# gvanhorn38/multibox

Measured on AMD Instinct MI355X. Metric: images/sec (299x299, 5-AR priors) train, higher is better.
Workload: dtype bf16; 1 GPU; full train step: Inception-ResNet-v2 + multibox heads fwd, on-device matching+loss, bwd, RMSProp+EMA; 299x299, k=5 (P=646), BATCH_SIZE=64/GPU, MAX_NUM_BBOXES=13; global_batch=64, parallelism=dp1, hip_graph=True

## Files before the change

### include/mbx.h

```cpp
#ifndef MBX_H
#define MBX_H

#include <stddef.h>
#include <stdint.h>

#ifdef __cplusplus
extern "C" {
#endif

typedef void* mbx_stream_t;

typedef enum {
  MBX_OK = 0,
  MBX_ERR_INVALID_ARG = -1,
  MBX_ERR_UNSUPPORTED = -2,
  MBX_ERR_LAUNCH = -3,
  MBX_ERR_WORKSPACE = -4
} mbx_status;

int mbx_version(void);
const char* mbx_status_string(int status);

int mbx_priors_count(int k, const int* grids, int n_grids);

uint32_t mbx_crc32c(const void* data, uint64_t n, uint32_t crc);
int mbx_generate_priors(const double* aspect_ratios, int k, double min_scale, double max_scale,
                        int restrict_to_image_bounds, const int* grids, int n_grids,
                        double* out );

int mbx_decode_conf(const float* raw_locs , const float* logits ,
                    const float* priors , int B, int P, float eps_add,
                    float* decoded , float* conf , mbx_stream_t stream);

size_t mbx_match_workspace_bytes(int B, int P, int G);
int mbx_match(const float* decoded , const float* conf ,
              const float* gt , const int32_t* n_gt , float alpha,
              int B, int P, int G, int32_t* match , int32_t* status ,
              void* workspace, size_t workspace_bytes, mbx_stream_t stream);

int mbx_match_extend(const float* priors , const float* gt ,
                     const int32_t* n_gt , const int32_t* status ,
                     float iou_threshold, int B, int P, int G,
                     int32_t* match ,
                     int32_t* n_extra , mbx_stream_t stream);

size_t mbx_loss_workspace_bytes(int B);
int mbx_loss_fwd_bwd(const float* decoded , const float* conf_in ,
                     int conf_is_logit, const float* gt ,
                     const int32_t* match , float alpha, float grad_scale, int B, int P,
                     int G, float* loss2 ,
                     float* d_raw_locs , float* d_logits ,
                     void* workspace, size_t workspace_bytes, mbx_stream_t stream);

size_t mbx_loss_mined_workspace_bytes(int B, int P);
int mbx_loss_fwd_bwd_mined(const float* decoded , const float* conf_in ,
                           int conf_is_logit, const float* gt ,
                           const int32_t* match , float alpha, float grad_scale, int B, int P,
                           int G, float* loss2 ,
                           float* d_raw_locs , float* d_logits ,
                           int neg_per_pos, int min_neg, int32_t* n_neg ,
                           void* workspace, size_t workspace_bytes, mbx_stream_t stream);

size_t mbx_loss_focal_workspace_bytes(int B, int P);
int mbx_loss_fwd_bwd_focal(const float* decoded , const float* conf_in ,
                           int conf_is_logit, const float* gt ,
                           const int32_t* match , float alpha, float grad_scale, int B, int P,
                           int G, float* loss2 ,
                           float* d_raw_locs , float* d_logits ,
                           float gamma, float w_pos, float w_neg,
                           int neg_per_pos , int min_neg, int32_t* n_neg ,
                           void* workspace, size_t workspace_bytes, mbx_stream_t stream);

typedef struct {
  int32_t offset_y, offset_x;
  int32_t patch_h, patch_w;
  int32_t image_h, image_w;
  int32_t is_flipped;
  int32_t max_to_keep;
  float restrictions[4];
} mbx_patch_meta;

int mbx_decode_filter_topk(const float* raw_locs , const float* conf ,
                           const float* priors , const mbx_patch_meta* meta ,
                           int B, int P, int k_max, double* out_boxes ,
                           float* out_scores , int32_t* out_index ,
                           int32_t* out_count , mbx_stream_t stream);

int mbx_nms(double* boxes , float* scores , int32_t* index ,
            int32_t* count , int B, int k_max, double iou_threshold, mbx_stream_t stream);

#define MBX_MERGE_MAX_CANDIDATES 16384
int mbx_merge_detections(const double* boxes , const float* scores ,
                         const int32_t* count , const int32_t* image_rows , int I, int k_max,
                         int max_det, double iou_threshold, double* out_boxes ,
                         float* out_scores , int32_t* out_src ,
                         int32_t* out_count , int32_t* out_status , mbx_stream_t stream);

int mbx_merge_detections_voted(const double* boxes , const float* scores ,
                               const int32_t* count , const int32_t* image_rows , int I,
                               int k_max, int max_det, double iou_threshold, double vote_iou_threshold,
                               double* out_boxes , float* out_scores ,
                               int32_t* out_src , int32_t* out_count ,
                               int32_t* out_status , int32_t* out_votes , mbx_stream_t stream);

#define MBX_SOFT_LINEAR 1
#define MBX_SOFT_GAUSSIAN 2
int mbx_merge_detections_soft(const double* boxes , const float* scores ,
                              const int32_t* count , const int32_t* image_rows , int I, int k_max,
                              int max_det, int method, double iou_threshold , double sigma ,
                              double min_score, double vote_iou_threshold ,
                              double* out_boxes , float* out_scores ,
                              int32_t* out_src , int32_t* out_count , int32_t* out_status ,
                              int32_t* out_votes , mbx_stream_t stream);

#define MBX_COCO_MAX_DET 100
#define MBX_COCO_MAX_GT 128
int mbx_coco_match(const double* dt , const int32_t* dt_rows ,
                   const double* gt , const int32_t* gt_rows , int I,
                   const double* iou_thrs , int T, const double* area_rng ,
                   int A, int16_t* match , uint8_t* ignore ,
                   int32_t* n_gt_counted , int32_t* status , mbx_stream_t stream);

#define MBX_COCO_ACC_MAX_R 128
#define MBX_COCO_ACC_MAX_M 4
#define MBX_COCO_ACC_MAX_ND 4194304
#define MBX_COCO_ACC_CHUNK 256
#define MBX_COCO_ACC_SORT_TILE 1024
size_t mbx_coco_accumulate_workspace(long long ND, int T, int A, int M);
int mbx_coco_accumulate(const double* dt , const int32_t* dt_rows , int I,
                        const int16_t* match , const uint8_t* ignore ,
                        const int32_t* n_gt_counted , int T, int A, const double* rec_thrs , int R,
                        const int32_t* max_dets , int M, double* precision ,
                        double* recall , void* workspace, size_t workspace_bytes, mbx_stream_t stream);

typedef enum {
  MBX_EPI_STORE = 0,
  MBX_EPI_AFFINE = 1,
  MBX_EPI_RESIDUAL = 2,
  MBX_EPI_STORE_F32 = 3
} mbx_epilogue;

typedef struct {
  int32_t n, rows_mod;
  int32_t c_begin[4];
  const void* y[4]; int32_t ld_y[4];
  const float* relu_thr[4];
  float* stats[4]; int32_t stats_ld[4];
} mbx_bn_bwd_stats;

#define MBX_GRID_BARRIER_BYTES 6400
typedef struct {
  void* barrier;
  void* a; int32_t ld_a;
  const float* beta;
  float* mean; float* rstd;
  float* moving_mean; float* moving_var;
  float* relu_thr;
  int32_t relu; float eps, decay;
  float* step_poison;
} mbx_bn_apply_desc;

#define MBX_BN_BWD_SLOTS 8
typedef struct {
  void* barrier;
  int32_t n;
  int32_t c_begin[4];
  const void* y[4]; int32_t ld_y[4];
  void* dy[4]; int32_t ld_dy[4];
  const float* mean[4]; const float* rstd[4]; const float* beta[4];
  float* dbeta[4];
  float* acc[4]; int32_t acc_ld[4];
  int32_t relu[4];
  float* step_poison;
} mbx_bn_bwd_fused;

typedef struct {
  const void* x; int64_t x_img_stride; int32_t ldx;
  int32_t N, H_in, W_in, C_in;
  const void* w; int32_t C_out, R, S;
  int32_t stride, transposed, pad_t, pad_l, H_out, W_out;
  void* y; int64_t y_img_stride; int32_t ldy;
  int32_t epilogue, relu, accumulate;
  const float* scale; const float* shift;
  const void* skip; int64_t skip_img_stride; int32_t ld_skip; float rscale;
  float* stats_partial;
  int32_t tile_config;
  const void* acc_src; int64_t acc_img_stride; int32_t ld_acc;
  int32_t* work_counter;
  int32_t max_workgroups;
  void* splitk_ws; int64_t splitk_ws_bytes;
  int32_t stats_rows_mod, stats_ld;
  const mbx_bn_bwd_stats* bn_bwd_stats;
  void* relu_bits; int32_t ld_bits;
  const mbx_bn_apply_desc* bn_apply;
  const mbx_bn_bwd_fused* bn_bwd;
} mbx_conv_desc;
#define MBX_CONV_TILE_CONFIGS 14
#define MBX_TILE_I5_BASE 32
#define MBX_TILE_I7 65
#define MBX_TILE_DIRECT3 96
#define MBX_TILE_DIRECTW 97
#define MBX_TILE_RESIDENT 98
#define MBX_TILE_PWRES 99
#define MBX_TILE_SPLITK_BASE 128
#define MBX_TILE_SPLITK_MAX 32

int mbx_conv_stats_rows(const mbx_conv_desc* desc );
int mbx_conv(const mbx_conv_desc* desc , mbx_stream_t stream);
int mbx_conv_supported(const mbx_conv_desc* desc );
int mbx_conv_pair(const mbx_conv_desc* a , const mbx_conv_desc* b , mbx_stream_t stream);
size_t mbx_conv_splitk_workspace_bytes(const mbx_conv_desc* desc );

int mbx_conv_wgrad(const mbx_conv_desc* desc , const void* dy,
                   int64_t dy_img_stride, int32_t ld_dy, float* dw, float* db, mbx_stream_t stream);

typedef struct {
  mbx_conv_desc desc;
  const void* dy; int64_t dy_img_stride; int32_t ld_dy;
  float scale;
  float* dw; float* db;
} mbx_wgrad_job;
typedef struct {
  int32_t n_layers, n_items;
  int64_t layers_off, items_off;
  int64_t queues_off, heads_off;
  double flops;
  int64_t tally_off;
} mbx_wgrad_plan_info;
#define MBX_WGRAD_DETERMINISTIC 1
#define MBX_WGRAD_SCATTER 2
size_t mbx_wgrad_plan_bytes(const mbx_wgrad_job* jobs , int n_jobs, int flags);
int mbx_wgrad_plan(const mbx_wgrad_job* jobs , int n_jobs, int flags, void* host_image, size_t bytes,
                   mbx_wgrad_plan_info* info );
int mbx_conv_wgrad_grouped(void* device_image , const mbx_wgrad_plan_info* info ,
                           mbx_stream_t stream);
int mbx_conv_wgrad_grouped_capped(void* device_image, const mbx_wgrad_plan_info* info , int max_workgroups,
                                  mbx_stream_t stream);

int mbx_conv_wgrad_scaled(const mbx_conv_desc* desc, const void* dy, int64_t dy_img_stride,
                          int32_t ld_dy, float scale, float* dw, float* db, mbx_stream_t stream);

int mbx_bn_finalize(const float* stats_partial , int rows, int C, int64_t count,
                    float eps, float decay, float* mean , float* rstd ,
                    float* moving_mean , float* moving_var ,
                    mbx_stream_t stream);
int mbx_bn_apply(const void* y, int64_t M, int C, const float* mean, const float* rstd,
                 const float* beta, int relu, void* a, int ld_a, mbx_stream_t stream);
int mbx_bn_apply_fused(const float* stats_partial, int rows, int64_t count, float eps, float decay,
                       const void* y, int64_t M, int C, const float* beta, int relu, void* a, int ld_a,
                       float* mean, float* rstd, float* moving_mean, float* moving_var,
                       mbx_stream_t stream);
int mbx_bn_apply_fused_mapped(const void* stats_fixed, int rows, int64_t count, float eps, float decay,
                              const void* y, int64_t M, int C, const float* beta, int relu, void* a, int ld_a,
                              const struct mbx_chan_map_s* a_map , float* mean, float* rstd, float* moving_mean,
                              float* moving_var, float* relu_thr, mbx_stream_t stream);
int mbx_bn_moving_update(float* moving_mean, float* moving_var, const float* batch_mean, const float* batch_var,
                         int64_t n, float decay, const float* skip_ctl, uint64_t* skipped_steps,
                         float* ema_mean, float* ema_var, float ema_decay, mbx_stream_t stream);
typedef struct mbx_chan_map_s { int32_t n; int32_t c_begin[4]; int32_t offset[4]; } mbx_chan_map;
int mbx_bn_finalize_parts(const float* const* parts , const int32_t* rows ,
                          const int32_t* Cs , int n_parts, int64_t count, float eps, float decay, float* mean,
                          float* rstd, float* moving_mean, float* moving_var, mbx_stream_t stream);
int mbx_bn_apply_mapped(const void* y, int64_t M, int C, const float* mean, const float* rstd, const float* beta,
                        int relu, void* a, int ld_a, const mbx_chan_map* a_map , mbx_stream_t stream);
int mbx_bn_apply_maxpool(const void* y, int N, int H, int W, int C, const float* mean, const float* rstd, const float* beta,
                         int relu, void* p, int64_t p_img_stride, int ld_p, int Ho, int Wo, uint8_t* argmax,
                         mbx_stream_t stream);
int mbx_bn_fold(const float* moving_mean, const float* moving_var, const float* beta, float eps,
                int C, float* scale, float* shift, mbx_stream_t stream);
int mbx_bn_bwd_rows(int64_t M, int C);
int mbx_bn_bwd_reduce(const void* da, int ld_da, const void* a, int ld_a, int relu, const void* y,
                      int64_t M, int C, const float* mean, const float* rstd, const float* beta,
                      float* partial , mbx_stream_t stream);
int mbx_bn_bwd_finalize(const float* partial, int rows, int C, int64_t M, float* dbeta ,
                        float* m12 , mbx_stream_t stream);
int mbx_bn_bwd_apply(const void* da, int ld_da, const void* a, int ld_a, int relu, const void* y,
                     int64_t M, int C, const float* mean, const float* rstd, const float* beta,
                     const float* m12, void* dy , mbx_stream_t stream);

int mbx_bn_bwd_reduce_mapped(const void* da, int ld_da, const void* a, int ld_a, int relu, const void* y, int64_t M, int C,
                             const float* mean, const float* rstd, const float* beta, float* partial,
                             const mbx_chan_map* da_map , mbx_stream_t stream);
int mbx_bn_bwd_apply_mapped(const void* da, int ld_da, const void* a, int ld_a, int relu, const void* y, int64_t M, int C,
                            const float* mean, const float* rstd, const float* beta, const float* m12, void* dy,
                            const mbx_chan_map* da_map , mbx_stream_t stream);

int mbx_bn_bwd_apply_rows(const float* stats, int rows, const void* da, int ld_da, const void* y, int64_t M, int C,
                          const float* mean, const float* rstd, const float* relu_thr, float* dbeta, void* dy,
                          const mbx_chan_map* da_map , mbx_stream_t stream);

size_t mbx_bn_bwd_onepass_workspace_bytes(int C);
int mbx_bn_bwd_onepass_supported(int64_t M, int C, int max_workgroups);
int mbx_bn_bwd_onepass(const void* da, int ld_da, int relu, const void* y, int64_t M, int C,
                       const float* mean, const float* rstd, const float* beta, float* dbeta ,
                       void* dy , void* ws, int max_workgroups, float* step_poison ,
                       mbx_stream_t stream);

int mbx_bn_bwd_rows_pooled(int N, int H, int W, int C);
int mbx_bn_bwd_reduce_pooled(const void* gy, int64_t gy_img_stride, int ld_gy, const uint8_t* argmax, int N, int H, int W,
                             int Ho, int Wo, int relu, const void* y, int C, const float* mean, const float* rstd,
                             const float* beta, float* partial , mbx_stream_t stream);
int mbx_bn_bwd_apply_pooled(const void* gy, int64_t gy_img_stride, int ld_gy, const uint8_t* argmax, int N, int H, int W,
                            int Ho, int Wo, int relu, const void* y, int C, const float* mean, const float* rstd,
                            const float* beta, const float* m12, void* dy, mbx_stream_t stream);
int mbx_bn_bwd_onepass_mapped(const void* da, int ld_da, int relu, const void* y, int64_t M, int C, const float* mean,
                              const float* rstd, const float* beta, float* dbeta, void* dy, void* ws, int max_workgroups,
                              float* step_poison, const mbx_chan_map* da_map , mbx_stream_t stream);

int mbx_maxpool_fwd(const void* x, int64_t x_img_stride, int ldx, int N, int H, int W, int C,
                    int k, int stride, void* y, int64_t y_img_stride, int ldy, int Ho, int Wo,
                    uint8_t* argmax , mbx_stream_t stream);
int mbx_maxpool_bwd(const void* dy, int64_t dy_img_stride, int ld_dy, const uint8_t* argmax,
                    int N, int H, int W, int C, int k, int stride, int Ho, int Wo, void* dx,
                    int64_t dx_img_stride, int ld_dx, int accumulate, mbx_stream_t stream);
int mbx_avgpool_fwd(const void* x, int64_t x_img_stride, int ldx, int N, int H, int W, int C,
                    int k, int pad, void* y, int64_t y_img_stride, int ldy, int Ho, int Wo,
                    mbx_stream_t stream);
int mbx_avgpool_bwd(const void* dy, int64_t dy_img_stride, int ld_dy, int N, int H, int W, int C,
                    int k, int pad, int Ho, int Wo, void* dx, int64_t dx_img_stride, int ld_dx,
                    int accumulate, mbx_stream_t stream);

int mbx_relu_mask(void* g, int ld_g, const void* a, int ld_a, int64_t M, int C, mbx_stream_t stream);
int mbx_pack_input(const float* img, int64_t pixels, void* out, mbx_stream_t stream);
int mbx_head_gather(const float* h, int ld_h, int N, int cells, int k, int P, int off,
                    float* locs, float* logits, mbx_stream_t stream);
int mbx_head_scatter(const float* d_locs, const float* d_logits, int N, int cells, int k, int P,
                     int off, void* g, int ld_g, mbx_stream_t stream);

typedef struct {
  const float* h; int32_t ld_h;
  void* g; int32_t ld_g;
  int32_t cells, k, off;
} mbx_head;
int mbx_head_gather_all(const mbx_head* heads , int n_heads, int N, int P, float* locs, float* logits,
                        mbx_stream_t stream);
int mbx_head_scatter_all(const float* d_locs, const float* d_logits, const mbx_head* heads , int n_heads, int N,
                         int P, mbx_stream_t stream);

int mbx_step_begin(float* grads, int64_t n_grads, float* bn_ws, int64_t n_ws, int64_t ctl_index, uint64_t* timeouts_total,
                   float* zero_scalar, mbx_stream_t stream);

typedef struct {
  int64_t src_off;
  int64_t dst_off;
  int32_t K, R, S, C, Kpad;
  int32_t first_block;
} mbx_filter_entry;
int mbx_filter_prepare(const void* w_bf16, void* w_dgrad, const mbx_filter_entry* table ,
                       int n_entries, int total_blocks, mbx_stream_t stream);

int mbx_rmsprop_ema_step(float* w, const float* g, float* ms, float* mom ,
                         float* ema , void* w_bf16 , int64_t n, float lr,
                         float decay, float momentum, float eps, float wd, float ema_decay,
                         int trainable, float* reg_loss, const float* skip_ctl, mbx_stream_t stream);
int mbx_ema_update(float* ema, const float* value, int64_t n, float ema_decay, const float* skip_ctl ,
                   mbx_stream_t stream);

typedef struct {
  uint64_t src_offset;
  int32_t src_h, src_w;
  int32_t method;
  int32_t flip;
  int32_t n_ops;
  int32_t op[4];
  int32_t pad_;
  double arg[4];
} mbx_augment_item;
size_t mbx_augment_workspace_bytes(int B, int S);
int mbx_augment_batch(const uint8_t* src , const mbx_augment_item* items , int B, int S,
                      int any_contrast, float* out , void* workspace, mbx_stream_t stream);

typedef struct {
  uint64_t src_offset;
  int32_t img_h, img_w;
  int32_t win_y, win_x, win_h, win_w;
  int32_t flip_source;
  int32_t pad_;
} mbx_patch_item;
int mbx_extract_patches(const uint8_t* src , const mbx_patch_item* items , int n, int S,
                        float* out , mbx_stream_t stream);

#ifdef __cplusplus
}
#endif
#endif
```

### multibox_amd/csrc/conv.hip

```cpp
#include <stdlib.h>

#include "conv_common.h"

namespace {

template <int BM, int BN, int WNW, int WMW, int EV, int MODE = 0, int NSTG = 3>
__device__ __forceinline__ void conv_igemm3_body(const ConvK& p, const int bid_, const int nblk_) {
  constexpr bool SH = MODE == 2, PW = MODE == 1;
  static_assert(WNW * WMW == 4 || WNW * WMW == 8, "four or eight waves");
  constexpr int NT = 64 * WNW * WMW, RPP = NT / 8;
  constexpr int TN = BN / WNW, TM = BM / WMW, NI = TN / 16, MI = TM / 16;
  constexpr int PI = BM / RPP, WI = BN / RPP, NL = PI + WI;
  constexpr int STAGE = (BM + BN) * 8;
  extern __shared__ __attribute__((aligned(16))) u32x4 smem[];

  const int tid = threadIdx.x, lane = tid & 63;
  const int wave = wave_id();
  const int wn = wave % WNW, wm = wave / WNW;
  int lid = xcd_remap(bid_, nblk_);
  int split = 0;
  if constexpr (EV == 5) { const int nt = p.tiles_m * p.tiles_n; split = lid / nt; lid -= split * nt; }
  const int tile_n = lid % p.tiles_n, tile_m = lid / p.tiles_n;
  const int m0 = tile_m * BM, n0 = tile_n * BN;

  const __amdgpu_buffer_rsrc_t xr = make_rsrc(p.x, p.x_bytes);
  const __amdgpu_buffer_rsrc_t wr = make_rsrc(p.w, p.w_bytes);
  const int lrow = tid >> 3;
  const int chunk = (tid & 7) ^ (lrow & 7);
  const int chunkw = (tid & 7) ^ ((((lrow >> 3) & 3) << 1) | ((lrow >> 1) & 1));
  int hb[PI], wb[PI], ro[PI];
#pragma unroll
  for (int i = 0; i < PI; ++i) {
    const int m = m0 + lrow + RPP * i;
    const bool mv = m < p.M;
    const unsigned mm = mv ? (unsigned)m : 0u;
    int img, oh, ow;
    if (SH && p.parity) decode_pixel_parity(p, mm, img, oh, ow); else decode_pixel(p, mm, img, oh, ow);
    hb[i] = mv ? oh * p.mul - p.pad_t : -(1 << 24);
    wb[i] = ow * p.mul - p.pad_l;
    ro[i] = SH ? img * p.x_img_stride * 2 : (img * p.x_img_stride + (hb[i] * p.W_in + wb[i]) * p.ldx) * 2;
    if (PW && !mv) ro[i] = (int)kOOB;
  }
  int wo[WI];
#pragma unroll
  for (int i = 0; i < WI; ++i) {
    const int n = n0 + lrow + RPP * i;
    wo[i] = n < p.C_out ? n * p.Ktot * 2 : -1;
  }

  f32x4 acc[NI][MI];
#pragma unroll
  for (int a = 0; a < NI; ++a)
#pragma unroll
    for (int b = 0; b < MI; ++b) acc[a][b] = f32x4{0.f, 0.f, 0.f, 0.f};

  const int frow = lane & 15, fch = lane >> 4;
  const int fr0 = frow * 8 + (fch ^ (frow & 7));
  const int fr1 = frow * 8 + ((4 + fch) ^ (frow & 7));
  const int fwrow = 8 * (frow >> 2) + (frow & 3), fwkey = ((frow >> 2) << 1) | ((frow >> 1) & 1);
  const int fw0 = fwrow * 8 + (fch ^ fwkey);
  const int fw1 = fwrow * 8 + ((4 + fch) ^ fwkey);
  int kr0 = 0, ks0 = 0, kstep = 1, nk = (p.Ktot + 63) >> 6;
  if (SH && p.skip_taps) {
    const int mlast = min(m0 + BM, p.M) - 1;
    const int c0 = pixel_class(p, m0);
    if (c0 == pixel_class(p, mlast)) {
      kr0 = (p.pad_t + (c0 >> 1)) & 1;
      ks0 = (p.pad_l + (c0 & 1)) & 1;
      kstep = 2;
      nk = ((p.R - kr0 + 1) >> 1) * ((p.S - ks0 + 1) >> 1) * (p.C_in >> 6);
    }
  }
  int kt0 = 0;
  if constexpr (EV == 5) { kt0 = split * p.kps; nk = min(p.kps, nk - kt0); }
  int kc = chunk * 8 + kt0 * 64, kr = kr0, ks = ks0;
  while (kc >= p.C_in) { kc -= p.C_in; if ((ks += kstep) >= p.S) { ks = ks0; kr += kstep; } }
  const int ldx2 = p.ldx * 2;
  int st_issue = 0, st_comp = 0;
#define MBX_ISSUE_TILE(LT)                                                                                   \
  do {                                                                                                       \
    u32x4* sp = smem + st_issue * STAGE + wave * 64;                                                         \
    const bool kv = kr < p.R;                                                                                \
    if (PW) {                                                                                                \
      _Pragma("unroll") for (int i = 0; i < PI; ++i)                                                         \
        glds16(xr, sp + i * NT, (kv && ro[i] >= 0) ? (ro[i] + kc * 2) : (int)kOOB);                          \
    } else if (!SH) {                                                                                        \
      const int toff = (kr * p.W_in + ks) * ldx2 + kc * 2;                                                   \
      _Pragma("unroll") for (int i = 0; i < PI; ++i) {                                                       \
        const bool ok = kv && ((unsigned)(hb[i] + kr) < (unsigned)p.H_in) &&                                 \
                        ((unsigned)(wb[i] + ks) < (unsigned)p.W_in);                                         \
        glds16(xr, sp + i * NT, ok ? (ro[i] + toff) : (int)kOOB);                                            \
      }                                                                                                      \
    } else {                                                                                                 \
      _Pragma("unroll") for (int i = 0; i < PI; ++i) {                                                       \
        const int hn = hb[i] + kr, wn_ = wb[i] + ks;                                                         \
        const bool ok = kv && (((hn | wn_) & 1) == 0) && ((unsigned)(hn >> 1) < (unsigned)p.H_in) &&         \
                        ((unsigned)(wn_ >> 1) < (unsigned)p.W_in);                                           \
        glds16(xr, sp + i * NT, ok ? (ro[i] + ((hn >> 1) * p.W_in + (wn_ >> 1)) * ldx2 + kc * 2) : (int)kOOB); \
      }                                                                                                      \
    }                                                                                                        \
                                 \
    const int kb = (SH && kstep == 2) ? ((kr * p.S + ks) * p.C_in + kc + (chunkw - chunk) * 8) * 2                \
                                      : (((LT) + kt0) * 64 + chunkw * 8) * 2;                                  \
    const bool kvw = (SH && kstep == 2) ? kv : (kb < p.Ktot * 2);                                              \
    u32x4* sw = sp + BM * 8;                                                                                 \
    _Pragma("unroll") for (int i = 0; i < WI; ++i)                                                           \
      glds16(wr, sw + i * NT, (kvw && wo[i] >= 0) ? (wo[i] + kb) : (int)kOOB);                               \
    kc += 64;                                                                                                \
    while (kc >= p.C_in) { kc -= p.C_in; if ((ks += kstep) >= p.S) { ks = ks0; kr += kstep; } }              \
    st_issue = st_issue == NSTG - 1 ? 0 : st_issue + 1;                                                      \
  } while (0)

  static_assert(NSTG == 2 || NSTG == 3, "ring depth");
  u32x4* const probe_base = smem + (PI + WI - 1) * NT + wave * 64 + lane;
  MBX_ISSUE_TILE(0);
  if (NSTG == 3 && nk > 1) { MBX_ISSUE_TILE(1); wait_vmcnt<NL>(); } else wait_vmcnt<0>();
  lds_readback_wait(lds_readback_issue(probe_base));
  raw_barrier();
  for (int it = 0; it < nk; ++it) {
    const bool more = it + NSTG - 1 < nk;
    if (more) MBX_ISSUE_TILE(it + NSTG - 1);
    st_comp = st_comp == NSTG - 1 ? 0 : st_comp + 1;
    const int st_prev = st_comp == 0 ? NSTG - 1 : st_comp - 1;
#ifndef MBX_NO_PROBE_I3
    unsigned probe;
    if constexpr (NSTG == 3) {
      if (more) wait_vmcnt<NL>(); else wait_vmcnt<0>();
      probe = lds_readback_issue(probe_base + st_comp * STAGE);
    }
#endif
    {
      const u32x4* cP = smem + st_prev * STAGE + (wm * TM) * 8;
      const u32x4* cW = smem + st_prev * STAGE + BM * 8 + (wn * TN) * 8;
#pragma unroll
      for (int kk = 0; kk < 2; ++kk) {
        const int fr = kk ? fr1 : fr0, fw = kk ? fw1 : fw0;
        bf16x8 wf[NI], pf[MI];
#pragma unroll
        for (int a = 0; a < NI; ++a) wf[a] = __builtin_bit_cast(bf16x8, cW[(a >> 1) * 256 + (a & 1) * 32 + fw]);
#pragma unroll
        for (int b = 0; b < MI; ++b) pf[b] = __builtin_bit_cast(bf16x8, cP[b * 128 + fr]);
#pragma unroll
        for (int a = 0; a < NI; ++a)
#pragma unroll
          for (int b = 0; b < MI; ++b)
            acc[a][b] = __builtin_amdgcn_mfma_f32_16x16x32_bf16(wf[a], pf[b], acc[a][b], 0, 0, 0);
      }
    }
#ifndef MBX_NO_PROBE_I3
    if constexpr (NSTG == 2) {
      wait_vmcnt<0>();
      probe = lds_readback_issue(probe_base + st_comp * STAGE);
    }
    lds_readback_wait(probe);
#else
    if (NSTG == 3 && more) wait_vmcnt<NL>(); else wait_vmcnt<0>();
#endif
    raw_barrier();
  }
#undef MBX_ISSUE_TILE
  wait_vmcnt<0>();
  static_assert(NI % 2 == 0, "wave tile: a multiple of 32 output channels");
  constexpr int NA = NI / 2;
  const int cl0 = wn * TN + fch * 8;
  if constexpr (EV == 5) {
#pragma unroll
    for (int b = 0; b < MI; ++b) {
      const int m = m0 + wm * TM + b * 16 + frow;
      if (m >= p.M) continue;
      const int img = (int)fast_div((unsigned)m, p.mg_hw, p.sh_hw), pix = m - img * p.HW_out;
      float* yrow = reinterpret_cast<float*>(p.y) + split * p.y_split_stride + img * p.y_img_stride + pix * p.ldy;
#pragma unroll
      for (int a = 0; a < NI; ++a) {
        const int c0 = n0 + cl0 + 32 * (a >> 1) + 4 * (a & 1);
#pragma unroll
        for (int r = 0; r < 4; ++r)
          if (c0 + r < p.C_out) yrow[c0 + r] = acc[a][b][r];
      }
    }
  } else {
    float s1[NA][8], s2[NA][8];
    conv_epilogue_direct<EV, SH, NI, MI, ((EV == 2 || EV == 6) && MI * NA >= 8 && MI % 2 == 0) ? 2 : MI>(p, acc, m0 + wm * TM + frow, n0 + cl0, s1, s2);
    if constexpr (EV == 1 || EV == 6) {
      float* red = reinterpret_cast<float*>(smem);
#pragma unroll
      for (int A = 0; A < NA; ++A) { row_sum16_x8(s1[A]); row_sum16_x8(s2[A]); }
#pragma unroll
      for (int A = 0; A < NA; ++A)
#pragma unroll
        for (int j = 0; j < 8; ++j) {
          const float x1 = s1[A][j], x2 = s2[A][j];
          if (frow == 0) {
            red[((wm * BN) + cl0 + 32 * A + j) * 2] = x1;
            red[((wm * BN) + cl0 + 32 * A + j) * 2 + 1] = x2;
          }
        }
      __syncthreads();
      if (tid < BN && n0 + tid < p.C_out) {
        float x1 = 0.f, x2 = 0.f;
#pragma unroll
        for (int w = 0; w < WMW; ++w) { x1 += red[(w * BN + tid) * 2]; x2 += red[(w * BN + tid) * 2 + 1]; }
        if constexpr (EV == 6) bw_stats_write(p, tile_m, n0 + tid, x1, x2); else stats_write(p, tile_m, n0 + tid, x1, x2);
      }
    }
  }
}

template <int BM, int BN, int WNW, int WMW, int EV, int MODE = 0, int NSTG = 3>
__global__ void __launch_bounds__(64 * WNW * WMW)
conv_igemm3_kernel(const ConvK p) {
  conv_igemm3_body<BM, BN, WNW, WMW, EV, MODE, NSTG>(p, (int)blockIdx.x, (int)gridDim.x);
}

template <int BM, int BN, int WNW, int WMW, int EV, int MODE = 0, int NSTG = 3>
__global__ void __launch_bounds__(64 * WNW * WMW)
conv_igemm3_pair_kernel(const ConvK p0, const ConvK p1, const int n0) {
  if ((int)blockIdx.x < n0) conv_igemm3_body<BM, BN, WNW, WMW, EV, MODE, NSTG>(p0, (int)blockIdx.x, n0);
  else conv_igemm3_body<BM, BN, WNW, WMW, EV, MODE, NSTG>(p1, (int)blockIdx.x - n0, (int)gridDim.x - n0);
}

constexpr int kSplitRows = 16;
__global__ void __launch_bounds__(256)
splitk_reduce_kernel(const float* __restrict__ part, int ksplit, long long slice_stride, int M, int C, int ldp,
                     unsigned short* __restrict__ y, int HW_out, long long y_img_stride, int ldy, float* __restrict__ stats,
                     int stats_mod, int stats_ld, float stats_cap) {
  __shared__ float red[kSplitRows][256][2];
  const int m0 = blockIdx.x * kSplitRows, tid = threadIdx.x;
  for (int cb = 0; cb < C; cb += 256) {
    const int cw = min(256, C - cb), c4 = (cw + 3) >> 2;
    if (cb) __syncthreads();
    for (int item = tid; item < kSplitRows * c4; item += 256) {
      const int r = item / c4, gq = item - r * c4, m = m0 + r, c = cb + 4 * gq;
      float4 a = make_float4(0.f, 0.f, 0.f, 0.f);
      if (m < M) {
        const float* src = part + (size_t)m * ldp + c;
        a = *reinterpret_cast<const float4*>(src);
        int sl = 1;
        for (; sl + 3 < ksplit; sl += 4) {
          const float4 b0 = *reinterpret_cast<const float4*>(src + (sl + 0) * slice_stride);
          const float4 b1 = *reinterpret_cast<const float4*>(src + (sl + 1) * slice_stride);
          const float4 b2 = *reinterpret_cast<const float4*>(src + (sl + 2) * slice_stride);
          const float4 b3 = *reinterpret_cast<const float4*>(src + (sl + 3) * slice_stride);
          a.x = (((a.x + b0.x) + b1.x) + b2.x) + b3.x; a.y = (((a.y + b0.y) + b1.y) + b2.y) + b3.y;
          a.z = (((a.z + b0.z) + b1.z) + b2.z) + b3.z; a.w = (((a.w + b0.w) + b1.w) + b2.w) + b3.w;
        }
        for (; sl < ksplit; ++sl) {
          const float4 b = *reinterpret_cast<const float4*>(src + sl * slice_stride);
          a.x += b.x; a.y += b.y; a.z += b.z; a.w += b.w;
        }
      }
      const float v[4] = {a.x, a.y, a.z, a.w};
      const unsigned q2[2] = {pack2bf(v[0], v[1]), pack2bf(v[2], v[3])};
      const unsigned q[4] = {q2[0] & 0xffffu, q2[0] >> 16, q2[1] & 0xffffu, q2[1] >> 16};
#pragma unroll
      for (int j = 0; j < 4; ++j) {
        const float f = (m < M && c + j < C) ? bf2f((unsigned short)q[j]) : 0.f;
        if (4 * gq + j < 256) { red[r][4 * gq + j][0] = f; red[r][4 * gq + j][1] = f * f; }
      }
      if (m < M) {
        const int img = m / HW_out, pix = m - img * HW_out;
        unsigned short* dst = y + img * y_img_stride + (long long)pix * ldy + c;
        if (c + 3 < C) *reinterpret_cast<u32x2*>(dst) = u32x2{q2[0], q2[1]};
        else for (int j = 0; j < 4; ++j) if (c + j < C) dst[j] = (unsigned short)q[j];
      }
    }
    if (stats) {
      __syncthreads();
      if (tid < cw) {
        float x1 = 0.f, x2 = 0.f;
#pragma unroll
        for (int r = 0; r < kSplitRows; ++r) { x1 += red[r][tid][0]; x2 += red[r][tid][1]; }
        if (stats_mod) {
          unsigned long long* o = reinterpret_cast<unsigned long long*>(stats) + ((size_t)((int)blockIdx.x % stats_mod) * stats_ld + cb + tid) * 2;
          stats_add_fixed(o, x1, x2, stats_cap);
        } else {
          float* o = stats + ((size_t)blockIdx.x * stats_ld + cb + tid) * 2;
          o[0] = x1;
          o[1] = x2;
        }
      }
    }
  }
}

struct TileCfg { int BM, BN; float eff; };
const TileCfg kCfgs[] = {{128, 128, 1.00f}, {128, 64, 0.85f}, {64, 128, 0.85f}, {128, 32, 0.60f}, {64, 64, 0.70f},
                          {256, 128, 1.30f}, {128, 128, 1.10f}, {256, 64, 1.0f},
                          {128, 128, 1.10f},
                          {128, 64, 0.85f}, {64, 64, 0.70f},
                          {128, 64, 0.85f}, {256, 64, 1.0f}, {128, 128, 1.0f}};

int pick_cfg(long M, int C_out) {
  int best = 0;
  double best_t = 1e300;
  for (int i = 0; i < (int)(sizeof(kCfgs) / sizeof(kCfgs[0])); ++i) {
    if (i >= 5) continue;
    const TileCfg& c = kCfgs[i];
    const long tiles = ((M + c.BM - 1) / c.BM) * ((C_out + c.BN - 1) / c.BN);
    const long lds = 3L * (c.BM + c.BN) * 128;
    long per_cu = (160 * 1024) / lds;
    if (per_cu > 2) per_cu = 2;
    const long rounds = (tiles + 256 * per_cu - 1) / (256 * per_cu);
    const double t = (double)rounds * c.BM * c.BN / c.eff;
    if (t < best_t) { best_t = t; best = i; }
  }
  return best;
}



constexpr int kNumCfgs = MBX_CONV_TILE_CONFIGS;
static_assert(kGbCtlWords * 4 == MBX_GRID_BARRIER_BYTES && kFbSlots == MBX_BN_BWD_SLOTS, "include/mbx.h and csrc/grid_barrier.h agree");
constexpr int kI5Flag = MBX_TILE_I5_BASE;
constexpr int kI7Cfg = MBX_TILE_I7;
constexpr int kDirectCfg = MBX_TILE_DIRECT3;
constexpr int kDirectWCfg = MBX_TILE_DIRECTW;
constexpr int kResidentCfg = MBX_TILE_RESIDENT;
constexpr int kPwResCfg = MBX_TILE_PWRES;
constexpr int kSplitFlag = MBX_TILE_SPLITK_BASE;
constexpr int kSplitMax = MBX_TILE_SPLITK_MAX;
inline void splitk_geom(int nk, int S, int& ksplit, int& kps) {
  if (S > nk) S = nk;
  if (S < 1) S = 1;
  kps = (nk + S - 1) / S;
  ksplit = (nk + kps - 1) / kps;
}
int choose_cfg(long M, int C_out, int desc_cfg) {
  static const int force = mbx_env_int("MBX_FORCE_CFG", -1);
  if (force >= 0) return force;
  if (desc_cfg > 0 && desc_cfg <= kNumCfgs) return desc_cfg - 1;
  {
    const long cols = (C_out + 127) / 128, tiles8 = ((M + 127) / 128) * cols;
    if (tiles8 >= 384 && (double)C_out >= 0.6 * (double)(cols * 128)) return 8;
  }
  if (C_out >= 256) {
    const long tiles5 = ((M + 255) / 256) * ((C_out + 127) / 128);
    const long rounds5 = (tiles5 + 255) / 256;
    if (tiles5 >= 128 && (double)tiles5 / (double)(rounds5 * 256) >= 0.7) return 5;
  }
  return pick_cfg(M, C_out);
}

struct PairCapture { ConvK k; int bm, bn, wnw, wmw, nstg, ev, mode, valid; };
thread_local PairCapture g_capture;

template <int BM, int BN, int WNW, int WMW, int EV, int NSTG>
int launch_pair_inst(const ConvK& a, const ConvK& b, hipStream_t s) {
  static bool attr = false;
  const size_t lds = NSTG * (size_t)(BM + BN) * 128;
  if (!attr) {
    (void)hipFuncSetAttribute(reinterpret_cast<const void*>(conv_igemm3_pair_kernel<BM, BN, WNW, WMW, EV, 0, NSTG>),
                              hipFuncAttributeMaxDynamicSharedMemorySize, (int)lds);
    attr = true;
  }
  const int n0 = a.tiles_m * a.tiles_n, n1 = b.tiles_m * b.tiles_n;
  hipLaunchKernelGGL((conv_igemm3_pair_kernel<BM, BN, WNW, WMW, EV, 0, NSTG>), dim3(n0 + n1), dim3(64 * WNW * WMW), lds, s, a, b, n0);
  MBX_LAUNCH_CHECK();
  return MBX_OK;
}

template <int BM, int BN, int WNW, int WMW, int NSTG = 3>
int launch_igemm(ConvK& k, hipStream_t s) {
  k.tiles_m = (k.M + BM - 1) / BM;
  k.tiles_n = (k.C_out + BN - 1) / BN;
  k.stats_cap = stats_cap_for(k.tiles_m);
  if (k.dry == 2) {
    g_capture.k = k; g_capture.bm = BM; g_capture.bn = BN; g_capture.wnw = WNW; g_capture.wmw = WMW; g_capture.nstg = NSTG;
    g_capture.ev = k.epi == MBX_EPI_STORE_F32 ? 5 : k.epi == MBX_EPI_RESIDUAL ? 4 : k.epi == MBX_EPI_AFFINE ? 3
                   : k.bw_n ? 6 : k.stats ? 1 : (k.accumulate || k.skip || k.bits) ? 2 : 0;
    g_capture.mode = k.shift ? 2 : k.pw ? 1 : 0;
    g_capture.valid = 1;
    return MBX_OK;
  }
  {
    const size_t lds = NSTG * (size_t)(BM + BN) * 128;
    const int ev = k.epi == MBX_EPI_STORE_F32 ? 5 : k.epi == MBX_EPI_RESIDUAL ? 4 : k.epi == MBX_EPI_AFFINE ? 3
                   : k.bw_n ? 6 : k.stats ? 1 : (k.accumulate || k.skip || k.bits) ? 2 : 0;
    static bool attr_set3[7] = {false, false, false, false, false, false, false};
#define MBX_LAUNCH_EV(EV)                                                                                     \
    case EV:                                                                                                  \
      if (!attr_set3[EV]) {                                                                                   \
        (void)hipFuncSetAttribute(reinterpret_cast<const void*>(conv_igemm3_kernel<BM, BN, WNW, WMW, EV, 0, NSTG>), \
                                  hipFuncAttributeMaxDynamicSharedMemorySize, (int)lds);                      \
        (void)hipFuncSetAttribute(reinterpret_cast<const void*>(conv_igemm3_kernel<BM, BN, WNW, WMW, EV, 1, NSTG>), \
                                  hipFuncAttributeMaxDynamicSharedMemorySize, (int)lds);                      \
        attr_set3[EV] = true;                                                                                 \
      }                                                                                                       \
      if (k.pw)                                                                                               \
        hipLaunchKernelGGL((conv_igemm3_kernel<BM, BN, WNW, WMW, EV, 1, NSTG>), dim3(k.tiles_m * k.tiles_n * (EV == 5 ? k.ksplit : 1)), \
                           dim3(64 * WNW * WMW), lds, s, k);                                                  \
      else                                                                                                    \
        hipLaunchKernelGGL((conv_igemm3_kernel<BM, BN, WNW, WMW, EV, 0, NSTG>), dim3(k.tiles_m * k.tiles_n * (EV == 5 ? k.ksplit : 1)), \
                           dim3(64 * WNW * WMW), lds, s, k);                                                  \
      break;
    static bool attr_sh[2] = {false, false};
#define MBX_LAUNCH_SH(EV, SLOT)                                                                               \
    do {                                                                                                      \
      if (!attr_sh[SLOT]) {                                                                                   \
        (void)hipFuncSetAttribute(reinterpret_cast<const void*>(conv_igemm3_kernel<BM, BN, WNW, WMW, EV, 2, NSTG>), \
                                  hipFuncAttributeMaxDynamicSharedMemorySize, (int)lds);                      \
        attr_sh[SLOT] = true;                                                                                 \
      }                                                                                                       \
      hipLaunchKernelGGL((conv_igemm3_kernel<BM, BN, WNW, WMW, EV, 2, NSTG>), dim3(k.tiles_m * k.tiles_n),      \
                         dim3(64 * WNW * WMW), lds, s, k);                                                    \
    } while (0)
    if (k.dry) return (k.shift && ev != 0 && ev != 2) ? MBX_ERR_UNSUPPORTED : MBX_OK;
    if (k.shift) {
      if (ev == 0) MBX_LAUNCH_SH(0, 0);
      else if (ev == 2) MBX_LAUNCH_SH(2, 1);
      else return MBX_ERR_UNSUPPORTED;
    } else
    switch (ev) {
      MBX_LAUNCH_EV(0) MBX_LAUNCH_EV(1) MBX_LAUNCH_EV(2) MBX_LAUNCH_EV(3) MBX_LAUNCH_EV(4) MBX_LAUNCH_EV(5) MBX_LAUNCH_EV(6)
    }
#undef MBX_LAUNCH_SH
#undef MBX_LAUNCH_EV
  }
  MBX_LAUNCH_CHECK();
  return MBX_OK;
}

}

extern "C" int mbx_conv_stats_rows(const mbx_conv_desc* d) {
  if (!d) return MBX_ERR_INVALID_ARG;
  if (d->stats_rows_mod > 0) return d->stats_rows_mod;
  const long M = (long)d->N * d->H_out * d->W_out;
  if (d->tile_config > kSplitFlag) return (int)((M + kSplitRows - 1) / kSplitRows);
  if (d->tile_config == kDirectCfg) return mbx_direct3_grid(d->N, d->H_out, d->W_out);
  if (d->tile_config == kDirectWCfg) { const int g = mbx_directw_grid(d->N, d->H_out, d->W_out); return g > 0 ? g : MBX_ERR_UNSUPPORTED; }
  if (d->tile_config == kResidentCfg) return mbx_resident_rows(d->N);
  if (d->tile_config == kI7Cfg) return (int)((M + 127) / 128);
  if (d->tile_config > kI5Flag) {
    const int i = d->tile_config - kI5Flag - 1;
    if (i >= mbx_i5_num_tiles) return MBX_ERR_INVALID_ARG;
    return (int)((M + mbx_i5_tiles[i][0] - 1) / mbx_i5_tiles[i][0]);
  }
  const TileCfg& c = kCfgs[choose_cfg(M, d->C_out, d->tile_config)];
  return (int)((M + c.BM - 1) / c.BM);
}

static int conv_impl(const mbx_conv_desc* d, mbx_stream_t stream, int dry);
extern "C" int mbx_conv(const mbx_conv_desc* d, mbx_stream_t stream) { return conv_impl(d, stream, 0); }
extern "C" int mbx_conv_supported(const mbx_conv_desc* d) { return conv_impl(d, nullptr, 1); }
extern "C" int mbx_conv_pair(const mbx_conv_desc* a, const mbx_conv_desc* b, mbx_stream_t stream) {
  PairCapture ca, cb;
  g_capture.valid = 0;
  int st = conv_impl(a, stream, 2);
  if (st != MBX_OK) return st;
  if (!g_capture.valid) return MBX_ERR_UNSUPPORTED;
  ca = g_capture;
  g_capture.valid = 0;
  st = conv_impl(b, stream, 2);
  if (st != MBX_OK) return st;
  if (!g_capture.valid) return MBX_ERR_UNSUPPORTED;
  cb = g_capture;
  if (ca.bm != cb.bm || ca.bn != cb.bn || ca.wnw != cb.wnw || ca.wmw != cb.wmw || ca.nstg != cb.nstg || ca.ev != cb.ev ||
      ca.mode != 0 || cb.mode != 0 || (ca.ev != 0 && ca.ev != 1 && ca.ev != 6) || ca.wnw != 2 || ca.wmw != 2 || ca.bn != 64)
    return MBX_ERR_UNSUPPORTED;
  ca.k.dry = cb.k.dry = 0;
  hipStream_t s = mbx_s(stream);
#define MBX_PAIR(BM_, NSTG_)                                                                                      \
  if (ca.bm == BM_ && ca.nstg == NSTG_)                                                                           \
    return ca.ev == 6 ? launch_pair_inst<BM_, 64, 2, 2, 6, NSTG_>(ca.k, cb.k, s)                                    \
           : ca.ev ? launch_pair_inst<BM_, 64, 2, 2, 1, NSTG_>(ca.k, cb.k, s) : launch_pair_inst<BM_, 64, 2, 2, 0, NSTG_>(ca.k, cb.k, s);
  MBX_PAIR(128, 2) MBX_PAIR(128, 3) MBX_PAIR(64, 2) MBX_PAIR(64, 3)
#undef MBX_PAIR
  return MBX_ERR_UNSUPPORTED;
}

extern "C" size_t mbx_conv_splitk_workspace_bytes(const mbx_conv_desc* d) {
  if (!d || d->tile_config <= kSplitFlag || d->tile_config > kSplitFlag + kSplitMax) return 0;
  int ksplit, kps;
  splitk_geom((d->R * d->S * d->C_in + 63) >> 6, d->tile_config - kSplitFlag, ksplit, kps);
  return (size_t)4 * d->N * d->H_out * d->W_out * (((d->C_out + 7) / 8) * 8) * ksplit;
}

static int conv_impl(const mbx_conv_desc* d, mbx_stream_t stream, int dry) {
  int st = check_desc(d);
  if (st != MBX_OK) return st;
  if (!d->w || !d->y) return MBX_ERR_INVALID_ARG;
  if ((reinterpret_cast<uintptr_t>(d->w) & 15)) return MBX_ERR_INVALID_ARG;
  const bool f32 = d->epilogue == MBX_EPI_STORE_F32;
  if (!f32 && (d->C_out % 8 || d->ldy % 8 || (reinterpret_cast<uintptr_t>(d->y) & 15))) return MBX_ERR_INVALID_ARG;
  if (d->epilogue == MBX_EPI_RESIDUAL && (!d->skip || d->ld_skip % 8 || (reinterpret_cast<uintptr_t>(d->skip) & 15)))
    return MBX_ERR_INVALID_ARG;
  if ((long long)d->N * d->y_img_stride >= (1LL << 31)) return MBX_ERR_UNSUPPORTED;
  if (d->stats_partial && (d->epilogue != MBX_EPI_STORE || d->accumulate || d->skip)) return MBX_ERR_INVALID_ARG;
  if (d->epilogue == MBX_EPI_STORE && d->skip && (d->ld_skip % 8 || (reinterpret_cast<uintptr_t>(d->skip) & 15))) return MBX_ERR_INVALID_ARG;
  MBX_ENTER();
  ConvK k;
  k.x = reinterpret_cast<const unsigned short*>(d->x);
  k.x_img_stride = (int)d->x_img_stride; k.ldx = d->ldx; k.H_in = d->H_in; k.W_in = d->W_in; k.C_in = d->C_in;
  k.w = reinterpret_cast<const unsigned short*>(d->w);
  k.C_out = d->C_out; k.R = d->R; k.S = d->S; k.Ktot = d->R * d->S * d->C_in;
  k.x_bytes = (unsigned)(2 * ((long long)(d->N - 1) * d->x_img_stride + ((long long)d->H_in * d->W_in - 1) * d->ldx + d->C_in));
  k.w_bytes = (unsigned)(2LL * d->C_out * k.Ktot);
  if (d->transposed) { k.mul = 1; k.shift = d->stride == 2 ? 1 : 0; } else { k.mul = d->stride; k.shift = 0; }
  k.pad_t = d->pad_t; k.pad_l = d->pad_l; k.W_out = d->W_out; k.HW_out = d->H_out * d->W_out;
  k.M = d->N * k.HW_out;
  k.y = d->y; k.y_img_stride = (int)d->y_img_stride; k.ldy = d->ldy;
  k.epi = d->epilogue; k.relu = d->relu; k.accumulate = d->accumulate;
  k.scale = d->scale; k.shiftv = d->shift;
  k.skip = reinterpret_cast<const unsigned short*>(d->skip);
  k.skip_img_stride = (int)d->skip_img_stride; k.ld_skip = d->ld_skip; k.rscale = d->rscale;
  k.bits = nullptr; k.bits_ld = 0; k.bits_bytes = 0;
  if (d->relu_bits) {
    const bool wr = d->epilogue == MBX_EPI_RESIDUAL && d->relu, rd = d->epilogue == MBX_EPI_STORE && !d->skip;
    if ((!wr && !rd) || d->ld_bits % 4 || d->ld_bits < 4 * ((d->C_out + 31) / 32) || (reinterpret_cast<uintptr_t>(d->relu_bits) & 3)) return MBX_ERR_INVALID_ARG;
    if (d->stats_partial || d->bn_bwd_stats) return MBX_ERR_UNSUPPORTED;
    const long long bb = (long long)d->N * d->H_out * d->W_out * d->ld_bits;
    if (bb >= (1LL << 31)) return MBX_ERR_UNSUPPORTED;
    k.bits = reinterpret_cast<unsigned char*>(d->relu_bits); k.bits_ld = d->ld_bits; k.bits_bytes = (unsigned)bb;
  }
  k.stats = d->stats_partial;
  if (d->stats_rows_mod < 0 || d->stats_rows_mod > 1024 || d->stats_ld < 0 || (d->stats_ld && d->stats_ld < d->C_out)) return MBX_ERR_INVALID_ARG;
  k.stats_mod = d->stats_rows_mod; k.stats_ld = d->stats_ld ? d->stats_ld : d->C_out;
  k.stats_cap = 0.f;
  k.fa = FusedApply{};
  k.fa.bar = nullptr;
  k.fb = FusedBwd{};
  k.fb.bar = nullptr;
  if (d->bn_bwd) {
    const mbx_bn_bwd_fused* b = d->bn_bwd;
    if (!b->barrier || (reinterpret_cast<uintptr_t>(b->barrier) & 127) || b->n < 1 || b->n > 4 || b->c_begin[0] != 0) return MBX_ERR_INVALID_ARG;
    if (d->epilogue != MBX_EPI_STORE || d->accumulate || d->skip || d->relu_bits || d->stats_partial || d->bn_bwd_stats || d->bn_apply ||
        d->stride != 1 || d->C_out > 2048 || d->y_img_stride != (int64_t)d->H_out * d->W_out * d->ldy)
      return MBX_ERR_UNSUPPORTED;
    const int tc = d->tile_config;
    if (!((tc > kI5Flag && tc <= kI5Flag + 7) || tc == kDirectWCfg || tc == kResidentCfg)) return MBX_ERR_UNSUPPORTED;
    const long long Mll = (long long)d->N * d->H_out * d->W_out;
    for (int i = 0; i < 4; ++i) k.fb.cb[i] = 1 << 30;
    for (int i = 0; i < b->n; ++i) {
      if (!b->y[i] || !b->dy[i] || !b->mean[i] || !b->rstd[i] || (b->relu[i] && !b->beta[i]) || !b->acc[i] ||
          (reinterpret_cast<uintptr_t>(b->y[i]) & 15) || (reinterpret_cast<uintptr_t>(b->dy[i]) & 15) || b->ld_y[i] % 8 || b->ld_dy[i] % 8 ||
          b->c_begin[i] % 8 || b->c_begin[i] >= d->C_out || (i && b->c_begin[i] <= b->c_begin[i - 1]) || b->acc_ld[i] <= 0)
        return MBX_ERR_INVALID_ARG;
      if (Mll * b->ld_y[i] >= (1LL << 31) || Mll * b->ld_dy[i] >= (1LL << 31)) return MBX_ERR_UNSUPPORTED;
      k.fb.cb[i] = b->c_begin[i];
      k.fb.y[i] = reinterpret_cast<const unsigned short*>(b->y[i]); k.fb.ldy[i] = b->ld_y[i];
      k.fb.dy[i] = reinterpret_cast<unsigned short*>(b->dy[i]); k.fb.lddy[i] = b->ld_dy[i];
      k.fb.mean[i] = b->mean[i]; k.fb.rstd[i] = b->rstd[i]; k.fb.beta[i] = b->beta[i]; k.fb.dbeta[i] = b->dbeta[i];
      k.fb.acc[i] = b->acc[i]; k.fb.acc_ld[i] = b->acc_ld[i]; k.fb.relu[i] = b->relu[i];
    }
    const int fault = mbx_barrier_fault() == '3';
    k.fb.n = b->n;
    k.fb.bar = reinterpret_cast<unsigned*>(b->barrier);
    static const int probe = mbx_env_int("MBX_FUSED_PROBE", 0) & ~1;
    k.fb.spin_limit = fault ? (1u << 10) : (1u << 22); k.fb.fault = fault | probe; k.fb.step_poison = b->step_poison;
    k.fb.inv_M = (float)(1.0 / (double)Mll);
  }
  if (d->bn_apply) {
    const mbx_bn_apply_desc* b = d->bn_apply;
    if (!b->barrier || !b->a || !b->beta || !b->mean || !b->rstd || (reinterpret_cast<uintptr_t>(b->barrier) & 127) ||
        (reinterpret_cast<uintptr_t>(b->a) & 15) || b->ld_a % 8 || b->ld_a < d->C_out)
      return MBX_ERR_INVALID_ARG;
    if (!d->stats_partial || d->stats_rows_mod < 1 || d->stats_rows_mod > 16 || d->epilogue != MBX_EPI_STORE || d->accumulate || d->skip ||
        d->transposed || d->rscale != 0.f || d->C_out > 2048 || d->y_img_stride != (int64_t)d->H_out * d->W_out * d->ldy ||
        (long long)d->N * d->H_out * d->W_out * b->ld_a >= (1LL << 31))
      return MBX_ERR_UNSUPPORTED;
    const int tc = d->tile_config;
    if (!((tc > kI5Flag && tc <= kI5Flag + 7) || tc == kDirectWCfg || tc == kResidentCfg)) return MBX_ERR_UNSUPPORTED;
    const int fault = mbx_barrier_fault() == '2';
    k.fa.bar = reinterpret_cast<unsigned*>(b->barrier);
    static const int probe = mbx_env_int("MBX_FUSED_PROBE", 0) & ~1;
    k.fa.spin_limit = fault ? (1u << 10) : (1u << 22); k.fa.fault = fault | probe; k.fa.step_poison = b->step_poison;
    k.fa.a = reinterpret_cast<unsigned short*>(b->a); k.fa.ld_a = b->ld_a; k.fa.beta = b->beta;
    k.fa.mean = b->mean; k.fa.rstd = b->rstd; k.fa.mmean = b->moving_mean; k.fa.mvar = b->moving_var; k.fa.thr = b->relu_thr;
    k.fa.relu = b->relu; k.fa.eps = b->eps; k.fa.decay = b->decay;
    k.fa.inv_count = 1.0 / (double)((long long)d->N * d->H_out * d->W_out);
  }
  k.bw_n = 0; k.bw_mod = 1;
  for (int i = 0; i < 4; ++i) { k.bw_cb[i] = 1 << 30; k.bw_ldy[i] = 0; k.bw_sld[i] = 0; k.bw_y[i] = nullptr; k.bw_thr[i] = nullptr; k.bw_stats[i] = nullptr; }
  if (d->bn_bwd_stats) {
    const mbx_bn_bwd_stats* b = d->bn_bwd_stats;
    if (d->epilogue != MBX_EPI_STORE || d->accumulate || d->skip || d->stats_partial || b->n < 1 || b->n > 4 || b->rows_mod < 1 ||
        b->rows_mod > 1024 || b->c_begin[0] != 0)
      return MBX_ERR_INVALID_ARG;
    for (int i = 0; i < b->n; ++i) {
      if (!b->y[i] || !b->relu_thr[i] || !b->stats[i] || (reinterpret_cast<uintptr_t>(b->y[i]) & 15) || b->ld_y[i] % 8 || b->c_begin[i] % 32 ||
          b->c_begin[i] >= d->C_out || (i && b->c_begin[i] <= b->c_begin[i - 1]) || b->stats_ld[i] <= 0)
        return MBX_ERR_INVALID_ARG;
      k.bw_cb[i] = b->c_begin[i]; k.bw_ldy[i] = b->ld_y[i]; k.bw_sld[i] = b->stats_ld[i];
      k.bw_y[i] = reinterpret_cast<const unsigned short*>(b->y[i]); k.bw_thr[i] = b->relu_thr[i]; k.bw_stats[i] = b->stats[i];
    }
    k.bw_n = b->n; k.bw_mod = b->rows_mod;
  }
  if (d->accumulate && d->acc_src) {
    if (d->ld_acc % 8 || (reinterpret_cast<uintptr_t>(d->acc_src) & 15) || (long long)d->N * d->acc_img_stride >= (1LL << 31))
      return MBX_ERR_INVALID_ARG;
    k.acc_src = reinterpret_cast<const unsigned short*>(d->acc_src); k.acc_img_stride = (int)d->acc_img_stride; k.ld_acc = d->ld_acc;
  } else {
    k.acc_src = reinterpret_cast<const unsigned short*>(d->y); k.acc_img_stride = (int)d->y_img_stride; k.ld_acc = d->ldy;
  }
  {
    const long long last_pix = (long long)k.HW_out - 1, span = ((d->C_out + 7) / 8) * 8;
    const long long yb = 2 * ((long long)(d->N - 1) * d->y_img_stride + last_pix * d->ldy + span);
    const long long sb = d->skip ? 2 * ((long long)(d->N - 1) * d->skip_img_stride + last_pix * d->ld_skip + span) : 0;
    const long long ab = 2 * ((long long)(d->N - 1) * k.acc_img_stride + last_pix * k.ld_acc + span);
    if (!f32 && (yb >= (1LL << 31) || sb >= (1LL << 31) || ab >= (1LL << 31))) return MBX_ERR_UNSUPPORTED;
    k.y_bytes = (unsigned)yb; k.skip_bytes = (unsigned)sb; k.acc_bytes = (unsigned)ab;
  }
  set_magic((unsigned)k.HW_out, k.mg_hw, k.sh_hw);
  set_magic((unsigned)k.W_out, k.mg_w, k.sh_w);
  k.pw = (d->R == 1 && d->S == 1 && d->pad_t == 0 && d->pad_l == 0 && d->stride == 1) ? 1 : 0;
  k.skip_taps = 0; k.parity = 0;
  k.work_counter = d->work_counter;
  k.max_wg = d->max_workgroups;
  k.dry = dry;
  k.ksplit = 1; k.kps = 1 << 30; k.y_split_stride = 0;
#ifdef MBX_I5_STAMPS
  {
    static const unsigned long long sp = getenv("MBX_I5_STAMP_PTR") ? strtoull(getenv("MBX_I5_STAMP_PTR"), nullptr, 10) : 0ull;
    k.stamps = reinterpret_cast<unsigned long long*>(sp);
    k.dbg = mbx_env_int("MBX_I5_DBG", 0);
    k.stagger = mbx_env_int("MBX_STAGGER", 0);
  }
#endif
  for (int c = 0; c < 4; ++c) { k.cls_m0[c] = 0; k.cls_hw[c] = 1; k.cls_w[c] = 1; }
  static const bool notap = mbx_env_char("MBX_NO_TAP_SKIP") == '1';
  if (k.shift && d->C_in % 64 == 0 && !notap) {
    int m0 = 0;
    for (int c = 0; c < 4; ++c) {
      const int hc = (d->H_out - (c >> 1) + 1) / 2, wc = (d->W_out - (c & 1) + 1) / 2;
      k.cls_m0[c] = m0;
      k.cls_hw[c] = hc * wc > 0 ? hc * wc : 1;
      k.cls_w[c] = wc > 0 ? wc : 1;
      m0 += d->N * hc * wc;
    }
    k.skip_taps = k.parity = 1;
  }
  if (k.bits && k.shift) return MBX_ERR_UNSUPPORTED;
  hipStream_t s = mbx_s(stream);
  if (d->tile_config > kSplitFlag) {
    const int S = d->tile_config - kSplitFlag;
    if (S < 2 || S > kSplitMax || d->transposed || d->bn_bwd_stats || d->relu_bits || d->epilogue != MBX_EPI_STORE || d->accumulate || d->skip || d->rscale != 0.f)
      return MBX_ERR_UNSUPPORTED;
    const int ldp = ((d->C_out + 7) / 8) * 8;
    int ksplit, kps;
    splitk_geom((k.Ktot + 63) >> 6, S, ksplit, kps);
    const long long slice = (long long)k.M * ldp;
    if (!d->splitk_ws || (reinterpret_cast<uintptr_t>(d->splitk_ws) & 15) || d->splitk_ws_bytes < (int64_t)(4 * slice * ksplit) ||
        slice * ksplit >= (1LL << 31))
      return MBX_ERR_WORKSPACE;
    ConvK g = k;
    g.epi = MBX_EPI_STORE_F32; g.stats = nullptr; g.relu = 0;
    g.y = d->splitk_ws; g.ldy = ldp; g.y_img_stride = k.HW_out * ldp;
    g.ksplit = ksplit; g.kps = kps; g.y_split_stride = slice;
    st = launch_igemm<128, 64, 2, 2>(g, s);
    if (st != MBX_OK || dry) return st;
    hipLaunchKernelGGL(splitk_reduce_kernel, dim3((k.M + kSplitRows - 1) / kSplitRows), dim3(256), 0, s, reinterpret_cast<const float*>(d->splitk_ws),
                       ksplit, slice, k.M, k.C_out, ldp, reinterpret_cast<unsigned short*>(k.y), k.HW_out,
                       (long long)k.y_img_stride, k.ldy, k.stats, k.stats_mod, k.stats_ld, stats_cap_for((k.M + kSplitRows - 1) / kSplitRows));
    MBX_LAUNCH_CHECK();
    return MBX_OK;
  }
  if (d->tile_config == kDirectCfg) return mbx_launch_direct3(k, d->N, d->H_out, s);
  if (d->tile_config == kDirectWCfg) return mbx_launch_directw(k, d->N, d->H_out, s);
  if (d->tile_config == kResidentCfg) return mbx_launch_resident(k, d->N, d->H_out, s);
  if (d->tile_config == kPwResCfg) return mbx_launch_pwres(k, s);
  if (d->tile_config == kI7Cfg) return mbx_launch_igemm7(k, s);
  if (d->tile_config > kI5Flag) return mbx_launch_igemm5(k, d->tile_config - kI5Flag - 1, s);
  switch (choose_cfg(k.M, k.C_out, d->tile_config)) {
    case 0: return launch_igemm<128, 128, 2, 2>(k, s);
    case 1: return launch_igemm<128, 64, 2, 2>(k, s);
    case 2: return launch_igemm<64, 128, 2, 2>(k, s);
    case 3: return launch_igemm<128, 32, 1, 4>(k, s);
    case 5: return launch_igemm<256, 128, 2, 4>(k, s);
    case 6: return launch_igemm<128, 128, 2, 4>(k, s);
    case 7: return launch_igemm<256, 64, 1, 8>(k, s);
    case 8: return launch_igemm<128, 128, 2, 4, 2>(k, s);
    case 9: return launch_igemm<128, 64, 2, 2, 2>(k, s);
    case 10: return launch_igemm<64, 64, 2, 2, 2>(k, s);
    case 11: return launch_igemm<128, 64, 2, 4, 2>(k, s);
    case 12: return launch_igemm<256, 64, 1, 8, 2>(k, s);
    case 13: return launch_igemm<128, 128, 2, 2, 2>(k, s);
    default: return launch_igemm<64, 64, 2, 2>(k, s);
  }
}
```

### multibox_amd/csrc/conv5.hip

```cpp
#include "conv_common.h"
#ifndef MBX_I5_NST4
#define MBX_I5_NST4 4
#endif

namespace {

template <int MY, int NW>
struct Ig5 {
  static constexpr int BM = 64 * MY, BN = 64 * NW;
  static_assert(NW >= 1 && NW <= 4, "64 / 128 / 192 / 256 output channels per tile");
  static constexpr int WM = (NW == 1) ? (MY == 4 ? 8 : 4) : (NW == 3) ? 4 : (MY == 4 && NW == 2) ? 4 : 2;
  static constexpr int WN = 8 / WM;
  static constexpr int TM = BM / WM, TN = BN / WN, MI = TM / 16, NI = TN / 16;
  static constexpr int STAGE = (BM + BN) * 8;
  static constexpr int RED_BYTES = WM * BN * 2 * 4;
  static constexpr int NST = (4 * STAGE * 16 + RED_BYTES + 64 <= 160 * 1024) ? MBX_I5_NST4 : 3;
  static constexpr int RING_BYTES = NST * STAGE * 16;
  static constexpr int LDS_BYTES = RING_BYTES + RED_BYTES + 16;
  static_assert(TM % 16 == 0 && TN % 32 == 0 && WM * WN == 8, "wave grid");
  static_assert(LDS_BYTES <= 160 * 1024, "LDS");
};

template <int MY, int NW, int EV, int MODE>
__global__ void __launch_bounds__(1024)
conv_igemm5_kernel(const ConvK p) {
  using G = Ig5<MY, NW>;
  constexpr bool PW = MODE == 1;
  constexpr int BM = G::BM, BN = G::BN, TM = G::TM, TN = G::TN, MI = G::MI, NI = G::NI, STAGE = G::STAGE, NST = G::NST;
  constexpr int NLW = 8, LV = 1;
  constexpr int NL = LV * (MY + NW);
  static_assert((NST - 2) * NL < 64, "vmcnt");
  constexpr int NBAR = (EV == 1 || EV == 6) ? 1 : 0;
  extern __shared__ __attribute__((aligned(16))) u32x4 smem[];
  float* const red = reinterpret_cast<float*>(smem + NST * STAGE);
  typedef __attribute__((address_space(3))) int* lds_int_ptr;
  const lds_int_ptr s_ids = (lds_int_ptr)(red + G::WM * BN * 2);

  const int tid = threadIdx.x, lane = tid & 63;
  const int wave = wave_id();
  const int ntiles = p.tiles_m * p.tiles_n;
  const int first = xcd_remap(blockIdx.x, gridDim.x);
#ifdef MBX_I5_STAMPS
  if (p.stagger) {
    const int n = (first & 3) * p.stagger;
    for (int i = 0; i < n; ++i) __builtin_amdgcn_s_sleep(8);
  }
#endif
  const int nk = (p.Ktot + 63) >> 6;
  const bool fused_tail = ((EV == 1) && p.fa.bar != nullptr) || ((EV == 0) && p.fb.bar != nullptr);
  const bool queued = p.work_counter != nullptr && nk > NST && ntiles > (int)gridDim.x && !fused_tail;

  if (wave >= 8) {
    const int lw0 = wave - 8;
    const __amdgpu_buffer_rsrc_t xr = make_rsrc(p.x, p.x_bytes);
    const __amdgpu_buffer_rsrc_t wr = make_rsrc(p.w, p.w_bytes);
    const int r8 = lane >> 3;
    const int chunk = (lane & 7) ^ r8;
    int chunkw[LV];
#pragma unroll
    for (int v = 0; v < LV; ++v) chunkw[v] = (lane & 7) ^ ((((lw0 + NLW * v) & 3) << 1) | ((r8 >> 1) & 1));
    const int ldx2 = p.ldx * 2;
    int t_i = first, it_i = 0, st_issue = 0, j_i = 0;
    int hb[LV][MY], wb[LV][MY], ro[LV][MY], wo[LV][NW];
    int kc = 0, kr = 0, ks = 0;
#define MBX5_SETUP_TILE()                                                                                     \
  do {                                                                                                        \
    const int tn_ = t_i % p.tiles_n, tm_ = t_i / p.tiles_n;                                                   \
    _Pragma("unroll") for (int v = 0; v < LV; ++v) {                                                          \
      const int lw = lw0 + NLW * v;                                                                           \
      _Pragma("unroll") for (int i = 0; i < MY; ++i) {                                                        \
        const int m = tm_ * BM + 64 * i + 8 * lw + r8;                                                        \
        const bool mv = m < p.M;                                                                              \
        int img, oh, ow;                                                                                      \
        decode_pixel(p, mv ? (unsigned)m : 0u, img, oh, ow);                                                  \
        hb[v][i] = mv ? oh * p.mul - p.pad_t : -(1 << 24);                                                    \
        wb[v][i] = ow * p.mul - p.pad_l;                                                                      \
        ro[v][i] = (img * p.x_img_stride + (hb[v][i] * p.W_in + wb[v][i]) * p.ldx) * 2;                       \
        if (PW && !mv) ro[v][i] = (int)kOOB;                                                                  \
      }                                                                                                       \
      _Pragma("unroll") for (int i = 0; i < NW; ++i) {                                                        \
        const int n = tn_ * BN + 64 * i + 8 * lw + r8;                                                        \
        wo[v][i] = n < p.C_out ? n * p.Ktot * 2 : -1;                                                         \
      }                                                                                                       \
    }                                                                                                         \
    kc = chunk * 8; kr = 0; ks = 0;                                                                           \
    while (kc >= p.C_in) { kc -= p.C_in; if (++ks >= p.S) { ks = 0; ++kr; } }                                 \
  } while (0)
#define MBX5_ISSUE_A()                                                                                        \
  do {                                                                                                        \
    const bool kv = kr < p.R;                                                                                 \
    _Pragma("unroll") for (int v = 0; v < LV; ++v) {                                                          \
      u32x4* sp = smem + st_issue * STAGE + (lw0 + NLW * v) * 64;                                             \
      if (PW) {                                                                                               \
        _Pragma("unroll") for (int i = 0; i < MY; ++i)                                                        \
          glds16(xr, sp + i * 512, (kv && ro[v][i] >= 0) ? (ro[v][i] + kc * 2) : (int)kOOB);                  \
      } else {                                                                                                \
        const int toff = (kr * p.W_in + ks) * ldx2 + kc * 2;                                                  \
        _Pragma("unroll") for (int i = 0; i < MY; ++i) {                                                      \
          const bool ok = kv && ((unsigned)(hb[v][i] + kr) < (unsigned)p.H_in) &&                             \
                          ((unsigned)(wb[v][i] + ks) < (unsigned)p.W_in);                                     \
          glds16(xr, sp + i * 512, ok ? (ro[v][i] + toff) : (int)kOOB);                                       \
        }                                                                                                     \
      }                                                                                                       \
    }                                                                                                         \
  } while (0)
#define MBX5_ISSUE_B()                                                                                        \
  do {                                                                                                        \
    _Pragma("unroll") for (int v = 0; v < LV; ++v) {                                                          \
      u32x4* sp = smem + st_issue * STAGE + (lw0 + NLW * v) * 64;                                             \
      const int kb = (it_i * 64 + chunkw[v] * 8) * 2;                     \
      const bool kvw = kb < p.Ktot * 2;                                                                       \
      _Pragma("unroll") for (int i = 0; i < NW; ++i)                                                          \
        glds16(wr, sp + (MY + i) * 512, (kvw && wo[v][i] >= 0) ? (wo[v][i] + kb) : (int)kOOB);                \
    }                                                                                                         \
    kc += 64;                                                                                                 \
    while (kc >= p.C_in) { kc -= p.C_in; if (++ks >= p.S) { ks = 0; ++kr; } }                                 \
    st_issue = st_issue == NST - 1 ? 0 : st_issue + 1;                                                        \
    if (++it_i == nk) {                                                                                       \
      it_i = 0; ++j_i;                                                                                        \
      t_i = queued ? s_ids[j_i & 3] : t_i + (int)gridDim.x;                                                   \
      if (t_i < ntiles) MBX5_SETUP_TILE();                                                                    \
    }                                                                                                         \
  } while (0)
#define MBX5_ISSUE() do { MBX5_ISSUE_A(); MBX5_ISSUE_B(); } while (0)
#define MBX5_READBACK() lds_readback_wait(lds_readback_issue(smem + st_pub * STAGE + (MY + NW - 1) * 512 + (lw0 + NLW * (LV - 1)) * 64 + lane))

    int st_pub = 0;
    if (t_i < ntiles) {
      MBX5_SETUP_TILE();
      MBX5_ISSUE();
      bool full = true;
#pragma unroll
      for (int a = 1; a < NST - 1; ++a) {
        if (t_i < ntiles) MBX5_ISSUE(); else full = false;
      }
      if (full) wait_vmcnt<(NST - 2) * NL>(); else wait_vmcnt<0>();
      MBX5_READBACK();
    }
    raw_barrier();
    int jc = 0;
    for (int t = first; t < ntiles; t = queued ? s_ids[++jc & 3] : t + (int)gridDim.x) {
      for (int it = 0; it < nk; ++it) {
        const bool more = t_i < ntiles;
        st_pub = st_pub == NST - 1 ? 0 : st_pub + 1;
#ifdef MBX_I5_STAMPS
        if (p.dbg & 4) { raw_barrier(); continue; }
#endif
        if (more) MBX5_ISSUE_A();
#ifdef MBX_I5_STAMPS
        if (p.dbg & 2) { if (more) MBX5_ISSUE_B(); raw_barrier(); continue; }
#endif
#ifndef MBX_NO_PROBE_I5
        if (more) wait_vmcnt<(NST - 3) * NL + LV * MY>(); else wait_vmcnt<0>();
        const unsigned probe = lds_readback_issue(smem + st_pub * STAGE + (MY + NW - 1) * 512 + (lw0 + NLW * (LV - 1)) * 64 + lane);
        if (more) MBX5_ISSUE_B();
        lds_readback_wait(probe);
#else
        if (more) { MBX5_ISSUE_B(); wait_vmcnt<(NST - 2) * NL>(); } else wait_vmcnt<0>();
#endif
        raw_barrier();
      }
#pragma unroll 1
      for (int b = 0; b < NBAR; ++b) raw_barrier();
    }
#undef MBX5_READBACK
#undef MBX5_ISSUE_B
#undef MBX5_ISSUE_A
#undef MBX5_ISSUE
#undef MBX5_SETUP_TILE
  } else {
  constexpr int WN = G::WN;
  const int wn = wave % WN, wm = wave / WN;
  const int frow = lane & 15, fch = lane >> 4;
  const int fr0 = frow * 8 + (fch ^ (frow & 7));
  const int fr1 = frow * 8 + ((4 + fch) ^ (frow & 7));
  const int fwrow = 8 * (frow >> 2) + (frow & 3), fwkey = ((frow >> 2) << 1) | ((frow >> 1) & 1);
  const int fw0 = fwrow * 8 + (fch ^ fwkey);
  const int fw1 = fwrow * 8 + ((4 + fch) ^ fwkey);
  int st_comp = 0;
  const bool fetcher = queued && tid == 0;
  auto fetch_raw = [&]() -> int { return atomicAdd(p.work_counter, 1); };
  auto tile_of = [&](const int raw) -> int { const int v = (int)gridDim.x + raw; return v < ntiles ? v : ntiles; };
  int raw1 = 0;
  if (fetcher) { s_ids[0] = first; raw1 = fetch_raw(); }
  raw_barrier();
  if (fetcher) s_ids[1] = tile_of(raw1);
  int jt = 0;
  for (int t = first; t < ntiles; t = queued ? s_ids[++jt & 3] : t + (int)gridDim.x) {
    const int tile_n = t % p.tiles_n, tile_m = t / p.tiles_n;
    const int m0 = tile_m * BM, n0 = tile_n * BN;
#ifdef MBX_I5_STAMPS
    const int tnum = (t - first) / (int)gridDim.x;
    const bool stamp = p.stamps && tid == 0 && tnum < 8 && blockIdx.x < 64;
#define MBX5_STAMP(i) do { if (stamp) p.stamps[(blockIdx.x * 8 + tnum) * 4 + (i)] = wall_clock64(); } while (0)
#else
#define MBX5_STAMP(i) do { } while (0)
#endif
    MBX5_STAMP(0);
#ifdef MBX_I5_STAMPS
    const unsigned long long cyc0 = __builtin_amdgcn_s_memtime();
#endif
    constexpr int NA = NI / 2;
    constexpr int EVC = EV == 7 ? 2 : EV, BMODE = EV == 7 ? 2 : EV == 2 ? 0 : 1;
    constexpr int PRE_RAW = (EV == 4 && G::BM * G::BN >= 256 * 128) ? 1
                            : (EV == 4 || EVC == 2 || EV == 6) ? 4 / (NA * (EVC == 2 ? 2 : 1)) : 0;
    constexpr int PREB = PRE_RAW > MI ? MI : PRE_RAW;
    const int cl0 = wn * TN + fch * 8, mlane = m0 + wm * TM + frow, clane = n0 + cl0;
    u32x4 pla[PREB > 0 ? PREB : 1][NA], plb[PREB > 0 ? PREB : 1][NA];
    if constexpr (PREB > 0) conv_epilogue_issue_reads<EVC, false, NA, PREB, BMODE>(p, mlane, clane, 0, pla, plb);
    int raw2 = 0;
    if (fetcher) raw2 = fetch_raw();
    f32x4 acc[NI][MI];
#pragma unroll
    for (int a = 0; a < NI; ++a)
#pragma unroll
      for (int b = 0; b < MI; ++b) acc[a][b] = f32x4{0.f, 0.f, 0.f, 0.f};
    for (int it = 0; it < nk; ++it) {
#ifdef MBX_I5_STAMPS
      if (p.dbg & 1) { st_comp = st_comp == NST - 1 ? 0 : st_comp + 1; raw_barrier(); continue; }
#endif
      const u32x4* cP = smem + st_comp * STAGE + (wm * TM) * 8;
      const u32x4* cW = smem + st_comp * STAGE + BM * 8 + (wn * TN) * 8;
#pragma unroll
      for (int kk = 0; kk < 2; ++kk) {
        const int fr = kk ? fr1 : fr0, fw = kk ? fw1 : fw0;
        bf16x8 wf[NI], pf[MI];
#pragma unroll
        for (int a = 0; a < NI; ++a) wf[a] = __builtin_bit_cast(bf16x8, cW[(a >> 1) * 256 + (a & 1) * 32 + fw]);
#pragma unroll
        for (int b = 0; b < MI; ++b) pf[b] = __builtin_bit_cast(bf16x8, cP[b * 128 + fr]);
#pragma unroll
        for (int a = 0; a < NI; ++a)
#pragma unroll
          for (int b = 0; b < MI; ++b)
            acc[a][b] = __builtin_amdgcn_mfma_f32_16x16x32_bf16(wf[a], pf[b], acc[a][b], 0, 0, 0);
      }
      st_comp = st_comp == NST - 1 ? 0 : st_comp + 1;
      asm volatile("s_waitcnt lgkmcnt(0)" ::: "memory");
      raw_barrier();
    }
    MBX5_STAMP(1);
#ifdef MBX_I5_STAMPS
    if (stamp) p.stamps[(blockIdx.x * 8 + tnum) * 4 + 3] = __builtin_amdgcn_s_memtime() - cyc0;
#endif
    if (fetcher) s_ids[(jt + 2) & 3] = tile_of(raw2);
    float s1[NA][8], s2[NA][8], sc[NA][8], sh[NA][8];
    conv_epilogue_channels<EVC, NA>(p, clane, sc, sh, s1, s2);
    if constexpr (PREB > 0) {
      conv_epilogue_finish<EVC, false, NI, MI, PREB, BMODE>(p, acc, mlane, clane, 0, pla, plb, sh, sc, s1, s2);
      asm volatile("" ::: "memory");
    }
    if constexpr (PREB < MI) {
      constexpr int REM = MI - PREB, CH = (EV == 0 || EV == 1 || EV == 3) ? REM : (REM % 2 == 0 ? 2 : 1);
      conv_epilogue_range<EVC, false, NI, MI, PREB, MI, CH, BMODE>(p, acc, mlane, clane, sh, sc, s1, s2);
    }
    MBX5_STAMP(2);
    if constexpr (EV == 1 || EV == 6) {
#pragma unroll
      for (int A = 0; A < NA; ++A) { row_sum16_x8(s1[A]); row_sum16_x8(s2[A]); }
#pragma unroll
      for (int A = 0; A < NA; ++A)
#pragma unroll
        for (int j = 0; j < 8; ++j) {
          const float x1 = s1[A][j], x2 = s2[A][j];
          if (frow == 0) {
            red[(wm * BN + cl0 + 32 * A + j) * 2] = x1;
            red[(wm * BN + cl0 + 32 * A + j) * 2 + 1] = x2;
          }
        }
      lds_barrier();
      if (tid < BN && n0 + tid < p.C_out) {
        float x1 = 0.f, x2 = 0.f;
#pragma unroll
        for (int w = 0; w < G::WM; ++w) { x1 += red[(w * BN + tid) * 2]; x2 += red[(w * BN + tid) * 2 + 1]; }
        if constexpr (EV == 6) bw_stats_write(p, tile_m, n0 + tid, x1, x2); else stats_write(p, tile_m, n0 + tid, x1, x2);
      }
    }
#undef MBX5_STAMP
  }
  }
  if constexpr (EV == 1) {
    if (fused_tail) {
      constexpr int NT = 512 + 64 * NLW;
      fused_apply_tail<NT>(p, smem, [&](auto&& fn) {
        for (int t = first; t < ntiles; t += (int)gridDim.x) fn((t / p.tiles_n) * BM, BM, (t % p.tiles_n) * BN, BN);
      });
    }
  }
  if constexpr (EV == 0 && !(MY == 2 && NW == 3)) {
    if (fused_tail) {
      constexpr int NT = 512 + 64 * NLW;
      static_assert(NT * 68 + sizeof(FbShared) <= G::RING_BYTES, "the tail's reduce area fits the ring");
      static_assert(BM * BN <= 8 * kFbChunk * NT, "a lane's share of a tile is one chunk");
      fused_bwd_tail<NT, true>(p, smem, [&](auto&& fn) {
        for (int t = first; t < ntiles; t += (int)gridDim.x) fn((t / p.tiles_n) * BM, BM, (t % p.tiles_n) * BN, BN);
      });
    }
  }
}


template <int MY, int NW>
int launch5(ConvK& k, hipStream_t s) {
  using G = Ig5<MY, NW>;
  k.tiles_m = (k.M + G::BM - 1) / G::BM;
  k.tiles_n = (k.C_out + G::BN - 1) / G::BN;
  k.stats_cap = stats_cap_for(k.tiles_m);
  const int ntiles = k.tiles_m * k.tiles_n;
  const int ncu = conv_cus();
  int grid = ntiles < ncu ? ntiles : ncu;
  if (k.max_wg > 0 && grid > k.max_wg) grid = k.max_wg;
  const int ev = k.epi == MBX_EPI_RESIDUAL ? 4 : k.epi == MBX_EPI_AFFINE ? 3 : k.bw_n ? 6 : k.stats ? 1 : k.bits ? 7 : (k.accumulate || k.skip) ? 2 : 0;
  constexpr bool kNo6 = (MY == 4 && NW == 2) || NW >= 3;
  constexpr bool kNo2 = NW == 3;
  if ((ev == 6 && kNo6) || ((ev == 2 || ev == 7) && kNo2)) return MBX_ERR_UNSUPPORTED;
  if (k.fb.bar && (ev != 0 || (MY == 2 && NW == 3))) return MBX_ERR_UNSUPPORTED;
  if (k.fa.bar && ev != 1) return MBX_ERR_UNSUPPORTED;
  if (k.dry) return MBX_OK;
  static bool attr[8][2] = {};
#define MBX5_LAUNCH(EV, MODE)                                                                                 \
  do {                                                                                                        \
    if (!attr[EV][MODE]) {                                                                                    \
      (void)hipFuncSetAttribute(reinterpret_cast<const void*>(conv_igemm5_kernel<MY, NW, EV, MODE>),          \
                                hipFuncAttributeMaxDynamicSharedMemorySize, G::LDS_BYTES);                    \
      attr[EV][MODE] = true;                                                                                  \
    }                                                                                                         \
    hipLaunchKernelGGL((conv_igemm5_kernel<MY, NW, EV, MODE>), dim3(grid), dim3(1024), G::LDS_BYTES, s, k);   \
  } while (0)
#define MBX5_EV(EV) case EV: if (k.pw) MBX5_LAUNCH(EV, 1); else MBX5_LAUNCH(EV, 0); break;
  switch (ev) {
    MBX5_EV(0) MBX5_EV(1) MBX5_EV(3) MBX5_EV(4)
    case 2:
      if constexpr (!kNo2) { if (k.pw) MBX5_LAUNCH(2, 1); else MBX5_LAUNCH(2, 0); }
      break;
    case 6:
      if constexpr (!kNo6) { if (k.pw) MBX5_LAUNCH(6, 1); else MBX5_LAUNCH(6, 0); }
      break;
    case 7:
      if constexpr (!kNo2) { if (k.pw) MBX5_LAUNCH(7, 1); else MBX5_LAUNCH(7, 0); }
      break;
  }
#undef MBX5_EV
#undef MBX5_LAUNCH
  MBX_LAUNCH_CHECK();
  return MBX_OK;
}

}

extern const int mbx_i5_tiles[][2] = {{128, 64}, {128, 128}, {192, 128}, {256, 128}, {256, 64}, {128, 192}, {128, 256}};
extern const int mbx_i5_num_tiles = 7;

int mbx_launch_igemm5(ConvK& k, int index, hipStream_t s) {
  if (k.shift || k.epi == MBX_EPI_STORE_F32) return MBX_ERR_UNSUPPORTED;
  switch (index) {
    case 0: return launch5<2, 1>(k, s);
    case 1: return launch5<2, 2>(k, s);
    case 2: return launch5<3, 2>(k, s);
    case 3: return launch5<4, 2>(k, s);
    case 4: return launch5<4, 1>(k, s);
    case 5: return launch5<2, 3>(k, s);
    case 6: return launch5<2, 4>(k, s);
    default: return MBX_ERR_UNSUPPORTED;
  }
}
```

### multibox_amd/csrc/conv_common.h

```cpp
#pragma once
#include "common.h"
#include "grid_barrier.h"

namespace mbx {

struct ConvK {
  const unsigned short* x; int x_img_stride, ldx, H_in, W_in, C_in;
  const unsigned short* w; int C_out, R, S, Ktot;
  unsigned x_bytes, w_bytes;
  unsigned y_bytes, skip_bytes, acc_bytes;
  int mul, shift, pad_t, pad_l, W_out, HW_out, M;
  void* y; int y_img_stride, ldy;
  int epi, relu, accumulate;
  const float* scale; const float* shiftv;
  const unsigned short* skip; int skip_img_stride, ld_skip; float rscale;
  const unsigned short* acc_src; int acc_img_stride, ld_acc;
  unsigned char* bits; int bits_ld; unsigned bits_bytes;
  float* stats;
  float stats_cap;
  int stats_mod, stats_ld;
  int bw_n, bw_mod;
  int bw_cb[4], bw_ldy[4], bw_sld[4];
  const unsigned short* bw_y[4];
  const float* bw_thr[4];
  float* bw_stats[4];
  FusedApply fa;
  FusedBwd fb;
  int tiles_m, tiles_n;
  unsigned mg_hw, sh_hw, mg_w, sh_w;
  int pw;
  int cls_m0[4], cls_hw[4], cls_w[4];
  int skip_taps;
  int parity;
  int* work_counter;
  int max_wg;
  int dry;
  int ksplit, kps; long long y_split_stride;
#ifdef MBX_I5_STAMPS
  unsigned long long* stamps;
  int dbg;
  int stagger;
#endif
};

}

int mbx_launch_igemm5(mbx::ConvK& k, int index, hipStream_t s);
extern const int mbx_i5_tiles[][2];
extern const int mbx_i5_num_tiles;
int mbx_launch_igemm7(mbx::ConvK& k, hipStream_t s);
int mbx_launch_direct3(mbx::ConvK& k, int N, int H_out, hipStream_t s);
int mbx_direct3_grid(int N, int H_out, int W_out);
int mbx_launch_directw(mbx::ConvK& k, int N, int H_out, hipStream_t s);
int mbx_directw_grid(int N, int H_out, int W_out);
int mbx_launch_resident(mbx::ConvK& k, int N, int H_out, hipStream_t s);
int mbx_resident_rows(int N);
int mbx_launch_pwres(mbx::ConvK& k, hipStream_t s);

namespace {

using mbx::ConvK;
using mbx::FusedApply;
using mbx::FusedBwd;

typedef __attribute__((ext_vector_type(8))) __bf16 bf16x8;
typedef __attribute__((ext_vector_type(4))) float f32x4;
typedef __attribute__((ext_vector_type(4))) short s16x4;
typedef __attribute__((ext_vector_type(4))) unsigned int u32x4;
typedef __attribute__((ext_vector_type(2))) unsigned int u32x2;

__device__ __forceinline__ float bf2f(unsigned short h) { return __uint_as_float(((unsigned)h) << 16); }
__device__ __forceinline__ unsigned short f2bf(float f) { return __builtin_bit_cast(unsigned short, (__bf16)f); }
typedef float f32x4u __attribute__((ext_vector_type(4), aligned(4)));
__device__ __forceinline__ unsigned pack2bf(float lo, float hi) {
  typedef float pk_f32x2 __attribute__((ext_vector_type(2)));
  typedef __bf16 pk_bf16x2 __attribute__((ext_vector_type(2)));
  return __builtin_bit_cast(unsigned, __builtin_convertvector(pk_f32x2{lo, hi}, pk_bf16x2));
}
__device__ __forceinline__ float bf_lo(unsigned w) { return __uint_as_float(w << 16); }
__device__ __forceinline__ float bf_hi(unsigned w) { return __uint_as_float(w & 0xffff0000u); }
__device__ __forceinline__ unsigned gather4_rows(unsigned b) {
  typedef unsigned g4_u32x2 __attribute__((ext_vector_type(2)));
  const g4_u32x2 r = __builtin_amdgcn_permlane16_swap(b, b, false, false);
  const unsigned t = r.x | (r.y << 8);
  const g4_u32x2 q = __builtin_amdgcn_permlane32_swap(t, t, false, false);
  return q.x | (q.y << 16);
}
__device__ __forceinline__ float relu_f(float x) {
  float r;
  asm("v_max_f32 %0, 0, %1" : "=v"(r) : "v"(x));
  return r;
}

constexpr int kThreads = 256;

inline int conv_cus() { const int n = mbx_cu_count(); return n ? n : 256; }

inline void set_magic(unsigned d, unsigned& mg, unsigned& sh) {
  unsigned l = 0;
  while ((1ull << l) < d) ++l;
  sh = 31 + l;
  mg = (unsigned)((1ull << sh) / d + 1);
}

inline int check_desc(const mbx_conv_desc* d) {
  if (!d || !d->x || !d->N || d->N < 0) return MBX_ERR_INVALID_ARG;
  if (d->C_in <= 0 || d->C_in % 8 || d->ldx % 8 || d->ldx < d->C_in) return MBX_ERR_INVALID_ARG;
  if (d->R <= 0 || d->S <= 0 || d->C_out <= 0 || d->H_out <= 0 || d->W_out <= 0) return MBX_ERR_INVALID_ARG;
  if (d->stride != 1 && d->stride != 2) return MBX_ERR_UNSUPPORTED;
  if ((reinterpret_cast<uintptr_t>(d->x) & 15)) return MBX_ERR_INVALID_ARG;
  const long long xe = (long long)d->N * d->x_img_stride;
  if (xe >= (1LL << 30) || (long long)d->N * d->H_out * d->W_out >= (1LL << 31)) return MBX_ERR_UNSUPPORTED;
  return MBX_OK;
}

__device__ __forceinline__ float row_sum16(float v) {
  asm volatile("s_nop 1\n\t"
               "v_add_f32_dpp %0, %0, %0 row_ror:8 row_mask:0xf bank_mask:0xf\n\t"
               "s_nop 1\n\t"
               "v_add_f32_dpp %0, %0, %0 row_ror:4 row_mask:0xf bank_mask:0xf\n\t"
               "s_nop 1\n\t"
               "v_add_f32_dpp %0, %0, %0 row_ror:2 row_mask:0xf bank_mask:0xf\n\t"
               "s_nop 1\n\t"
               "v_add_f32_dpp %0, %0, %0 row_ror:1 row_mask:0xf bank_mask:0xf"
               : "+v"(v));
  return v;
}
__device__ __forceinline__ void row_sum16_x8(float (&v)[8]) {
#define MBX_RS_STEP(R)                                                                                                     \
  "v_add_f32_dpp %0, %0, %0 row_ror:" #R " row_mask:0xf bank_mask:0xf\n\tv_add_f32_dpp %1, %1, %1 row_ror:" #R " row_mask:0xf bank_mask:0xf\n\t" \
  "v_add_f32_dpp %2, %2, %2 row_ror:" #R " row_mask:0xf bank_mask:0xf\n\tv_add_f32_dpp %3, %3, %3 row_ror:" #R " row_mask:0xf bank_mask:0xf\n\t" \
  "v_add_f32_dpp %4, %4, %4 row_ror:" #R " row_mask:0xf bank_mask:0xf\n\tv_add_f32_dpp %5, %5, %5 row_ror:" #R " row_mask:0xf bank_mask:0xf\n\t" \
  "v_add_f32_dpp %6, %6, %6 row_ror:" #R " row_mask:0xf bank_mask:0xf\n\tv_add_f32_dpp %7, %7, %7 row_ror:" #R " row_mask:0xf bank_mask:0xf\n\t"
  asm volatile("s_nop 1\n\t" MBX_RS_STEP(8) MBX_RS_STEP(4) MBX_RS_STEP(2) MBX_RS_STEP(1)
               : "+v"(v[0]), "+v"(v[1]), "+v"(v[2]), "+v"(v[3]), "+v"(v[4]), "+v"(v[5]), "+v"(v[6]), "+v"(v[7]));
#undef MBX_RS_STEP
}
__device__ __forceinline__ unsigned fast_div(unsigned m, unsigned magic, unsigned shift) {
  return (unsigned)(((unsigned long long)m * magic) >> shift);
}
constexpr float kStatsFix = 1048576.f;
constexpr float kStatsTotal = 4398046511104.f;
__host__ __device__ __forceinline__ float stats_cap_for(long long adders) { return kStatsTotal / (float)(adders > 0 ? adders : 1); }
__device__ __forceinline__ void stats_add_fixed(unsigned long long* o, const float x1, const float x2, const float cap) {
  if (__builtin_fabsf(x1) < cap && __builtin_fabsf(x2) < cap) {
    atomicAdd(o, (unsigned long long)__float2ll_rn(x1 * kStatsFix));
    atomicAdd(o + 1, (unsigned long long)__float2ll_rn(x2 * kStatsFix));
  } else {
    atomicMin(reinterpret_cast<long long*>(o + 1), (long long)0x8000000000000000ull);
  }
}
__device__ __forceinline__ void stats_write(const ConvK& p, const int tile_row, const int ch, const float x1, const float x2) {
  if (p.stats_mod) {
    unsigned long long* o = reinterpret_cast<unsigned long long*>(p.stats) + ((size_t)(tile_row % p.stats_mod) * p.stats_ld + ch) * 2;
    stats_add_fixed(o, x1, x2, p.stats_cap);
  } else {
    float* o = p.stats + ((size_t)tile_row * p.stats_ld + ch) * 2;
    o[0] = x1;
    o[1] = x2;
  }
}
__device__ __forceinline__ int bw_seg(const ConvK& p, const int c) {
  int s = 0;
#pragma unroll
  for (int i = 1; i < 4; ++i) if (i < p.bw_n && c >= p.bw_cb[i]) s = i;
  return s;
}
__device__ __forceinline__ void bw_stats_write(const ConvK& p, const int tile_row, const int ch, const float x1, const float x2) {
  const int s = bw_seg(p, ch);
  float* o = p.bw_stats[s] + ((size_t)(tile_row % p.bw_mod) * p.bw_sld[s] + (ch - p.bw_cb[s])) * 2;
  unsafeAtomicAdd(o, x1);
  unsafeAtomicAdd(o + 1, x2);
}
__device__ __forceinline__ void decode_pixel(const ConvK& p, unsigned m, int& img, int& oh, int& ow) {
  img = (int)fast_div(m, p.mg_hw, p.sh_hw);
  const int rem = (int)m - img * p.HW_out;
  oh = (int)fast_div((unsigned)rem, p.mg_w, p.sh_w);
  ow = rem - oh * p.W_out;
}
__device__ __forceinline__ void decode_pixel_parity(const ConvK& p, unsigned m, int& img, int& oh, int& ow) {
  const int c = ((int)m >= p.cls_m0[1]) + ((int)m >= p.cls_m0[2]) + ((int)m >= p.cls_m0[3]);
  const int m0 = c == 0 ? p.cls_m0[0] : c == 1 ? p.cls_m0[1] : c == 2 ? p.cls_m0[2] : p.cls_m0[3];
  const int hw = c == 0 ? p.cls_hw[0] : c == 1 ? p.cls_hw[1] : c == 2 ? p.cls_hw[2] : p.cls_hw[3];
  const int wc = c == 0 ? p.cls_w[0] : c == 1 ? p.cls_w[1] : c == 2 ? p.cls_w[2] : p.cls_w[3];
  unsigned r = m - (unsigned)m0;
  img = (int)(r / (unsigned)hw);
  r -= (unsigned)img * (unsigned)hw;
  const int a = (int)(r / (unsigned)wc), b = (int)r - a * wc;
  oh = 2 * a + (c >> 1);
  ow = 2 * b + (c & 1);
}
__device__ __forceinline__ int pixel_class(const ConvK& p, int m) {
  return (m >= p.cls_m0[1]) + (m >= p.cls_m0[2]) + (m >= p.cls_m0[3]);
}
constexpr unsigned kOOB = 0x80000000u;

__device__ __forceinline__ __amdgpu_buffer_rsrc_t make_rsrc(const void* p, unsigned bytes) {
  return __builtin_amdgcn_make_buffer_rsrc(const_cast<void*>(p), (short)0, (int)bytes, 0x00020000);
}
__device__ __forceinline__ u32x4 buf_load16(__amdgpu_buffer_rsrc_t r, unsigned byte_off) {
  return __builtin_amdgcn_raw_buffer_load_b128(r, (int)byte_off, 0, 0);
}

__device__ __forceinline__ int xcd_remap(int bid, int nblk) {
  const int xcd = bid & 7, q = nblk >> 3, r = nblk & 7;
  return (xcd < r ? xcd * (q + 1) : r * (q + 1) + (xcd - r) * q) + (bid >> 3);
}

__device__ __forceinline__ void glds16(__amdgpu_buffer_rsrc_t r, u32x4* lds_dst, int off) {
  __builtin_amdgcn_raw_ptr_buffer_load_lds(r, (__attribute__((address_space(3))) void*)lds_dst, 16, off, 0, 0, 0);
}
__device__ __forceinline__ int wave_id() { return __builtin_amdgcn_readfirstlane(threadIdx.x >> 6); }
__device__ __forceinline__ void raw_barrier() {
#ifndef MBX_UNFENCED_BARRIER
  asm volatile("" ::: "memory");
#endif
  __builtin_amdgcn_s_barrier();
#ifndef MBX_UNFENCED_BARRIER
  asm volatile("" ::: "memory");
#endif
}
__device__ __forceinline__ void lds_barrier() {
  asm volatile("s_waitcnt lgkmcnt(0)" ::: "memory");
  __builtin_amdgcn_s_barrier();
  asm volatile("" ::: "memory");
}

#ifdef MBX_NO_LANDING_PROBE
#define MBX_NO_PROBE_I3 1
#define MBX_NO_PROBE_I5 1
#define MBX_NO_PROBE_WG 1
#endif

template <int N>
__device__ __forceinline__ void wait_vmcnt() { asm volatile("s_waitcnt vmcnt(%0)" ::"n"(N) : "memory"); }

__device__ __forceinline__ unsigned lds_readback_issue(const void* lds_slot) {
  unsigned v;
  const unsigned long long a = reinterpret_cast<unsigned long long>(lds_slot) - 12ull * (threadIdx.x & 63);
  asm volatile("flat_load_dword %0, %1" : "=v"(v) : "v"(a) : "memory");
  return v;
}
__device__ __forceinline__ void lds_readback_wait(unsigned v) { asm volatile("s_waitcnt lgkmcnt(0)" ::"v"(v) : "memory"); }

template <bool SH>
__device__ __forceinline__ void epi_pixel(const ConvK& p, const int m, int& img, int& pix) {
  const unsigned mm = m < p.M ? (unsigned)m : 0u;
  if (SH && p.parity) {
    int oh_, ow_;
    decode_pixel_parity(p, mm, img, oh_, ow_);
    pix = oh_ * p.W_out + ow_;
  } else {
    img = (int)fast_div(mm, p.mg_hw, p.sh_hw);
    pix = (int)mm - img * p.HW_out;
  }
}

template <int EV, bool SH, int NA, int BCH, int BMODE = 1>
__device__ __forceinline__ void conv_epilogue_issue_reads(const ConvK& p, const int mlane, const int clane, const int b0,
                                                          u32x4 (&la)[BCH][NA], u32x4 (&lb)[BCH][NA]) {
  if constexpr (EV == 6) {
#pragma unroll
    for (int A = 0; A < NA; ++A) {
      const int c0 = clane + 32 * A;
      const int sg = bw_seg(p, c0 < p.C_out ? c0 : 0);
      const unsigned short* yb = p.bw_y[sg] + (c0 < p.C_out ? c0 - p.bw_cb[sg] : 0);
      const long long ld = p.bw_ldy[sg];
#pragma unroll
      for (int bb = 0; bb < BCH; ++bb) {
        const int m = mlane + (b0 + bb) * 16;
        la[bb][A] = *reinterpret_cast<const u32x4*>(yb + ((m < p.M && c0 < p.C_out) ? m * ld : 0ll));
      }
    }
  }
  if constexpr (EV == 2 || EV == 4) {
    const __amdgpu_buffer_rsrc_t kr_ = make_rsrc(p.skip, p.skip ? p.skip_bytes : 0u);
    const __amdgpu_buffer_rsrc_t ar = make_rsrc(p.acc_src, p.acc_bytes);
    const bool do_acc = EV == 2 && p.accumulate, do_mask = EV == 2 && BMODE != 2 && p.skip != nullptr;
    const bool do_bits = EV == 2 && (BMODE == 2 || (BMODE == 1 && p.bits != nullptr));
    const __amdgpu_buffer_rsrc_t br = make_rsrc(p.bits, p.bits ? p.bits_bytes : 0u);
#pragma unroll
    for (int bb = 0; bb < BCH; ++bb) {
      const int m = mlane + (b0 + bb) * 16;
      int img, pix;
      epi_pixel<SH>(p, m, img, pix);
#pragma unroll
      for (int A = 0; A < NA; ++A) {
        const int c0 = clane + 32 * A;
        const bool ok = m < p.M && c0 < p.C_out;
        const unsigned so = ok ? (unsigned)((img * p.skip_img_stride + pix * p.ld_skip + c0) * 2) : kOOB;
        if constexpr (EV == 4) {
          la[bb][A] = buf_load16(kr_, so);
        } else {
          const unsigned ao = ok ? (unsigned)((img * p.acc_img_stride + pix * p.ld_acc + c0) * 2) : kOOB;
          if (do_acc) la[bb][A] = buf_load16(ar, ao);
          if (do_mask) lb[bb][A] = buf_load16(kr_, so);
          if (do_bits) lb[bb][A].x = __builtin_amdgcn_raw_buffer_load_b8(br, ok ? m * p.bits_ld + (c0 >> 3) : (int)kOOB, 0, 0);
        }
      }
    }
  }
}

template <int EV, bool SH, int NI, int MI, int BCH, int BMODE = 1>
__device__ __forceinline__ void conv_epilogue_finish(const ConvK& p, const f32x4 (&acc)[NI][MI], const int mlane, const int clane,
                                                     const int b0, const u32x4 (&la)[BCH][NI / 2], const u32x4 (&lb)[BCH][NI / 2],
                                                     const float (&sh)[NI / 2][8], const float (&sc)[NI / 2][8],
                                                     float (&s1)[NI / 2][8], float (&s2)[NI / 2][8]) {
  constexpr int NA = NI / 2;
  const __amdgpu_buffer_rsrc_t yr = make_rsrc(p.y, p.y_bytes);
  const bool do_acc = EV == 2 && p.accumulate, do_mask = EV == 2 && BMODE != 2 && p.skip != nullptr;
  const bool do_bits = (EV == 2 && BMODE == 2) || ((EV == 2 || EV == 4) && BMODE == 1 && p.bits != nullptr);
  const __amdgpu_buffer_rsrc_t br = make_rsrc(p.bits, p.bits ? p.bits_bytes : 0u);
  const int fch_ = (threadIdx.x >> 4) & 3;
#pragma unroll
  for (int bb = 0; bb < BCH; ++bb) {
    const int b = b0 + bb;
    const int m = mlane + b * 16;
    int img, pix;
    epi_pixel<SH>(p, m, img, pix);
    unsigned bits_dw = 0;
#pragma unroll
    for (int A = 0; A < NA; ++A) {
      const int c0 = clane + 32 * A;
      const unsigned yo = (m < p.M && c0 < p.C_out) ? (unsigned)((img * p.y_img_stride + pix * p.ldy + c0) * 2) : kOOB;
      float v[8] = {acc[2 * A][b][0], acc[2 * A][b][1], acc[2 * A][b][2], acc[2 * A][b][3],
                    acc[2 * A + 1][b][0], acc[2 * A + 1][b][1], acc[2 * A + 1][b][2], acc[2 * A + 1][b][3]};
      if constexpr (EV == 3) {
#pragma unroll
        for (int j = 0; j < 8; ++j) v[j] = v[j] * sc[A][j] + sh[A][j];
      } else if constexpr (EV == 4) {
        const unsigned w[4] = {la[bb][A].x, la[bb][A].y, la[bb][A].z, la[bb][A].w};
#pragma unroll
        for (int j = 0; j < 4; ++j) {
          v[2 * j] = bf2f(w[j] & 0xffffu) + p.rscale * (v[2 * j] + sh[A][2 * j]);
          v[2 * j + 1] = bf2f(w[j] >> 16) + p.rscale * (v[2 * j + 1] + sh[A][2 * j + 1]);
        }
      } else if constexpr (EV == 2) {
#pragma clang fp contract(off)
        const float rs = p.rscale != 0.f ? p.rscale : 1.f;
#pragma unroll
        for (int j = 0; j < 8; ++j) v[j] *= rs;
      } else {
        const float rs = p.rscale != 0.f ? p.rscale : 1.f;
#pragma unroll
        for (int j = 0; j < 8; ++j) v[j] *= rs;
      }
      if constexpr (EV == 2) {
        if (do_acc) {
          const unsigned w[4] = {la[bb][A].x, la[bb][A].y, la[bb][A].z, la[bb][A].w};
#pragma unroll
          for (int j = 0; j < 4; ++j) { v[2 * j] += bf2f(w[j] & 0xffffu); v[2 * j + 1] += bf2f(w[j] >> 16); }
        }
        if (do_mask) {
          const unsigned w[4] = {lb[bb][A].x, lb[bb][A].y, lb[bb][A].z, lb[bb][A].w};
#pragma unroll
          for (int j = 0; j < 4; ++j) {
            if (!(bf2f(w[j] & 0xffffu) > 0.f)) v[2 * j] = 0.f;
            if (!(bf2f(w[j] >> 16) > 0.f)) v[2 * j + 1] = 0.f;
          }
        }
      }
      if constexpr (EV == 3 || EV == 4) {
        if (p.relu) {
#pragma unroll
          for (int j = 0; j < 8; ++j) v[j] = relu_f(v[j]);
        }
      }
      unsigned q4[4];
#pragma unroll
      for (int j = 0; j < 4; ++j) q4[j] = pack2bf(v[2 * j], v[2 * j + 1]);
      if constexpr (EV == 2) {
        if (do_bits) {
          const int byte = (int)lb[bb][A].x;
#pragma unroll
          for (int j = 0; j < 4; ++j)
            q4[j] &= ((unsigned)__builtin_amdgcn_sbfe(byte, 2 * j, 1) & 0xffffu) | ((unsigned)__builtin_amdgcn_sbfe(byte, 2 * j + 1, 1) << 16);
        }
      }
      __builtin_amdgcn_raw_buffer_store_b128(u32x4{q4[0], q4[1], q4[2], q4[3]}, yr, (int)yo, 0, 0);
      if constexpr (EV == 4) {
        if (do_bits) {
          unsigned sidx = 0;
#pragma unroll
          for (int j = 0; j < 4; ++j) {
            unsigned h;
            asm("v_pk_min_u16 %0, %1, %2" : "=v"(h) : "v"(q4[j] & 0x7fff7fffu), "s"(0x00010001u));
            sidx |= h << (2 * j);
          }
          const unsigned byte = (sidx | (sidx >> 15)) & 0xffu;
          const unsigned dw = gather4_rows(byte);
          if (A == 0 || fch_ == A) bits_dw = dw;
        }
      }
      if constexpr (EV == 1) {
#pragma unroll
        for (int j = 0; j < 8; ++j) { const float f = (j & 1) ? bf_hi(q4[j >> 1]) : bf_lo(q4[j >> 1]); s1[A][j] += f; s2[A][j] += f * f; }
      }
      if constexpr (EV == 6) {
        const unsigned w[4] = {la[bb][A].x, la[bb][A].y, la[bb][A].z, la[bb][A].w};
#pragma unroll
        for (int j = 0; j < 8; ++j) {
          const float yv = bf2f((unsigned short)((j & 1) ? (w[j >> 1] >> 16) : (w[j >> 1] & 0xffffu)));
          const float g = yv > sh[A][j] ? ((j & 1) ? bf_hi(q4[j >> 1]) : bf_lo(q4[j >> 1])) : 0.f;
          s1[A][j] += g;
          s2[A][j] += g * yv;
        }
      }
    }
    if constexpr (EV == 4) {
      if (do_bits) {
        const int cw = clane - 8 * fch_ + 32 * fch_;
        __builtin_amdgcn_raw_buffer_store_b32(bits_dw, br, (fch_ < NA && m < p.M && cw < p.C_out) ? m * p.bits_ld + (cw >> 3) : (int)kOOB, 0, 0);
      }
    }
  }
}

template <int EV, int NA>
__device__ __forceinline__ void conv_epilogue_channels(const ConvK& p, const int clane, float (&sc)[NA][8], float (&sh)[NA][8],
                                                       float (&s1)[NA][8], float (&s2)[NA][8]) {
#pragma unroll
  for (int A = 0; A < NA; ++A)
#pragma unroll
    for (int j = 0; j < 8; ++j) { sc[A][j] = 1.f; sh[A][j] = 0.f; s1[A][j] = 0.f; s2[A][j] = 0.f; }
  if constexpr (EV == 6) {
#pragma unroll
    for (int A = 0; A < NA; ++A) {
      const int c0 = clane + 32 * A;
      if (c0 < p.C_out) {
        const int sg = bw_seg(p, c0);
        const float* t = p.bw_thr[sg] + (c0 - p.bw_cb[sg]);
#pragma unroll
        for (int j = 0; j < 8; ++j) sh[A][j] = t[j];
      }
    }
  }
  if constexpr (EV == 3 || EV == 4) {
#pragma unroll
    for (int A = 0; A < NA; ++A) {
      const int c0 = clane + 32 * A;
      if (c0 < p.C_out) {
        if (p.scale) {
          const f32x4u u0 = *reinterpret_cast<const f32x4u*>(p.scale + c0), u1 = *reinterpret_cast<const f32x4u*>(p.scale + c0 + 4);
          sc[A][0] = u0.x; sc[A][1] = u0.y; sc[A][2] = u0.z; sc[A][3] = u0.w; sc[A][4] = u1.x; sc[A][5] = u1.y; sc[A][6] = u1.z; sc[A][7] = u1.w;
        }
        if (p.shiftv) {
          const f32x4u u0 = *reinterpret_cast<const f32x4u*>(p.shiftv + c0), u1 = *reinterpret_cast<const f32x4u*>(p.shiftv + c0 + 4);
          sh[A][0] = u0.x; sh[A][1] = u0.y; sh[A][2] = u0.z; sh[A][3] = u0.w; sh[A][4] = u1.x; sh[A][5] = u1.y; sh[A][6] = u1.z; sh[A][7] = u1.w;
        }
      }
    }
  }
}

template <int EV, bool SH, int NI, int MI, int B0, int B1, int BCH, int BMODE = 1>
__device__ __forceinline__ void conv_epilogue_range(const ConvK& p, const f32x4 (&acc)[NI][MI], const int mlane, const int clane,
                                                    const float (&sh)[NI / 2][8], const float (&sc)[NI / 2][8],
                                                    float (&s1)[NI / 2][8], float (&s2)[NI / 2][8]) {
  static_assert((B1 - B0) % BCH == 0 && B0 >= 0 && B1 <= MI, "chunks");
  constexpr int NA = NI / 2;
#pragma unroll
  for (int b0 = B0; b0 < B1; b0 += BCH) {
    u32x4 la[BCH][NA], lb[BCH][NA];
    conv_epilogue_issue_reads<EV, SH, NA, BCH, BMODE>(p, mlane, clane, b0, la, lb);
    conv_epilogue_finish<EV, SH, NI, MI, BCH, BMODE>(p, acc, mlane, clane, b0, la, lb, sh, sc, s1, s2);
    if (b0 + BCH < B1) asm volatile("" ::: "memory");
  }
}

template <int EV, bool SH, int NI, int MI, int BCH = MI>
__device__ __forceinline__ void conv_epilogue_direct(const ConvK& p, const f32x4 (&acc)[NI][MI], const int mlane, const int clane,
                                                     float (&s1)[NI / 2][8], float (&s2)[NI / 2][8]) {
  static_assert(NI % 2 == 0 && EV != 5 && MI % BCH == 0, "wave tile: a multiple of 32 output channels; float32 heads are handled by the caller");
  constexpr int NA = NI / 2;
  float sc[NA][8], sh[NA][8];
  conv_epilogue_channels<EV, NA>(p, clane, sc, sh, s1, s2);
  conv_epilogue_range<EV, SH, NI, MI, 0, MI, BCH>(p, acc, mlane, clane, sh, sc, s1, s2);
}

}

#include "fused_bn.h"
```

### multibox_amd/engine.py

```python
from __future__ import annotations

import ctypes as C
import math
import os
import re

import numpy as np
import torch

from . import _lib, ops
from .ops import View

BN_EPS = 0.001
STATS_ROWS = int(os.environ.get("MBX_STATS_ROWS", "8"))
WEIGHT_DECAY = 0.00004


def _same_pad(n, k, s):
    out = -(-n // s)
    total = max((out - 1) * s + k - n, 0)
    return out, total // 2


def _valid(n, k, s):
# ... 395 lines not shown
    def pool(self, kind, x, out, ksz, stride, pad=0, scope=None):
        op = PoolOp(self, kind, x, out, ksz, stride, pad)
        op.scope = scope
        self.fwd.append(op)

    def _finalize(self, seed):
        dev = self.dev
        w_off = bt_off = 0
        self.param_index = {}
        for op in self.convs:
            op.w_off = w_off
            ktot = op.R * op.S * op.Cin
            row = 0
            for m in op.members:
                real_c = 3 if op.x is self.images else m.Cin
                self.param_index[m.scope + "/weights"] = ("W", w_off + row * ktot, (m.K, m.R, m.S, real_c), m.Cin)
                row += m.K
            w_off += op.K * ktot
            w_off = (w_off + 7) // 8 * 8
            if op.kind == "residual":
                op.b_off = w_off
                self.param_index[op.members[0].scope + "/biases"] = ("W", w_off, (op.K,), None)
                w_off += (op.K + 7) // 8 * 8
            if op.kind in ("bn", "frozen"):
                op.beta_off = bt_off
                ch = 0
                for m in op.members:
                    self.param_index[m.scope + "/BatchNorm/beta"] = ("Bt", bt_off + ch, (m.K,), None)
                    self.param_index[m.scope + "/BatchNorm/moving_mean"] = ("MM", bt_off + ch, (m.K,), None)
                    self.param_index[m.scope + "/BatchNorm/moving_variance"] = ("MV", bt_off + ch, (m.K,), None)
                    ch += m.K
                bt_off += (op.K + 7) // 8 * 8
        self.nW, self.nBt = w_off, bt_off
        first_head = next(op for op in self.convs if op.is_head)
        self.head_w_start, self.head_bt_start = first_head.w_off, first_head.beta_off
        f32 = dict(dtype=torch.float32, device=dev)
        self.W = torch.zeros(self.nW, **f32)
        self.Wb = torch.zeros(self.nW, dtype=torch.bfloat16, device=dev)
        self.Bt = torch.zeros(self.nBt, **f32)
        self.MM = torch.zeros(self.nBt, **f32)
        self.MV = torch.ones(self.nBt, **f32)
        self.bn_mean = torch.zeros(self.nBt, **f32)
        self.bn_var = torch.zeros(self.nBt, **f32)
        self.bn_rstd = torch.ones(self.nBt, **f32)
        self.bn_scale = torch.ones(self.nBt, **f32)
        self.bn_shift = torch.zeros(self.nBt, **f32)
        self.init_weights(seed)
        if self.mode == "train":
            self.G_off = (self.nBt + 8 + 63) // 64 * 64
            assert self.G_off % 8 == 0
            self.G = torch.zeros(self.G_off + self.nW, **f32)
            self.Btg = self.G[:self.nBt + 8]
            self.Wg = self.G[self.G_off:]
            self.step_ctl = self.Btg[self.nBt:self.nBt + 8]
        self._alloc_scratch()
        self._build_backward()
        if torch.device(self.dev).type == "cuda":
            self.prepare_filters()
            if os.environ.get("MBX_TUNE_SAVE"):
                ops.save_tune_cache()

    def init_weights(self, seed):
        gen = torch.Generator().manual_seed(seed)
        W = torch.zeros(self.nW, dtype=torch.float32)
        for name, (buf, off, shape, cpad) in self.param_index.items():
            if buf == "W" and name.endswith("/weights"):
                K, R, S_, Cc = shape
                lim = math.sqrt(6.0 / (R * S_ * Cc + R * S_ * K))
                n = K * R * S_ * Cc
                v = ((torch.rand(n, generator=gen) * 2 - 1) * lim).reshape(shape)
                W[off:off + K * R * S_ * cpad].reshape(K, R, S_, cpad)[..., :Cc] = v
        self.W.copy_(W)
        self.Wb.copy_(self.W.to(torch.bfloat16))

    def get_param(self, name, kind="value"):
        buf, off, shape, cpad = self.param_index[name]
        t = {"W": self.W, "Bt": self.Bt, "MM": self.MM, "MV": self.MV}[buf] if kind == "value" else \
            {"W": self.Wg, "Bt": self.Btg}[buf]
        if cpad is not None and cpad != shape[-1]:
            K, R, S_, Cc = shape
            return t[off:off + K * R * S_ * cpad].reshape(K, R, S_, cpad)[..., :Cc]
        n = int(np.prod(shape))
        return t[off:off + n].reshape(shape)

    def set_param(self, name, value):
        self.get_param(name).copy_(torch.as_tensor(value, dtype=torch.float32).reshape(self.get_param(name).shape))

    def refresh_bf16(self):
        self.Wb.copy_(self.W.to(torch.bfloat16))
        self.prepare_filters()

    def _alloc_scratch(self):
        dev = self.dev
        max_stats = max_bwd = n_stats16 = 0
        l = _lib.lib()
        for members in self._bn_group_requests:
            idx = [self.fwd.index(m) for m in members]
            ok = all(m.kind == "bn" and m.M == members[0].M and m.relu == members[0].relu and m.trainable == members[0].trainable and
                     m.out.buf is members[0].out.buf and m.out.ld == members[0].out.ld and m.K % 8 == 0 for m in members)
            ok = ok and idx == list(range(idx[0], idx[0] + len(idx))) and len(members) <= 4
            ok = ok and all(b.beta_off == a.beta_off + a.K for a, b in zip(members, members[1:]))
            g = BnUnit(members)
            ok = ok and g.K <= 2048 and g.chan_map([m.out for m in members])[0] >= 0
            if ok:
                self.bn_groups.append(g)
                for m in members:
                    m.group = m.unit = g
        for op in self.convs:
            if op.kind == "bn":
                u = op.unit = op.unit or BnUnit([op])
                i = u.members.index(op)
                N_, H_, W_ = op.out.N, op.out.H, op.out.W
                if op is u.lead:
                    u.y = torch.empty((op.M, u.K), dtype=torch.bfloat16, device=dev)
                    self._bufs.append(u.y)
                    u.stats16_base = n_stats16
                    n_stats16 += STATS_ROWS * u.K * 4
                op.y_view = View(u.y, N_, H_, W_, op.K, u.K, u.koff[i])
                op.stats16_off = u.stats16_base + 4 * u.koff[i]
                d = self._desc(op, op.y_view)
                rows = max(ops.conv_stats_rows(d), (op.M + 63) // 64)
                if len(u.members) == 1 and ops.splitk_slices(d, self.n_cus):
                    rows = max(rows, (op.M + 15) // 16)
                op.stats_off = u.stats_off[i] = 0 if i == 0 else u.stats_end
                u.stats_end = op.stats_off + rows * op.K * 2
                max_stats = max(max_stats, u.stats_end)
                if op.trainable:
                    if op is u.lead:
                        u.dy = torch.empty((op.M, u.K), dtype=torch.bfloat16, device=dev)
                        self._bufs.append(u.dy)
                        max_bwd = max(max_bwd, l.mbx_bn_bwd_rows(op.M, u.K) * u.K * 2,
                                      l.mbx_bn_bwd_rows_pooled(N_, H_, W_, u.K) * u.K * 2)
                    op.dy_view = View(u.dy, N_, H_, W_, op.K, u.K, u.koff[i])
        ws_floats = 0
        for op in self.convs:
            op.bn_ws_off = -1
            if op.kind != "bn":
                continue
            u = op.unit
            if op is not u.lead:
                op.bn_ws_off = u.lead.bn_ws_off
            elif op.trainable and torch.device(dev).type == "cuda" and l.mbx_bn_bwd_onepass_supported(op.M, u.K, self.chain_cap or self.bn_max_wg):
                op.bn_ws_off = ws_floats
                ws_floats += (l.mbx_bn_bwd_onepass_workspace_bytes(u.K) // 4 + 7) // 8 * 8
        self._plan_bw_stats()
        for op in self.convs:
            op.bw_rows_off = -1
            u = op.bw_unit
            if u is not None:
                if op is u.lead:
                    op.bw_rows_off = ws_floats
                    ws_floats += STATS_ROWS * u.K * 2
                else:
                    op.bw_rows_off = u.lead.bw_rows_off
        self._plan_fused_bwd()
        for op in self.convs:
            op.fb_acc_off = op.fb_bar_off = -1
        for op in self.convs:
            u = op.fb_unit
            if u is not None and op is u.lead:
                ws_floats = (ws_floats + 31) // 32 * 32
                op.fb_acc_off = ws_floats
                ws_floats += ops.BN_BWD_SLOTS * 2 * u.K
            if op.fb_segments is not None:
                ws_floats = (ws_floats + 31) // 32 * 32
                op.fb_bar_off = ws_floats
                ws_floats += ops.GRID_BARRIER_BYTES // 4
        ws_floats = (ws_floats + 31) // 32 * 32
        self.bn_ws = torch.zeros(max(ws_floats, 8), dtype=torch.float32, device=dev)
        assert self.bn_ws.data_ptr() % 128 == 0 or torch.device(dev).type != "cuda"
        n_ctr = self.i5_counters.numel()
        n_stats16 = (max(n_stats16, 4) + 31) // 32 * 32
        self._n_fwd_barriers = sum(1 for op in self.convs if op.kind == "bn") if self.fuse_apply else 0
        self._fwd_barriers_used = 0
        bar_words = ops.GRID_BARRIER_BYTES // 4
        self._fwd_clear = torch.zeros(n_ctr + n_stats16 + self._n_fwd_barriers * bar_words + 32, dtype=torch.int32, device=dev)
        self.i5_counters = self._fwd_clear[:n_ctr]
        self.stats16 = self._fwd_clear[n_ctr:n_ctr + n_stats16].view(torch.float32)
        b0 = n_ctr + n_stats16
        b0 += (-(self._fwd_clear.data_ptr() // 4 + b0)) % 32
        self._fwd_barrier_base = self._fwd_clear.data_ptr() + 4 * b0
        self.bn_thr = torch.zeros(max(self.nBt, 8), dtype=torch.float32, device=dev)
        self.bn_timeouts_total = torch.zeros((), dtype=torch.int64, device=dev)
        self.stats_scratch = torch.zeros(max(max_stats, 2), dtype=torch.float32, device=dev)
        self.bwd_scratch = torch.zeros(max(max_bwd, 2), dtype=torch.float32, device=dev)
        self.m12 = torch.zeros(2 * 2048, dtype=torch.float32, device=dev)
        self.reg_loss = torch.zeros(1, dtype=torch.float32, device=dev)

    def _plan_bw_stats(self):
        for op in self.convs:
            op.bw_unit, op.bw_segments = None, None
        if not self.bw_stats or torch.device(self.dev).type != "cuda":
            return

        def consumer_ok(X):
            dd = dgrad_probe(X)
            return not (ops.direct3_applies(dd) or ops.directw_applies(dd) or ops.resident_applies(dd))

        units, segs = plan_consumer_fusion(self.convs, self.fwd, lambda u: True, consumer_ok, align=32)
        for u in units:
            for m in u.members:
                m.bw_unit = u
        for X, sg in segs.items():
            X.bw_segments = sg

    def _plan_fused_bwd(self):
        for op in self.convs:
            op.fb_unit, op.fb_segments = None, None
        if not self.fuse_bwd:
            return
        pairs_ok = os.environ.get("MBX_FUSE_BWD_PAIRS", "1") != "0"
        only = re.compile(os.environ["MBX_FUSE_BWD_ONLY"]) if os.environ.get("MBX_FUSE_BWD_ONLY") else None
        max_rounds = int(os.environ.get("MBX_FUSE_BWD_MAX_ROUNDS", "1"))

        def consumer_ok(X):
            if X.x.img_stride != X.x.H * X.x.W * X.x.ld or X.Cin % 8 or (only is not None and not only.search(X.name)):
                return False
            if not pairs_ok and X.kind == "bn" and len(X.unit.members) == 2:
                return False
            dd = dgrad_probe(X)
            if ops.direct3_applies(dd):
                return False
            return ops.fused_tail_rounds(dd, self.n_cus) <= max_rounds

        units, segs = plan_consumer_fusion(self.convs, self.fwd, lambda u: all(m.fused_pool is None for m in u.members),
                                           consumer_ok, align=8)
        for u in units:
            for m in u.members:
                m.fb_unit = u
        for X, sg in segs.items():
            X.fb_segments = sg

    def _fb_table(self, X):
        t = ops.BnBwdFused()
        t.barrier = self.bn_ws.data_ptr() + 4 * X.fb_bar_off
        t.n = len(X.fb_segments)
        t.step_poison = self.step_ctl.data_ptr()
        for i, (c_rel, m, c_in, n) in enumerate(X.fb_segments):
            u = m.unit
            ko = m.y_view.ch_off
            assert m.y_view.ld == u.K and m.dy_view.ld == u.K and u.lead.fb_acc_off >= 0
            t.c_begin[i] = c_rel
            t.y[i], t.ld_y[i] = m.y_view.buf.data_ptr() + 2 * (ko + c_in), u.K
            t.dy[i], t.ld_dy[i] = m.dy_view.buf.data_ptr() + 2 * (ko + c_in), u.K
            t.mean[i] = self.bn_mean.data_ptr() + 4 * (m.beta_off + c_in)
            t.rstd[i] = self.bn_rstd.data_ptr() + 4 * (m.beta_off + c_in)
            t.beta[i] = self.Bt.data_ptr() + 4 * (m.beta_off + c_in)
            t.dbeta[i] = self.Btg.data_ptr() + 4 * (m.beta_off + c_in)
            t.acc[i], t.acc_ld[i] = self.bn_ws.data_ptr() + 4 * (u.lead.fb_acc_off + ko + c_in), u.K
            t.relu[i] = int(m.relu)
        self._keep.append(t)
        return t

    def _bw_table(self, X):
        t = _lib.BnBwdStats()
        t.n, t.rows_mod = len(X.bw_segments), STATS_ROWS
        for i, (c_rel, m, c_in, n) in enumerate(X.bw_segments):
            u = m.unit
            ko = m.y_view.ch_off
            t.c_begin[i] = c_rel
            t.y[i], t.ld_y[i] = m.y_view.buf.data_ptr() + 2 * (ko + c_in), u.K
            t.relu_thr[i] = self.bn_thr.data_ptr() + 4 * (m.beta_off + c_in)
            t.stats[i], t.stats_ld[i] = self.bn_ws.data_ptr() + 4 * (u.lead.bw_rows_off + 2 * (ko + c_in)), u.K
        self._keep.append(t)
        return t

    def _w(self, op):
        return self.Wb[op.w_off:]

    def _desc(self, op, y: View, **kw):
        return ops.make_desc(op.x, self._w(op), op.K, op.R, op.S, op.stride, op.pad_t, op.pad_l, y, **kw)

    def _sl(self, t, off, n):
        return t[off:off + n]

    def _tune(self, op, d, what):
        key = (what, op.x.N, op.x.H, op.x.W, op.x.C, op.K, op.R, op.S, op.stride, op.pad_t, op.pad_l, d.C_out, d.C_in,
               d.epilogue, bool(d.stats_partial), d.accumulate, bool(d.skip) or (bool(d.relu_bits) and d.epilogue == ops.EPI_STORE), d.relu)
        if d.relu_bits and d.epilogue == ops.EPI_RESIDUAL:
            key = key + ("bits",)
        self.tune_registry.append((repr(key), d, what))
        if self.autotune:
            ops.autotune(d, key)
            over = ops._TUNED.get(repr(key) + "#norule") if os.environ.get("MBX_NO_RULE_EXCEPTIONS") != "1" else None
            if over is not None:
                keep = d.tile_config
                d.tile_config = int(over)
                if _lib.lib().mbx_conv_supported(C.byref(d)) != 0:
                    d.tile_config, over = keep, None
            if os.environ.get("MBX_NO_I5") == "1" and d.tile_config > ops.I5_FLAG:
                d.tile_config = ops._TUNED.get(repr(key) + "#i3", 0)
            if d.tile_config > ops.I5_FLAG and os.environ.get("MBX_I5_STATIC") != "1":
                n = ops.I7_COUNTERS if d.tile_config == ops.I7_TILE_CONFIG else 1
                assert self._i5_used + n <= self.i5_counters.numel()
                d.work_counter = self.i5_counters.data_ptr() + 4 * self._i5_used
                self._i5_used += n
            if os.environ.get("MBX_NO_2STAGE") == "1":
                d.tile_config = {9: 7, 10: 2, 11: 5, 12: 2, 13: 8, 14: 1}.get(d.tile_config, d.tile_config)
            pair = (what == "fwd" and bool(d.stats_partial) and op.group is not None and len(op.group.members) == 2
                    and os.environ.get("MBX_CONV_PAIR", "1") != "0")
            rule = ops.launch_rule(d, pair) if over is None else None
            if rule is not None:
                d.tile_config, d.work_counter = rule[0], None
                _lib.check(_lib.lib().mbx_conv_supported(C.byref(d)), rule[1] + " " + op.name)
        return d

    def _build_forward_launches(self):
        L = []
        l = _lib.lib()
        st = lambda: torch.cuda.current_stream().cuda_stream
        for op in self.fwd:
            if isinstance(op, PoolOp):
                if not op.fused_fwd:
                    L.append(op.forward)
                continue
            if op.kind == "bn":
                L.append(self._bn_forward(op))
            elif op.kind == "frozen":
                d = self._tune(op, self._desc(op, op.out, epilogue=ops.EPI_AFFINE, relu=op.relu,
                                              scale=self._sl(self.bn_scale, op.beta_off, op.K),
                                              shift=self._sl(self.bn_shift, op.beta_off, op.K)), "fwd")
                L.append(lambda d=d, op=op: _lib.check(l.mbx_conv(C.byref(d), st()), op.name))
            elif op.kind == "residual":
                d = self._tune(op, self._desc(op, op.out, epilogue=ops.EPI_RESIDUAL, relu=op.relu,
                                              shift=self._sl(self.W, op.b_off, op.K), skip=op.skip, rscale=op.rscale,
                                              relu_bits=op.relu_bits), "fwd")
                L.append(lambda d=d, op=op: _lib.check(l.mbx_conv(C.byref(d), st()), op.name))
            elif op.kind == "head":
                d = self._desc(op, op.out, epilogue=ops.EPI_STORE_F32)
                L.append(lambda d=d, op=op: _lib.check(l.mbx_conv(C.byref(d), st()), op.name))
                if op is self.heads[-1]:
                    L.append(lambda: _lib.check(l.mbx_head_gather_all(self.head_table, len(self.heads), self.B, self.P,
                                                                      self.locs.data_ptr(), self.logits.data_ptr(), st()), "head_gather_all"))
        return L

    def _bn_forward(self, op):
        l = _lib.lib()
        st = lambda: torch.cuda.current_stream().cuda_stream
        cuda = torch.device(self.dev).type == "cuda"
        u = op.unit
        i, n, single = u.members.index(op), len(u.members), len(u.members) == 1
        fpool = op.fused_pool
        use16 = self.atomic_stats and fpool is None
        if use16:
            d = self._desc(op, op.y_view, stats=self.stats16[op.stats16_off:], stats_rows_mod=STATS_ROWS, stats_ld=0 if single else u.K)
        else:
            d = self._desc(op, op.y_view, stats=self.stats_scratch[op.stats_off:])
        d = self._tune(op, d, "fwd")
        S_ = ops.splitk_slices(d, self.n_cus) if single and cuda else 0
        if S_:
            d.tile_config = ops.SPLITK_FLAG + S_
            need = int(l.mbx_conv_splitk_workspace_bytes(C.byref(d)))
            ws = torch.empty(need // 4, dtype=torch.float32, device=self.dev)
            self._keep.append(ws)
            d.splitk_ws, d.splitk_ws_bytes = ws.data_ptr(), ws.numel() * 4
            _lib.check(l.mbx_conv_supported(C.byref(d)), "split-K " + op.name)
        rows = u.rows[i] = ops.conv_stats_rows(d)
        assert use16 or i + 1 == n or rows * op.K * 2 <= u.stats_off[i + 1] - u.stats_off[i]
        u.fwd_desc[i] = d
        if i + 1 < n:
            return lambda: None if u.pair_fwd else _lib.check(l.mbx_conv(C.byref(d), st()), op.name)
        if n == 2 and cuda and os.environ.get("MBX_CONV_PAIR", "1") != "0":
            u.pair_fwd = l.mbx_conv_pair(C.byref(u.fwd_desc[0]), C.byref(d), st()) == 0
        K, M, out = u.K, op.M, op.out
        mean, rstd, mm, mv, var, beta, thr = (self._sl(t, u.lead.beta_off, K) for t in
                                              (self.bn_mean, self.bn_rstd, self.MM, self.MV, self.bn_var, self.Bt, self.bn_thr))
        s16 = self.stats16[u.stats16_base:]
        a_ptr, a_ld, amap = u.target([m.out for m in u.members])
        amap = None if amap is None else C.byref(amap)
        parts = (C.c_void_p * n)(*[self.stats_scratch.data_ptr() + 4 * o for o in u.stats_off])
        rows_a, cs_a = (C.c_int32 * n)(*u.rows), (C.c_int32 * n)(*[m.K for m in u.members])
        if fpool is not None:
            fpool.fused_fwd = True
        fd = ba = None
        if single and use16 and self.fuse_apply and not S_ and cuda and out.img_stride == out.H * out.W * out.ld \
                and (not os.environ.get("MBX_FUSE_APPLY_ONLY") or re.search(os.environ["MBX_FUSE_APPLY_ONLY"], op.name)):
            ba = ops.BnApplyDesc()
            ba.barrier = self._fwd_barrier_base + ops.GRID_BARRIER_BYTES * self._fwd_barriers_used
            ba.a, ba.ld_a, ba.beta, ba.mean, ba.rstd = out.ptr, out.ld, beta.data_ptr(), mean.data_ptr(), rstd.data_ptr()
            ba.relu_thr, ba.relu, ba.eps, ba.step_poison = thr.data_ptr(), int(op.relu), BN_EPS, self.step_ctl.data_ptr()
            fd = ops.ConvDesc.from_buffer_copy(d)
            fd.bn_apply = C.addressof(ba)
            fd.work_counter = None
            if l.mbx_conv_supported(C.byref(fd)) == 0:
                assert self._fwd_barriers_used < self._n_fwd_barriers
                self._fwd_barriers_used += 1
                self.fused_apply_launches += 1
            else:
                fd = ba = None

        def run():
            s = st()
            mm_, mv_, decay = (None, var, -1.0) if self.defer_moving else (mm, mv, self.bn_decay)
            if fd is not None and not self.no_onepass:
                ba.moving_mean, ba.moving_var, ba.decay = ops._p(mm_), ops._p(mv_), decay
                fd.max_workgroups = self.cu_cap or self.bn_max_wg
                _lib.check(l.mbx_conv(C.byref(fd), s), op.name + " + bn apply")
                return
            if u.pair_fwd:
                _lib.check(l.mbx_conv_pair(C.byref(u.fwd_desc[0]), C.byref(d), s), "pair " + op.name)
            else:
                _lib.check(l.mbx_conv(C.byref(d), s), op.name)
            totals = (mean.data_ptr(), rstd.data_ptr(), ops._p(mm_), ops._p(mv_))
            if use16:
                _lib.check(l.mbx_bn_apply_fused_mapped(s16.data_ptr(), STATS_ROWS, M, BN_EPS, decay, u.y.data_ptr(), M, K,
                                                       beta.data_ptr(), int(op.relu), a_ptr, a_ld, amap, *totals,
                                                       thr.data_ptr(), s), "bn_apply_fused_mapped")
            elif not single:
                _lib.check(l.mbx_bn_finalize_parts(parts, rows_a, cs_a, n, M, BN_EPS, decay, *totals, s), "bn_finalize_parts")
                _lib.check(l.mbx_bn_apply_mapped(u.y.data_ptr(), M, K, mean.data_ptr(), rstd.data_ptr(), beta.data_ptr(),
                                                 int(op.relu), a_ptr, a_ld, amap, s), "bn_apply_mapped")
            elif fpool is not None:
                po = fpool.out
                _lib.check(l.mbx_bn_finalize(self.stats_scratch.data_ptr(), rows, K, M, BN_EPS, decay, *totals, s), "bn_finalize")
                _lib.check(l.mbx_bn_apply_maxpool(u.y.data_ptr(), out.N, out.H, out.W, K, mean.data_ptr(), rstd.data_ptr(),
                                                  beta.data_ptr(), int(op.relu), po.ptr, po.img_stride, po.ld, po.H, po.W,
                                                  fpool.argmax.data_ptr(), s), "bn_apply_maxpool")
            elif self._probe_skip_apply and ("/block" in op.name or "/Block8" in op.name):
                _lib.check(l.mbx_bn_finalize(self.stats_scratch.data_ptr(), rows, K, M, BN_EPS, decay, *totals, s), "fin")
            else:
                _lib.check(l.mbx_bn_apply_fused(self.stats_scratch.data_ptr(), rows, M, BN_EPS, decay, u.y.data_ptr(), M, K,
                                                beta.data_ptr(), int(op.relu), a_ptr, a_ld, *totals, s), "bn_apply_fused")
        return run

    def _gview(self, v: View) -> View:
        return self.grad_of(v)

    def _claim(self, g: View):
        key = (id(g.buf), g.ch_off, g.C)
        if key in self.written:
            return 1, None
        self.written.add(key)
        src = self.pending_acc.pop(key, None)
        return (1, src) if src is not None else (0, None)

    def _make_head_table(self):
        arr = (_lib.Head * len(self.heads))()
        for j, op in enumerate(self.heads):
            cells, kk, off = op.head
            if self.mode == "train":
                op.head_grad = View(torch.zeros((op.M, self.head_ld), dtype=torch.bfloat16, device=self.dev),
                                    op.out.N, op.out.H, op.out.W, self.head_ld)
                self._bufs.append(op.head_grad.buf)
            arr[j].h, arr[j].ld_h = op.out.buf.data_ptr(), self.head_ld
            arr[j].g, arr[j].ld_g = (op.head_grad.buf.data_ptr() if op.head_grad is not None else None), self.head_ld
            arr[j].cells, arr[j].k, arr[j].off = cells, kk, off
        self.head_table = arr

    def _build_backward(self):
        self._make_head_table()
        if self.mode != "train":
            self.fwd_launches = self._build_forward_launches()
            self.bwd_launches = []
            self.bwd_jobs = []
            return
        l = _lib.lib()
        st = lambda: torch.cuda.current_stream().cuda_stream
        entries, d_off, blocks = [], 0, 0
        for op in self.convs:
            if op.need_dx:
                kpad = (op.K + 7) // 8 * 8
                e = _lib.FilterEntry(op.w_off, d_off, op.K, op.R, op.S, op.Cin, kpad, blocks)
                op.dgrad_off, op.kpad = d_off, kpad
                n = op.Cin * op.R * op.S * kpad
                d_off += (n + 7) // 8 * 8
                blocks += op.R * op.S * ((op.Cin + 31) // 32) * ((kpad + 63) // 64)
                entries.append(e)
        self.Wd = torch.zeros(max(d_off, 8), dtype=torch.bfloat16, device=self.dev)
        arr = (_lib.FilterEntry * len(entries))(*entries)
        raw = np.frombuffer(C.string_at(C.addressof(arr), C.sizeof(arr)), dtype=np.uint8).copy()
        self.filter_table = torch.from_numpy(raw).to(self.dev)
        self.filter_blocks, self.filter_entries = blocks, len(entries)

        mask_of = {}
        fused_mask = set()
        for r in self.convs:
            if r.kind == "residual" and r.relu and r.trainable:
                for c in self.fwd:
                    if isinstance(c, ConvOp) and c.x.buf is r.out.buf:
                        if c.need_dx and c.x.ch_off == r.out.ch_off and c.x.C == r.out.C:
                            mask_of[id(c)] = r
                            fused_mask.add(id(r))
                        break
                    if isinstance(c, PoolOp) and c.x.buf is r.out.buf:
                        break
        self.pending_acc = {}
        L = []
        self.bwd_ops = []
        self.bwd_jobs = []
        for op in reversed(self.fwd):
            if isinstance(op, PoolOp):
                if op.needs_backward():
                    prod = self._pool_producer(op)
                    if prod is not None:
                        prod.fused_pool = op
                        continue
                    gx = self._gview(op.x)
                    acc, src = self._claim(gx)
                    assert src is None, "a pooling layer cannot be the first writer of a residual block's input gradient"
                    L.append(op.make_backward(self._gview(op.out), gx, acc))
                    self.bwd_ops.append(op)
                    self.bwd_jobs.append(None)
                continue
            if not op.trainable:
                continue
            K, M = op.K, op.M
            dw = self._sl(self.Wg, op.w_off, K * op.R * op.S * op.Cin)
            if op.kind == "head":
                cells, kk, off = op.head
                g = op.head_grad
                dyv, scale, db = g, 1.0, None
                pre = None
                if op is self.heads[-1]:
                    pre = lambda s: _lib.check(l.mbx_head_scatter_all(self.d_locs.data_ptr(), self.d_logits.data_ptr(), self.head_table,
                                                                      len(self.heads), self.B, self.P, s), "head_scatter_all")
            elif op.kind == "residual":
                gout = self._gview(op.out)
                gs = self._gview(op.skip)
                self.pending_acc[(id(gs.buf), gs.ch_off, gs.C)] = gout
                zb = id(self.grad_of(op.x).buf)
                self.written = {k for k in self.written if k[0] != zb}
                dyv, scale, db = gout, op.rscale, self._sl(self.Wg, op.b_off, K)
                if op.relu and id(op) not in fused_mask:
                    pre = lambda s, gout=gout, op=op: _lib.check(
                        l.mbx_relu_mask(gout.ptr, gout.ld, op.out.ptr, op.out.ld, op.M, op.K, s), "relu_mask")
                else:
                    pre = None
            else:
                dyv, scale, db = op.dy_view, 1.0, None
                pre = self._bn_backward(op)
            ddesc = fdesc = None
            if op.need_dx:
                gx = self._gview(op.x)
                acc, acc_src = self._claim(gx)
                dyin = View(dyv.buf, dyv.N, dyv.H, dyv.W, op.kpad, dyv.ld, dyv.ch_off, 2)
                mr = mask_of.get(id(op))
                ddesc = ops.make_desc(dyin, self.Wd[op.dgrad_off:], op.Cin, op.R, op.S, op.stride,
                                      op.R - 1 - op.pad_t, op.S - 1 - op.pad_l, gx, transposed=1, accumulate=acc,
                                      rscale=(scale if scale != 1.0 else 0.0), skip=(mr.out if mr is not None else None),
                                      acc_src=acc_src)
                if mr is not None and self.relu_bits and op.Cin % 8 == 0:
                    bits = torch.zeros((op.x.N * op.x.H * op.x.W, (op.Cin + 31) // 32 * 4), dtype=torch.uint8, device=self.dev)
                    alt = ops.make_desc(dyin, self.Wd[op.dgrad_off:], op.Cin, op.R, op.S, op.stride,
                                        op.R - 1 - op.pad_t, op.S - 1 - op.pad_l, gx, transposed=1, accumulate=acc,
                                        rscale=(scale if scale != 1.0 else 0.0), acc_src=acc_src, relu_bits=bits)
                    if torch.device(self.dev).type != "cuda" or l.mbx_conv_supported(C.byref(alt)) == 0:
                        ddesc, mr.relu_bits = alt, bits
                self._tune(op, ddesc, "dgrad")
                if op.fb_segments is not None:
                    assert acc == 0 and acc_src is None and mr is None, op.name
                    fdesc = ops.ConvDesc.from_buffer_copy(ddesc)
                    fdesc.bn_bwd = C.addressof(self._fb_table(op))
                    fdesc.work_counter = None
                    if not (ops.I5_FLAG < fdesc.tile_config <= ops.I5_FLAG + 7 or fdesc.tile_config in (ops.DIRECTW_TILE_CONFIG, ops.RESIDENT_TILE_CONFIG)):
                        fdesc.tile_config = ops.i5_tile_for(op.x.M, op.Cin, self.n_cus)
                    if l.mbx_conv_supported(C.byref(fdesc)) != 0:
                        fdesc.tile_config = ops.i5_tile_for(op.x.M, op.Cin, self.n_cus)
                    _lib.check(l.mbx_conv_supported(C.byref(fdesc)), "data gradient + BN backward " + op.name)
                    self.fused_bwd_launches += 1
                if op.bw_segments is not None:
                    assert acc == 0 and acc_src is None and mr is None, op.name
                    ddesc.bn_bwd_stats = C.addressof(self._bw_table(op))
                    if l.mbx_conv_supported(C.byref(ddesc)) != 0:
                        for alt in (ops.I5_TILE_CONFIGS[2], ops.I5_TILE_CONFIGS[1], 0):
                            ddesc.tile_config = alt
                            if alt == 0:
                                ddesc.work_counter = None
                            if l.mbx_conv_supported(C.byref(ddesc)) == 0:
                                break
                        _lib.check(l.mbx_conv_supported(C.byref(ddesc)), "statistics epilogue " + op.name)

            job = ops.WgradJob()
            job.desc = ops.make_desc(op.x, None, K, op.R, op.S, op.stride, op.pad_t, op.pad_l,
                                     View(dyv.buf, op.out.N, op.out.H, op.out.W, 8, dyv.ld, dyv.ch_off, 2))
            job.desc.C_out = K
            job.dy, job.dy_img_stride, job.ld_dy = dyv.ptr, dyv.img_stride, dyv.ld
            job.scale = float(scale)
            job.dw, job.db = dw.data_ptr(), (None if db is None else db.data_ptr())

            grp = op.group
            if grp is not None and ddesc is not None:
                grp.dgrad_desc[grp.members.index(op)] = ddesc

            op.fdesc = fdesc

            def run(op=op, pre=pre, ddesc=ddesc, grp=grp, fdesc=fdesc):
                s = st()
                if pre is not None and not (op.kind == "bn" and self._probe_skip_bn_bwd):
                    pre(s)
                if fdesc is not None and not self.no_onepass:
                    fdesc.max_workgroups = self.cu_cap or self.bn_max_wg
                    _lib.check(l.mbx_conv(C.byref(fdesc), s), "dgrad + bn backward " + op.name)
                    return
                if ddesc is not None:
                    if grp is not None and grp.pair_bwd:
                        if op is grp.members[-1]:
                            _lib.check(l.mbx_conv_pair(C.byref(ddesc), C.byref(grp.dgrad_desc[0]), s), "dgrad pair " + op.name)
                        return
                    ddesc.max_workgroups = self.cu_cap
                    _lib.check(l.mbx_conv(C.byref(ddesc), s), "dgrad " + op.name)
            L.append(run)
            self.bwd_ops.append(op)
            self.bwd_jobs.append(job)
        if torch.device(self.dev).type == "cuda" and os.environ.get("MBX_CONV_PAIR", "1") != "0":
            for grp in self.bn_groups:
                if len(grp.members) == 2 and len(grp.dgrad_desc) == 2 and not any(m.fdesc is not None for m in grp.members):
# ... 231 lines not shown
```

### multibox_amd/ops.py

```python
from __future__ import annotations

import ctypes as C
import os

import torch

from . import _lib

EPI_STORE, EPI_AFFINE, EPI_RESIDUAL, EPI_STORE_F32 = 0, 1, 2, 3


class ConvDesc(C.Structure):
    _fields_ = [
        ("x", C.c_void_p), ("x_img_stride", C.c_int64), ("ldx", C.c_int32),
        ("N", C.c_int32), ("H_in", C.c_int32), ("W_in", C.c_int32), ("C_in", C.c_int32),
        ("w", C.c_void_p), ("C_out", C.c_int32), ("R", C.c_int32), ("S", C.c_int32),
        ("stride", C.c_int32), ("transposed", C.c_int32), ("pad_t", C.c_int32), ("pad_l", C.c_int32),
        ("H_out", C.c_int32), ("W_out", C.c_int32),
        ("y", C.c_void_p), ("y_img_stride", C.c_int64), ("ldy", C.c_int32),
        ("epilogue", C.c_int32), ("relu", C.c_int32), ("accumulate", C.c_int32),
        ("scale", C.c_void_p), ("shift", C.c_void_p),
        ("skip", C.c_void_p), ("skip_img_stride", C.c_int64), ("ld_skip", C.c_int32), ("rscale", C.c_float),
        ("stats_partial", C.c_void_p),
        ("tile_config", C.c_int32),
        ("acc_src", C.c_void_p), ("acc_img_stride", C.c_int64), ("ld_acc", C.c_int32),
        ("work_counter", C.c_void_p),
        ("max_workgroups", C.c_int32),
        ("splitk_ws", C.c_void_p), ("splitk_ws_bytes", C.c_int64),
        ("stats_rows_mod", C.c_int32), ("stats_ld", C.c_int32),
        ("bn_bwd_stats", C.c_void_p),
        ("relu_bits", C.c_void_p), ("ld_bits", C.c_int32),
        ("bn_apply", C.c_void_p),
        ("bn_bwd", C.c_void_p),
    ]


class BnApplyDesc(C.Structure):
    _fields_ = [("barrier", C.c_void_p), ("a", C.c_void_p), ("ld_a", C.c_int32), ("beta", C.c_void_p), ("mean", C.c_void_p),
                ("rstd", C.c_void_p), ("moving_mean", C.c_void_p), ("moving_var", C.c_void_p), ("relu_thr", C.c_void_p),
                ("relu", C.c_int32), ("eps", C.c_float), ("decay", C.c_float), ("step_poison", C.c_void_p)]


class BnBwdFused(C.Structure):
    _fields_ = [("barrier", C.c_void_p), ("n", C.c_int32), ("c_begin", C.c_int32 * 4), ("y", C.c_void_p * 4), ("ld_y", C.c_int32 * 4),
                ("dy", C.c_void_p * 4), ("ld_dy", C.c_int32 * 4), ("mean", C.c_void_p * 4), ("rstd", C.c_void_p * 4),
                ("beta", C.c_void_p * 4), ("dbeta", C.c_void_p * 4), ("acc", C.c_void_p * 4), ("acc_ld", C.c_int32 * 4),
                ("relu", C.c_int32 * 4), ("step_poison", C.c_void_p)]


GRID_BARRIER_BYTES = 6400
BN_BWD_SLOTS = 8


def i5_tile_for(M, C_out, n_cus=256):
    best, best_key = None, None
    for i, (bm, bn) in enumerate(I5_TILES):
        if (bm, bn) == (128, 192):
            continue
        t = -(-M // bm) * -(-C_out // bn)
        key = (0, -t, 0) if t <= n_cus else (1, -(-t // n_cus), -(-t // n_cus) * bm * bn)
        if best_key is None or key < best_key:
            best, best_key = I5_FLAG + 1 + i, key
    return best


def fused_tail_rounds(desc, n_cus=256):
    M = desc.N * desc.H_out * desc.W_out
    if resident_applies(desc, min_images=1):
        return -(-desc.N * 4 // n_cus)
    if directw_applies(desc):
        th = max(1, 256 // desc.W_out)
        return -(-desc.N * -(-desc.H_out // th) // n_cus)
    return min(-(-(-(-M // bm) * -(-desc.C_out // bn)) // n_cus) for bm, bn in I5_TILES if (bm, bn) != (128, 192))


class WgradJob(C.Structure):
    _fields_ = [("desc", ConvDesc), ("dy", C.c_void_p), ("dy_img_stride", C.c_int64), ("ld_dy", C.c_int32),
                ("scale", C.c_float), ("dw", C.c_void_p), ("db", C.c_void_p)]


class WgradPlanInfo(C.Structure):
    _fields_ = [("n_layers", C.c_int32), ("n_items", C.c_int32), ("layers_off", C.c_int64), ("items_off", C.c_int64),
                ("queues_off", C.c_int64), ("heads_off", C.c_int64), ("flops", C.c_double), ("tally_off", C.c_int64)]


class View:
    __slots__ = ("buf", "N", "H", "W", "C", "ld", "ch_off", "elem_size")

    def __init__(self, buf, N, H, W, C, ld=None, ch_off=0, elem_size=2):
        self.buf, self.N, self.H, self.W, self.C = buf, N, H, W, C
        self.ld = C if ld is None else ld
        self.ch_off, self.elem_size = ch_off, elem_size
        assert buf.numel() * buf.element_size() >= N * H * W * self.ld * elem_size, "view larger than its buffer"

    @property
    def ptr(self):
        return self.buf.data_ptr() + self.ch_off * self.elem_size

    @property
    def img_stride(self):
        return self.H * self.W * self.ld

    @property
    def M(self):
        return self.N * self.H * self.W

    def slice(self, off, C):
        assert off + C <= self.C
        return View(self.buf, self.N, self.H, self.W, C, self.ld, self.ch_off + off, self.elem_size)

    def tensor(self):
        dt = self.buf.dtype
        flat = self.buf.reshape(-1)[: self.N * self.H * self.W * self.ld].reshape(self.N, self.H, self.W, self.ld)
        return flat[..., self.ch_off:self.ch_off + self.C]

    @staticmethod
    def alloc(N, H, W, C, ld=None, dtype=torch.bfloat16, device="cuda", zero=False):
        ld = C if ld is None else ld
        f = torch.zeros if zero else torch.empty
        buf = f((N, H, W, ld), dtype=dtype, device=device)
        if not zero and os.environ.get("MBX_POISON"):
            buf.fill_(float("nan"))
        return View(buf, N, H, W, C, ld, 0, torch.empty((), dtype=dtype).element_size())


def _stream():
    return torch.cuda.current_stream().cuda_stream


def _p(t):
    return None if t is None else t.data_ptr()


def make_desc(x: View, w, C_out, R, S, stride, pad_t, pad_l, y: View, transposed=0, epilogue=EPI_STORE, relu=0,
              accumulate=0, scale=None, shift=None, skip: View = None, rscale=0.0, stats=None, acc_src: View = None,
              stats_rows_mod=0, stats_ld=0, relu_bits=None, ld_bits=0):
    d = ConvDesc()
    d.x, d.x_img_stride, d.ldx = x.ptr, x.img_stride, x.ld
    d.N, d.H_in, d.W_in, d.C_in = x.N, x.H, x.W, x.C
    d.w, d.C_out, d.R, d.S = (w.data_ptr() if w is not None else None), C_out, R, S
    d.stride, d.transposed, d.pad_t, d.pad_l = stride, transposed, pad_t, pad_l
    d.H_out, d.W_out = y.H, y.W
    d.y, d.y_img_stride, d.ldy = y.ptr, y.img_stride, y.ld
    d.epilogue, d.relu, d.accumulate = epilogue, int(relu), int(accumulate)
    d.scale, d.shift = _p(scale), _p(shift)
    if skip is not None:
        d.skip, d.skip_img_stride, d.ld_skip = skip.ptr, skip.img_stride, skip.ld
    d.rscale = float(rscale)
    d.stats_partial = _p(stats)
    d.stats_rows_mod, d.stats_ld = int(stats_rows_mod), int(stats_ld)
    if acc_src is not None:
        d.acc_src, d.acc_img_stride, d.ld_acc = acc_src.ptr, acc_src.img_stride, acc_src.ld
    if relu_bits is not None:
        d.relu_bits, d.ld_bits = relu_bits.data_ptr(), int(ld_bits if ld_bits else relu_bits.shape[-1])
    return d


def conv(desc: ConvDesc):
    _lib.check(_lib.lib().mbx_conv(C.byref(desc), _stream()), "mbx_conv")


def conv_stats_rows(desc: ConvDesc):
    r = _lib.lib().mbx_conv_stats_rows(C.byref(desc))
    if r < 0:
        _lib.check(r, "mbx_conv_stats_rows")
    return r


def conv_wgrad(desc: ConvDesc, dy: View, dw, db=None):
    _lib.check(_lib.lib().mbx_conv_wgrad(C.byref(desc), dy.ptr, dy.img_stride, dy.ld, dw.data_ptr(), _p(db), _stream()),
               "mbx_conv_wgrad")


WG_OVERLAP_DEFAULT = 0


def wgrad_overlap_cus():
    return max(0, int(os.environ.get("MBX_WG_OVERLAP", WG_OVERLAP_DEFAULT)))


N_TILE_CONFIGS = 14
I5_FLAG = 32
I5_TILE_CONFIGS = (33, 34, 35, 36, 37, 38, 39)
I5_TILES = ((128, 64), (128, 128), (192, 128), (256, 128), (256, 64), (128, 192), (128, 256))
I7_TILE_CONFIG = 65
I7_COUNTERS = 32
SPLITK_FLAG = 128
DIRECT3_TILE_CONFIG = 96


def direct3_applies(desc: ConvDesc, min_pixels=300000):
    if os.environ.get("MBX_DIRECT3", "1") == "0":
        return False
    if desc.R != 3 or desc.S != 3 or desc.epilogue not in (EPI_STORE, EPI_AFFINE) or desc.accumulate or desc.skip \
            or desc.rscale != 0.0 or (desc.epilogue == EPI_AFFINE and desc.stats_partial) or desc.bn_bwd_stats:
        return False
    if desc.stride == 2 and not desc.transposed and desc.C_in == 8 and desc.C_out <= 32 and desc.C_out % 8 == 0:
        pass
    elif desc.stride != 1 or desc.C_in not in (32, 64) or desc.C_out > 64 or desc.C_out % 8 or (desc.C_in == 64 and desc.C_out > 48):
        return False
    if -(-desc.W_out // 32) * 32 > 1.15 * desc.W_out:
        return False
    return desc.N * desc.H_out * desc.W_out >= int(os.environ.get("MBX_DIRECT3_MIN_PIXELS", min_pixels))


DIRECTW_TILE_CONFIG = 97


def directw_applies(desc: ConvDesc, min_pixels=60000):
    if os.environ.get("MBX_DIRECTW", "1") == "0":
        return False
    if desc.R != 3 or desc.S != 3 or desc.stride != 1 or desc.epilogue not in (EPI_STORE, EPI_AFFINE) or desc.accumulate or desc.skip \
            or desc.rscale != 0.0 or (desc.epilogue == EPI_AFFINE and desc.stats_partial) or desc.bn_bwd_stats:
        return False
    if desc.C_in not in (32, 48, 64) or desc.C_out > 64 or desc.C_out % 8 or (desc.C_in == 64 and desc.C_out > 48):
        return False
    if not (8 <= desc.W_out <= 64) or desc.W_in > desc.W_out + 2:
        return False
    return desc.N * desc.H_out * desc.W_out >= int(os.environ.get("MBX_DIRECTW_MIN_PIXELS", min_pixels))


RESIDENT_TILE_CONFIG = 98


def resident_applies(desc: ConvDesc, min_images=32):
    if os.environ.get("MBX_RESIDENT", "1") == "0":
        return False
    if desc.R * desc.S not in (3, 7) or min(desc.R, desc.S) != 1 or desc.stride != 1 or desc.epilogue not in (EPI_STORE, EPI_AFFINE) \
            or desc.accumulate or desc.skip or desc.rscale != 0.0 or (desc.epilogue == EPI_AFFINE and desc.stats_partial) \
            or desc.bn_bwd_stats or desc.relu_bits:
        return False
    if desc.H_in != desc.H_out or desc.W_in != desc.W_out or not (64 <= desc.H_out * desc.W_out <= 289):
        return False
    if desc.N < int(os.environ.get("MBX_RESIDENT_MIN_IMAGES", min_images)):
        return False
    if not desc.x or not desc.w or not desc.y:
        hw = desc.H_out * desc.W_out
        if desc.C_out % 8:
            return False
        if desc.R * desc.S == 3:
            return hw == 64 and desc.C_in in (192, 224, 256)
        return 65 <= hw <= 289 and desc.C_in in (128, 160, 192)
    keep = desc.tile_config
    desc.tile_config = RESIDENT_TILE_CONFIG
    ok = _lib.lib().mbx_conv_supported(C.byref(desc)) == 0
    desc.tile_config = keep
    return ok


PWRES_DEFAULT = "2"
PWRES_TILE_CONFIG = 99


def pwres_applies(desc: ConvDesc, min_pixels=4096):
    mode = os.environ.get("MBX_PWRES", PWRES_DEFAULT)
    if mode == "0":
        return False
    if desc.R != 1 or desc.S != 1 or desc.stride != 1 or desc.pad_t or desc.pad_l or desc.stats_partial or desc.bn_bwd_stats:
        return False
    if desc.C_in not in (96, 128, 320, 384, 448) or desc.C_out < 256 or desc.C_out % 8:
        return False
    res = desc.epilogue == EPI_RESIDUAL
    accm = desc.epilogue == EPI_STORE and desc.relu_bits and not desc.skip
    if not (res or accm) or (mode == "2" and not accm):
        return False
    return desc.N * desc.H_out * desc.W_out >= int(os.environ.get("MBX_PWRES_MIN_PIXELS", min_pixels))


def launch_rule(desc: ConvDesc, pair=False):
    if direct3_applies(desc):
        return DIRECT3_TILE_CONFIG, "direct 3x3"
    if directw_applies(desc) and not pair:
        return DIRECTW_TILE_CONFIG, "direct 3x3 (whole-width)"
    if pwres_applies(desc):
        return PWRES_TILE_CONFIG, "pixel-resident 1x1"
    if resident_applies(desc):
        return RESIDENT_TILE_CONFIG, "resident image"
    return None


def splitk_slices(desc: ConvDesc, n_cus=256):
    if os.environ.get("MBX_SPLITK", "1") == "0" or desc.transposed or desc.epilogue != EPI_STORE or desc.accumulate or desc.skip:
        return 0
    ktot = desc.R * desc.S * desc.C_in
    M = desc.N * desc.H_out * desc.W_out
    tiles = ((M + 127) // 128) * ((desc.C_out + 63) // 64)
    if ktot < 8192 or tiles > 96:
        return 0
    s = int(os.environ.get("MBX_SPLITK_SLICES", "0")) or max(2, min(16, (2 * n_cus) // tiles))
    return min(s, 32)
_TUNED = {}
TUNE_STATS = {"hits": 0, "remeasured": 0, "rejected": 0}
_TUNE_FILE = os.path.join(os.path.dirname(os.path.abspath(__file__)), "tune_cache.json")


def _load_tune_cache():
    if os.environ.get("MBX_TUNE_CACHE", "1") != "0" and os.path.exists(_TUNE_FILE):
        try:
            import json
            with open(_TUNE_FILE) as f:
                _TUNED.update({k: int(v) for k, v in json.load(f).items()})
        except (OSError, ValueError):
            pass


def save_tune_cache(path=None):
    import json
    with open(path or _TUNE_FILE, "w") as f:
        json.dump(dict(sorted(_TUNED.items())), f, indent=0)


_load_tune_cache()


def autotune(desc: ConvDesc, key, candidates=None, iters=10):
    key = repr(key)
    if key in _TUNED:
        desc.tile_config = _TUNED[key]
        if _lib.lib().mbx_conv_supported(C.byref(desc)) == 0:
            TUNE_STATS["hits"] += 1
            return desc.tile_config
        del _TUNED[key]
        TUNE_STATS["rejected"] += 1
    TUNE_STATS["remeasured"] += 1
    if candidates is None:
        candidates = (0, 2, 4, 5, 6, 9, 10, 12, 13, 14)
        if os.environ.get("MBX_AUTOTUNE_SET") == "all":
            candidates = tuple(range(0, N_TILE_CONFIGS + 1))
    l = _lib.lib()
    best, best_t = 0, float("inf")
    s = _stream()
    iters = int(os.environ.get("MBX_TUNE_ITERS", iters))
    for cfg in candidates:
        desc.tile_config = cfg
        if l.mbx_conv(C.byref(desc), s) != 0:
            continue
        e0, e1 = torch.cuda.Event(enable_timing=True), torch.cuda.Event(enable_timing=True)
        e0.record()
        for _ in range(iters):
            l.mbx_conv(C.byref(desc), s)
        e1.record()
        e1.synchronize()
        t = e0.elapsed_time(e1)
        if t < best_t * 0.97 or (cfg == 0 and t < best_t):
            best, best_t = cfg, t
    desc.tile_config = best
    _TUNED[key] = best
    return best


def autotune_wgrad(desc: ConvDesc, dy: View, scale, dw, db, key, candidates=(0, 2, 3, 4, 7, 8, 9, 10), iters=10):
    key = repr(key)
    if key in _TUNED:
        desc.tile_config = _TUNED[key]
        return desc.tile_config
    l = _lib.lib()
    s = _stream()
    best, best_t = 0, float("inf")
    iters = int(os.environ.get("MBX_TUNE_ITERS", iters))
    if os.environ.get("MBX_AUTOTUNE_WG"):
        candidates = tuple(int(v) for v in os.environ["MBX_AUTOTUNE_WG"].split(","))
    args = (dy.ptr, dy.img_stride, dy.ld, float(scale), dw.data_ptr(), _p(db), s)
    for cfg in candidates:
        desc.tile_config = cfg
        if l.mbx_conv_wgrad_scaled(C.byref(desc), *args) != 0:
            continue
        e0, e1 = torch.cuda.Event(enable_timing=True), torch.cuda.Event(enable_timing=True)
        e0.record()
        for _ in range(iters):
            l.mbx_conv_wgrad_scaled(C.byref(desc), *args)
        e1.record()
        e1.synchronize()
        t = e0.elapsed_time(e1)
        if t < best_t * 0.97 or (cfg == 0 and t < best_t):
            best, best_t = cfg, t
    desc.tile_config = best
    _TUNED[key] = best
    return best


class WgradGroup:

    def __init__(self, jobs, deterministic=False, device="cuda"):
        l = _lib.lib()
        self.n = len(jobs)
        arr = (WgradJob * self.n)(*jobs)
        flags = (1 if deterministic else 0) | (2 if os.environ.get("MBX_WGRAD_SCATTER") == "1" else 0)
        nbytes = l.mbx_wgrad_plan_bytes(arr, self.n, flags)
        assert nbytes > 0
        host = (C.c_uint8 * nbytes)()
        self.info = WgradPlanInfo()
        _lib.check(l.mbx_wgrad_plan(arr, self.n, flags, host, nbytes, C.byref(self.info)), "mbx_wgrad_plan")
        import numpy as np
        self.host_image = np.frombuffer(host, dtype=np.uint8).copy()
        self.image = torch.from_numpy(self.host_image).to(device)
        self.flops = float(self.info.flops)

    def launch(self, max_workgroups=0):
        _lib.check(_lib.lib().mbx_conv_wgrad_grouped_capped(self.image.data_ptr(), C.byref(self.info), int(max_workgroups),
                                                            _stream()), "mbx_conv_wgrad_grouped")

    def tally(self):
        o = int(self.info.tally_off)
        t = self.image[o:o + 16].cpu().numpy().view("<u8")
        return int(t[0]), int(t[1])

    def completed_ok(self):
        items, launches = self.tally()
        return items == launches * int(self.info.n_items)

    def reset(self):
        self.image.copy_(torch.from_numpy(self.host_image))
```

Before: 4349 images/sec.

## Add parity-split stride-2 data-gradient kernel that skips zero taps

Adds a stride-2 transposed-convolution (data gradient) path to the igemm5 persistent kernel. Output pixels are grouped into four parity classes, each padded to a tile boundary, so every tile loops only over the filter taps that contribute for its parity. This removes the multiply-by-zero work of the dilated formulation. It adds per-tile variable K-loop lengths, an atomic work queue, and new host-side routing for large stride-2 transposed convs without BN or mask epilogues. The cost is some padding waste at class boundaries and more code complexity.

```diff
diff --git a/include/mbx.h b/include/mbx.h
--- a/include/mbx.h
+++ b/include/mbx.h
@@ -202,6 +202,7 @@
 #define MBX_TILE_DIRECTW 97
 #define MBX_TILE_RESIDENT 98
 #define MBX_TILE_PWRES 99
+#define MBX_TILE_S2DGRAD_BASE 100
 #define MBX_TILE_SPLITK_BASE 128
 #define MBX_TILE_SPLITK_MAX 32
 
diff --git a/multibox_amd/csrc/conv.hip b/multibox_amd/csrc/conv.hip
--- a/multibox_amd/csrc/conv.hip
+++ b/multibox_amd/csrc/conv.hip
@@ -317,6 +317,7 @@
 constexpr int kDirectWCfg = MBX_TILE_DIRECTW;
 constexpr int kResidentCfg = MBX_TILE_RESIDENT;
 constexpr int kPwResCfg = MBX_TILE_PWRES;
+constexpr int kS2Flag = MBX_TILE_S2DGRAD_BASE;
 constexpr int kSplitFlag = MBX_TILE_SPLITK_BASE;
 constexpr int kSplitMax = MBX_TILE_SPLITK_MAX;
 inline void splitk_geom(int nk, int S, int& ksplit, int& kps) {
@@ -431,6 +432,7 @@
   if (d->tile_config == kDirectWCfg) { const int g = mbx_directw_grid(d->N, d->H_out, d->W_out); return g > 0 ? g : MBX_ERR_UNSUPPORTED; }
   if (d->tile_config == kResidentCfg) return mbx_resident_rows(d->N);
   if (d->tile_config == kI7Cfg) return (int)((M + 127) / 128);
+  if (d->tile_config > kS2Flag) return MBX_ERR_UNSUPPORTED;
   if (d->tile_config > kI5Flag) {
     const int i = d->tile_config - kI5Flag - 1;
     if (i >= mbx_i5_num_tiles) return MBX_ERR_INVALID_ARG;
@@ -617,7 +619,7 @@
     k.stagger = mbx_env_int("MBX_STAGGER", 0);
   }
 #endif
-  for (int c = 0; c < 4; ++c) { k.cls_m0[c] = 0; k.cls_hw[c] = 1; k.cls_w[c] = 1; }
+  for (int c = 0; c < 4; ++c) { k.cls_m0[c] = 0; k.cls_hw[c] = 1; k.cls_w[c] = 1; k.cls_n[c] = 0; }
   static const bool notap = mbx_env_char("MBX_NO_TAP_SKIP") == '1';
   if (k.shift && d->C_in % 64 == 0 && !notap) {
     int m0 = 0;
@@ -660,6 +662,7 @@
   if (d->tile_config == kResidentCfg) return mbx_launch_resident(k, d->N, d->H_out, s);
   if (d->tile_config == kPwResCfg) return mbx_launch_pwres(k, s);
   if (d->tile_config == kI7Cfg) return mbx_launch_igemm7(k, s);
+  if (d->tile_config > kS2Flag) return mbx_launch_s2dgrad(k, d->tile_config - kS2Flag - 1, s);
   if (d->tile_config > kI5Flag) return mbx_launch_igemm5(k, d->tile_config - kI5Flag - 1, s);
   switch (choose_cfg(k.M, k.C_out, d->tile_config)) {
     case 0: return launch_igemm<128, 128, 2, 2>(k, s);
diff --git a/multibox_amd/csrc/conv5.hip b/multibox_amd/csrc/conv5.hip
--- a/multibox_amd/csrc/conv5.hip
+++ b/multibox_amd/csrc/conv5.hip
@@ -21,11 +21,29 @@
   static_assert(LDS_BYTES <= 160 * 1024, "LDS");
 };
 
+struct S2Tile { int nk, kr0, ks0, nts, mlim; };
+__device__ __forceinline__ S2Tile s2_tile(const ConvK& p, const int m0) {
+  const int c = pixel_class(p, m0);
+  S2Tile t;
+  t.kr0 = (p.pad_t + (c >> 1)) & 1;
+  t.ks0 = (p.pad_l + (c & 1)) & 1;
+  t.nts = (p.S - t.ks0 + 1) >> 1;
+  t.nk = ((p.R - t.kr0 + 1) >> 1) * t.nts * ((p.C_in + 63) >> 6);
+  t.mlim = 0x7fffffff;
+#pragma unroll
+  for (int j = 0; j < 4; ++j) {
+    const int e = p.cls_m0[j] + p.cls_n[j];
+    t.mlim = (e > m0 && e < t.mlim) ? e : t.mlim;
+  }
+  return t;
+}
+
 template <int MY, int NW, int EV, int MODE>
 __global__ void __launch_bounds__(1024)
 conv_igemm5_kernel(const ConvK p) {
   using G = Ig5<MY, NW>;
-  constexpr bool PW = MODE == 1;
+  constexpr bool PW = MODE == 1, S2 = MODE == 2;
+  static_assert(!S2 || EV == 0 || EV == 2, "the stride-2 data gradient: store / accumulate (+ bf16 mask)");
   constexpr int BM = G::BM, BN = G::BN, TM = G::TM, TN = G::TN, MI = G::MI, NI = G::NI, STAGE = G::STAGE, NST = G::NST;
   constexpr int NLW = 8, LV = 1;
   constexpr int NL = LV * (MY + NW);
@@ -47,8 +65,8 @@
   }
 #endif
   const int nk = (p.Ktot + 63) >> 6;
-  const bool fused_tail = ((EV == 1) && p.fa.bar != nullptr) || ((EV == 0) && p.fb.bar != nullptr);
-  const bool queued = p.work_counter != nullptr && nk > NST && ntiles > (int)gridDim.x && !fused_tail;
+  const bool fused_tail = !S2 && (((EV == 1) && p.fa.bar != nullptr) || ((EV == 0) && p.fb.bar != nullptr));
+  const bool queued = p.work_counter != nullptr && (S2 || nk > NST) && ntiles > (int)gridDim.x && !fused_tail;
 
   if (wave >= 8) {
     const int lw0 = wave - 8;
@@ -63,18 +81,32 @@
     int t_i = first, it_i = 0, st_issue = 0, j_i = 0;
     int hb[LV][MY], wb[LV][MY], ro[LV][MY], wo[LV][NW];
     int kc = 0, kr = 0, ks = 0;
+    int nk_i = nk, kr0_i = 0, ks0_i = 0, nts_i = 1, jr = 0, js = 0, kt = 0;
+    const int nkc = (p.C_in + 63) >> 6;
 #define MBX5_SETUP_TILE()                                                                                     \
   do {                                                                                                        \
     const int tn_ = t_i % p.tiles_n, tm_ = t_i / p.tiles_n;                                                   \
+    S2Tile g_ = S2Tile{};                                                                                     \
+    if (S2) {                                                                                                 \
+      g_ = s2_tile(p, tm_ * BM);                                                                              \
+      nk_i = g_.nk; kr0_i = g_.kr0; ks0_i = g_.ks0; nts_i = g_.nts; jr = 0; js = 0; kt = 0;                   \
+    }                                                                                                         \
+    const int mlim_ = S2 ? g_.mlim : p.M;                                                                     \
     _Pragma("unroll") for (int v = 0; v < LV; ++v) {                                                          \
       const int lw = lw0 + NLW * v;                                                                           \
       _Pragma("unroll") for (int i = 0; i < MY; ++i) {                                                        \
         const int m = tm_ * BM + 64 * i + 8 * lw + r8;                                                        \
-        const bool mv = m < p.M;                                                                              \
+        const bool mv = m < mlim_;                                                                            \
         int img, oh, ow;                                                                                      \
-        decode_pixel(p, mv ? (unsigned)m : 0u, img, oh, ow);                                                  \
-        hb[v][i] = mv ? oh * p.mul - p.pad_t : -(1 << 24);                                                    \
-        wb[v][i] = ow * p.mul - p.pad_l;                                                                      \
+        if (S2) {                    \
+          decode_pixel_parity(p, mv ? (unsigned)m : (unsigned)(tm_ * BM), img, oh, ow);                       \
+          hb[v][i] = mv ? (oh - p.pad_t + g_.kr0) >> 1 : -(1 << 24);                                          \
+          wb[v][i] = (ow - p.pad_l + g_.ks0) >> 1;                                                            \
+        } else {                                                                                              \
+          decode_pixel(p, mv ? (unsigned)m : 0u, img, oh, ow);                                                \
+          hb[v][i] = mv ? oh * p.mul - p.pad_t : -(1 << 24);                                                  \
+          wb[v][i] = ow * p.mul - p.pad_l;                                                                    \
+        }                                                                                                     \
         ro[v][i] = (img * p.x_img_stride + (hb[v][i] * p.W_in + wb[v][i]) * p.ldx) * 2;                       \
         if (PW && !mv) ro[v][i] = (int)kOOB;                                                                  \
       }                                                                                                       \
@@ -94,6 +126,15 @@
       if (PW) {                                                                                               \
         _Pragma("unroll") for (int i = 0; i < MY; ++i)                                                        \
           glds16(xr, sp + i * 512, (kv && ro[v][i] >= 0) ? (ro[v][i] + kc * 2) : (int)kOOB);                  \
+      } else if (S2) {                                                                                        \
+        const int kcl = kt * 64 + chunk * 8;                                                                  \
+        const bool kvp = kcl < p.C_in;                                 \
+        const int toff = (jr * p.W_in + js) * ldx2 + kcl * 2;                                                 \
+        _Pragma("unroll") for (int i = 0; i < MY; ++i) {                                                      \
+          const bool ok = kvp && ((unsigned)(hb[v][i] + jr) < (unsigned)p.H_in) &&                            \
+                          ((unsigned)(wb[v][i] + js) < (unsigned)p.W_in);                                     \
+          glds16(xr, sp + i * 512, ok ? (ro[v][i] + toff) : (int)kOOB);                                       \
+        }                                                                                                     \
       } else {                                                                                                \
         const int toff = (kr * p.W_in + ks) * ldx2 + kc * 2;                                                  \
         _Pragma("unroll") for (int i = 0; i < MY; ++i) {                                                      \
@@ -108,15 +149,21 @@
   do {                                                                                                        \
     _Pragma("unroll") for (int v = 0; v < LV; ++v) {                                                          \
       u32x4* sp = smem + st_issue * STAGE + (lw0 + NLW * v) * 64;                                             \
-      const int kb = (it_i * 64 + chunkw[v] * 8) * 2;                     \
-      const bool kvw = kb < p.Ktot * 2;                                                                       \
+      const int kcw = kt * 64 + chunkw[v] * 8;                         \
+      const int kb = S2 ? (((kr0_i + 2 * jr) * p.S + ks0_i + 2 * js) * p.C_in + kcw) * 2                       \
+                        : (it_i * 64 + chunkw[v] * 8) * 2;                \
+      const bool kvw = S2 ? kcw < p.C_in : kb < p.Ktot * 2;                \
       _Pragma("unroll") for (int i = 0; i < NW; ++i)                                                          \
         glds16(wr, sp + (MY + i) * 512, (kvw && wo[v][i] >= 0) ? (wo[v][i] + kb) : (int)kOOB);                \
     }                                                                                                         \
-    kc += 64;                                                                                                 \
-    while (kc >= p.C_in) { kc -= p.C_in; if (++ks >= p.S) { ks = 0; ++kr; } }                                 \
+    if (S2) {                                                                                                 \
+      if (++kt == nkc) { kt = 0; if (++js == nts_i) { js = 0; ++jr; } }                                       \
+    } else {                                                                                                  \
+      kc += 64;                                                                                               \
+      while (kc >= p.C_in) { kc -= p.C_in; if (++ks >= p.S) { ks = 0; ++kr; } }                               \
+    }                                                                                                         \
     st_issue = st_issue == NST - 1 ? 0 : st_issue + 1;                                                        \
-    if (++it_i == nk) {                                                                                       \
+    if (++it_i == nk_i) {                                                                                     \
       it_i = 0; ++j_i;                                                                                        \
       t_i = queued ? s_ids[j_i & 3] : t_i + (int)gridDim.x;                                                   \
       if (t_i < ntiles) MBX5_SETUP_TILE();                                                                    \
@@ -140,7 +187,8 @@
     raw_barrier();
     int jc = 0;
     for (int t = first; t < ntiles; t = queued ? s_ids[++jc & 3] : t + (int)gridDim.x) {
-      for (int it = 0; it < nk; ++it) {
+      const int nk_c = S2 ? s2_tile(p, (t / p.tiles_n) * BM).nk : nk;
+      for (int it = 0; it < nk_c; ++it) {
         const bool more = t_i < ntiles;
         st_pub = st_pub == NST - 1 ? 0 : st_pub + 1;
 #ifdef MBX_I5_STAMPS
@@ -189,6 +237,8 @@
   for (int t = first; t < ntiles; t = queued ? s_ids[++jt & 3] : t + (int)gridDim.x) {
     const int tile_n = t % p.tiles_n, tile_m = t / p.tiles_n;
     const int m0 = tile_m * BM, n0 = tile_n * BN;
+    int nk_c = nk, mend = -1;
+    if constexpr (S2) { const S2Tile g_ = s2_tile(p, m0); nk_c = g_.nk; mend = g_.mlim; }
 #ifdef MBX_I5_STAMPS
     const int tnum = (t - first) / (int)gridDim.x;
     const bool stamp = p.stamps && tid == 0 && tnum < 8 && blockIdx.x < 64;
@@ -207,7 +257,7 @@
     constexpr int PREB = PRE_RAW > MI ? MI : PRE_RAW;
     const int cl0 = wn * TN + fch * 8, mlane = m0 + wm * TM + frow, clane = n0 + cl0;
     u32x4 pla[PREB > 0 ? PREB : 1][NA], plb[PREB > 0 ? PREB : 1][NA];
-    if constexpr (PREB > 0) conv_epilogue_issue_reads<EVC, false, NA, PREB, BMODE>(p, mlane, clane, 0, pla, plb);
+    if constexpr (PREB > 0) conv_epilogue_issue_reads<EVC, S2, NA, PREB, BMODE>(p, mlane, clane, 0, pla, plb, mend);
     int raw2 = 0;
     if (fetcher) raw2 = fetch_raw();
     f32x4 acc[NI][MI];
@@ -215,7 +265,7 @@
     for (int a = 0; a < NI; ++a)
 #pragma unroll
       for (int b = 0; b < MI; ++b) acc[a][b] = f32x4{0.f, 0.f, 0.f, 0.f};
-    for (int it = 0; it < nk; ++it) {
+    for (int it = 0; it < nk_c; ++it) {
 #ifdef MBX_I5_STAMPS
       if (p.dbg & 1) { st_comp = st_comp == NST - 1 ? 0 : st_comp + 1; raw_barrier(); continue; }
 #endif
@@ -247,12 +297,12 @@
     float s1[NA][8], s2[NA][8], sc[NA][8], sh[NA][8];
     conv_epilogue_channels<EVC, NA>(p, clane, sc, sh, s1, s2);
     if constexpr (PREB > 0) {
-      conv_epilogue_finish<EVC, false, NI, MI, PREB, BMODE>(p, acc, mlane, clane, 0, pla, plb, sh, sc, s1, s2);
+      conv_epilogue_finish<EVC, S2, NI, MI, PREB, BMODE>(p, acc, mlane, clane, 0, pla, plb, sh, sc, s1, s2, mend);
       asm volatile("" ::: "memory");
     }
     if constexpr (PREB < MI) {
       constexpr int REM = MI - PREB, CH = (EV == 0 || EV == 1 || EV == 3) ? REM : (REM % 2 == 0 ? 2 : 1);
-      conv_epilogue_range<EVC, false, NI, MI, PREB, MI, CH, BMODE>(p, acc, mlane, clane, sh, sc, s1, s2);
+      conv_epilogue_range<EVC, S2, NI, MI, PREB, MI, CH, BMODE>(p, acc, mlane, clane, sh, sc, s1, s2, mend);
     }
     MBX5_STAMP(2);
     if constexpr (EV == 1 || EV == 6) {
@@ -287,7 +337,7 @@
       });
     }
   }
-  if constexpr (EV == 0 && !(MY == 2 && NW == 3)) {
+  if constexpr (EV == 0 && !S2 && !(MY == 2 && NW == 3)) {
     if (fused_tail) {
       constexpr int NT = 512 + 64 * NLW;
       static_assert(NT * 68 + sizeof(FbShared) <= G::RING_BYTES, "the tail's reduce area fits the ring");
@@ -346,6 +396,55 @@
   return MBX_OK;
 }
 
+template <int MY, int NW>
+int launch5s(ConvK& k, hipStream_t s) {
+  using G = Ig5<MY, NW>;
+  const int N = k.M / k.HW_out, H_out = k.HW_out / k.W_out;
+  int m0 = 0, nk_min = 1 << 30;
+  for (int c = 0; c < 4; ++c) {
+    const int hc = (H_out - (c >> 1) + 1) / 2, wc = (k.W_out - (c & 1) + 1) / 2, n = N * hc * wc;
+    k.cls_m0[c] = m0;
+    k.cls_n[c] = n;
+    k.cls_hw[c] = hc * wc > 0 ? hc * wc : 1;
+    k.cls_w[c] = wc > 0 ? wc : 1;
+    m0 += (n + G::BM - 1) / G::BM * G::BM;
+    if (n > 0) {
+      const int kr0 = (k.pad_t + (c >> 1)) & 1, ks0 = (k.pad_l + (c & 1)) & 1;
+      const int nk = ((k.R - kr0 + 1) >> 1) * ((k.S - ks0 + 1) >> 1) * ((k.C_in + 63) >> 6);
+      if (nk < nk_min) nk_min = nk;
+    }
+  }
+  if (nk_min < 1) return MBX_ERR_UNSUPPORTED;
+  k.parity = k.skip_taps = 1;
+  k.tiles_m = m0 / G::BM;
+  k.tiles_n = (k.C_out + G::BN - 1) / G::BN;
+  k.stats_cap = 0.f;
+  if (nk_min <= G::NST) k.work_counter = nullptr;
+  const int ntiles = k.tiles_m * k.tiles_n;
+  const int ncu = conv_cus();
+  int grid = ntiles < ncu ? ntiles : ncu;
+  if (k.max_wg > 0 && grid > k.max_wg) grid = k.max_wg;
+  constexpr bool kNo2 = MY == 4 && NW == 2;
+  const bool ev2 = k.accumulate || k.skip;
+  if (ev2 && kNo2) return MBX_ERR_UNSUPPORTED;
+  if (k.dry) return MBX_OK;
+  static bool attr[2] = {};
+#define MBX5S_LAUNCH(EV, SLOT)                                                                                \
+  do {                                                                                                        \
+    if (!attr[SLOT]) {                                                                                        \
+      (void)hipFuncSetAttribute(reinterpret_cast<const void*>(conv_igemm5_kernel<MY, NW, EV, 2>),             \
+                                hipFuncAttributeMaxDynamicSharedMemorySize, G::LDS_BYTES);                    \
+      attr[SLOT] = true;                                                                                      \
+    }                                                                                                         \
+    hipLaunchKernelGGL((conv_igemm5_kernel<MY, NW, EV, 2>), dim3(grid), dim3(1024), G::LDS_BYTES, s, k);      \
+  } while (0)
+  if (!ev2) MBX5S_LAUNCH(0, 0);
+  else if constexpr (!kNo2) MBX5S_LAUNCH(2, 1);
+#undef MBX5S_LAUNCH
+  MBX_LAUNCH_CHECK();
+  return MBX_OK;
+}
+
 }
 
 extern const int mbx_i5_tiles[][2] = {{128, 64}, {128, 128}, {192, 128}, {256, 128}, {256, 64}, {128, 192}, {128, 256}};
@@ -364,3 +463,16 @@
     default: return MBX_ERR_UNSUPPORTED;
   }
 }
+
+extern const int mbx_s2_tiles[][2] = {{128, 128}, {256, 128}, {256, 64}};
+extern const int mbx_s2_num_tiles = 3;
+
+int mbx_launch_s2dgrad(ConvK& k, int index, hipStream_t s) {
+  if (!k.shift || k.C_in % 32 || k.epi != MBX_EPI_STORE || k.stats || k.bw_n || k.bits || k.fa.bar || k.fb.bar) return MBX_ERR_UNSUPPORTED;
+  switch (index) {
+    case 0: return launch5s<2, 2>(k, s);
+    case 1: return launch5s<4, 2>(k, s);
+    case 2: return launch5s<4, 1>(k, s);
+    default: return MBX_ERR_UNSUPPORTED;
+  }
+}
diff --git a/multibox_amd/csrc/conv_common.h b/multibox_amd/csrc/conv_common.h
--- a/multibox_amd/csrc/conv_common.h
+++ b/multibox_amd/csrc/conv_common.h
@@ -30,6 +30,7 @@
   unsigned mg_hw, sh_hw, mg_w, sh_w;
   int pw;
   int cls_m0[4], cls_hw[4], cls_w[4];
+  int cls_n[4];
   int skip_taps;
   int parity;
   int* work_counter;
@@ -48,6 +49,9 @@
 int mbx_launch_igemm5(mbx::ConvK& k, int index, hipStream_t s);
 extern const int mbx_i5_tiles[][2];
 extern const int mbx_i5_num_tiles;
+int mbx_launch_s2dgrad(mbx::ConvK& k, int index, hipStream_t s);
+extern const int mbx_s2_tiles[][2];
+extern const int mbx_s2_num_tiles;
 int mbx_launch_igemm7(mbx::ConvK& k, hipStream_t s);
 int mbx_launch_direct3(mbx::ConvK& k, int N, int H_out, hipStream_t s);
 int mbx_direct3_grid(int N, int H_out, int W_out);
@@ -244,8 +248,8 @@
 __device__ __forceinline__ void lds_readback_wait(unsigned v) { asm volatile("s_waitcnt lgkmcnt(0)" ::"v"(v) : "memory"); }
 
 template <bool SH>
-__device__ __forceinline__ void epi_pixel(const ConvK& p, const int m, int& img, int& pix) {
-  const unsigned mm = m < p.M ? (unsigned)m : 0u;
+__device__ __forceinline__ void epi_pixel(const ConvK& p, const int m, int& img, int& pix, const int mend = -1) {
+  const unsigned mm = m < (mend >= 0 ? mend : p.M) ? (unsigned)m : 0u;
   if (SH && p.parity) {
     int oh_, ow_;
     decode_pixel_parity(p, mm, img, oh_, ow_);
@@ -258,7 +262,8 @@
 
 template <int EV, bool SH, int NA, int BCH, int BMODE = 1>
 __device__ __forceinline__ void conv_epilogue_issue_reads(const ConvK& p, const int mlane, const int clane, const int b0,
-                                                          u32x4 (&la)[BCH][NA], u32x4 (&lb)[BCH][NA]) {
+                                                          u32x4 (&la)[BCH][NA], u32x4 (&lb)[BCH][NA], const int mend = -1) {
+  const int M_ = mend >= 0 ? mend : p.M;
   if constexpr (EV == 6) {
 #pragma unroll
     for (int A = 0; A < NA; ++A) {
@@ -283,11 +288,11 @@
     for (int bb = 0; bb < BCH; ++bb) {
       const int m = mlane + (b0 + bb) * 16;
       int img, pix;
-      epi_pixel<SH>(p, m, img, pix);
+      epi_pixel<SH>(p, m, img, pix, mend);
 #pragma unroll
       for (int A = 0; A < NA; ++A) {
         const int c0 = clane + 32 * A;
-        const bool ok = m < p.M && c0 < p.C_out;
+        const bool ok = m < M_ && c0 < p.C_out;
         const unsigned so = ok ? (unsigned)((img * p.skip_img_stride + pix * p.ld_skip + c0) * 2) : kOOB;
         if constexpr (EV == 4) {
           la[bb][A] = buf_load16(kr_, so);
@@ -306,8 +311,9 @@
 __device__ __forceinline__ void conv_epilogue_finish(const ConvK& p, const f32x4 (&acc)[NI][MI], const int mlane, const int clane,
                                                      const int b0, const u32x4 (&la)[BCH][NI / 2], const u32x4 (&lb)[BCH][NI / 2],
                                                      const float (&sh)[NI / 2][8], const float (&sc)[NI / 2][8],
-                                                     float (&s1)[NI / 2][8], float (&s2)[NI / 2][8]) {
+                                                     float (&s1)[NI / 2][8], float (&s2)[NI / 2][8], const int mend = -1) {
   constexpr int NA = NI / 2;
+  const int M_ = mend >= 0 ? mend : p.M;
   const __amdgpu_buffer_rsrc_t yr = make_rsrc(p.y, p.y_bytes);
   const bool do_acc = EV == 2 && p.accumulate, do_mask = EV == 2 && BMODE != 2 && p.skip != nullptr;
   const bool do_bits = (EV == 2 && BMODE == 2) || ((EV == 2 || EV == 4) && BMODE == 1 && p.bits != nullptr);
@@ -318,12 +324,12 @@
     const int b = b0 + bb;
     const int m = mlane + b * 16;
     int img, pix;
-    epi_pixel<SH>(p, m, img, pix);
+    epi_pixel<SH>(p, m, img, pix, mend);
     unsigned bits_dw = 0;
 #pragma unroll
     for (int A = 0; A < NA; ++A) {
       const int c0 = clane + 32 * A;
-      const unsigned yo = (m < p.M && c0 < p.C_out) ? (unsigned)((img * p.y_img_stride + pix * p.ldy + c0) * 2) : kOOB;
+      const unsigned yo = (m < M_ && c0 < p.C_out) ? (unsigned)((img * p.y_img_stride + pix * p.ldy + c0) * 2) : kOOB;
       float v[8] = {acc[2 * A][b][0], acc[2 * A][b][1], acc[2 * A][b][2], acc[2 * A][b][3],
                     acc[2 * A + 1][b][0], acc[2 * A + 1][b][1], acc[2 * A + 1][b][2], acc[2 * A + 1][b][3]};
       if constexpr (EV == 3) {
@@ -457,14 +463,14 @@
 template <int EV, bool SH, int NI, int MI, int B0, int B1, int BCH, int BMODE = 1>
 __device__ __forceinline__ void conv_epilogue_range(const ConvK& p, const f32x4 (&acc)[NI][MI], const int mlane, const int clane,
                                                     const float (&sh)[NI / 2][8], const float (&sc)[NI / 2][8],
-                                                    float (&s1)[NI / 2][8], float (&s2)[NI / 2][8]) {
+                                                    float (&s1)[NI / 2][8], float (&s2)[NI / 2][8], const int mend = -1) {
   static_assert((B1 - B0) % BCH == 0 && B0 >= 0 && B1 <= MI, "chunks");
   constexpr int NA = NI / 2;
 #pragma unroll
   for (int b0 = B0; b0 < B1; b0 += BCH) {
     u32x4 la[BCH][NA], lb[BCH][NA];
-    conv_epilogue_issue_reads<EV, SH, NA, BCH, BMODE>(p, mlane, clane, b0, la, lb);
-    conv_epilogue_finish<EV, SH, NI, MI, BCH, BMODE>(p, acc, mlane, clane, b0, la, lb, sh, sc, s1, s2);
+    conv_epilogue_issue_reads<EV, SH, NA, BCH, BMODE>(p, mlane, clane, b0, la, lb, mend);
+    conv_epilogue_finish<EV, SH, NI, MI, BCH, BMODE>(p, acc, mlane, clane, b0, la, lb, sh, sc, s1, s2, mend);
     if (b0 + BCH < B1) asm volatile("" ::: "memory");
   }
 }
diff --git a/multibox_amd/engine.py b/multibox_amd/engine.py
--- a/multibox_amd/engine.py
+++ b/multibox_amd/engine.py
@@ -721,6 +721,10 @@
             rule = ops.launch_rule(d, pair) if over is None else None
             if rule is not None:
                 d.tile_config, d.work_counter = rule[0], None
+                if d.tile_config > ops.S2DGRAD_BASE and os.environ.get("MBX_I5_STATIC") != "1":
+                    assert self._i5_used + 1 <= self.i5_counters.numel()
+                    d.work_counter = self.i5_counters.data_ptr() + 4 * self._i5_used
+                    self._i5_used += 1
                 _lib.check(_lib.lib().mbx_conv_supported(C.byref(d)), rule[1] + " " + op.name)
         return d
 
diff --git a/multibox_amd/ops.py b/multibox_amd/ops.py
--- a/multibox_amd/ops.py
+++ b/multibox_amd/ops.py
@@ -267,6 +267,32 @@
     return desc.N * desc.H_out * desc.W_out >= int(os.environ.get("MBX_PWRES_MIN_PIXELS", min_pixels))
 
 
+S2DGRAD_BASE = 100
+S2DGRAD_TILES = ((128, 128), (256, 128), (256, 64))
+S2DGRAD_TILE_CONFIGS = (101, 102, 103)
+
+
+def stride2_dgrad_applies(desc: ConvDesc):
+    if os.environ.get("MBX_S2DGRAD", "1") == "0":
+        return 0
+    if not desc.transposed or desc.stride != 2 or desc.epilogue != EPI_STORE or desc.C_in % 32 or desc.R * desc.S < 2:
+        return 0
+    if desc.stats_partial or desc.bn_bwd_stats or desc.relu_bits or desc.bn_apply or desc.bn_bwd:
+        return 0
+    if desc.N * desc.H_out * desc.W_out < int(os.environ.get("MBX_S2DGRAD_MIN_PIXELS", S2DGRAD_MIN_PIXELS)):
+        return 0
+    plain = not (desc.accumulate or desc.skip)
+    forced = int(os.environ.get("MBX_S2DGRAD_TILE", "0"))
+    if forced:
+        return S2DGRAD_BASE + (forced if plain or S2DGRAD_TILES[forced - 1] != (256, 128) else 1)
+    if plain:
+        return S2DGRAD_BASE + 2
+    return S2DGRAD_BASE + (3 if 0 < desc.C_out % 128 <= 64 else 1)
+
+
+S2DGRAD_MIN_PIXELS = 16384
+
+
 def launch_rule(desc: ConvDesc, pair=False):
     if direct3_applies(desc):
         return DIRECT3_TILE_CONFIG, "direct 3x3"
@@ -276,6 +302,9 @@
         return PWRES_TILE_CONFIG, "pixel-resident 1x1"
     if resident_applies(desc):
         return RESIDENT_TILE_CONFIG, "resident image"
+    s2 = stride2_dgrad_applies(desc)
+    if s2:
+        return s2, "stride-2 data gradient"
     return None
 
 
```

Result: no change. 4385 images/sec, median of 6 (+0.8%).
